# leopard-ai/betty

Measured on AMD Instinct MI355X. Metric: hypergradient-steps/sec (CG K=20, 10M inner params), higher is better.
Workload: dtype f32

## Files before the change

### betty_amd/_native.py

```python
from __future__ import annotations

import ctypes
import os
from ctypes import POINTER, c_char_p, c_double, c_float, c_int, c_int32, c_int64, c_size_t, c_void_p

_HERE = os.path.dirname(os.path.abspath(__file__))
LIB_PATH = os.environ.get("BHG_LIB") or os.path.join(_HERE, "csrc", "libbhg.so")
AB_LIB_PATH = os.environ.get("BHG_AB_LIB") or os.path.join(_HERE, "csrc", "libbhg_ab.so")

BHG_CHUNK_ELEMS = 4096
BHG_FLAT_ALIGN = 64
BHG_CG_AUTO, BHG_CG_STREAM, BHG_CG_RESIDENT = 0, 1, 2
BHG_CG_GLOBAL_CHAIN, BHG_CG_GLOBAL_UPDATE, BHG_CG_GLOBAL_DOTS = 0, 1, 2
BHG_CG_FX_BEGIN, BHG_CG_FX_CHAIN, BHG_CG_FX_GRAM, BHG_CG_FX_END = 0, 1, 2, 3


class NativeLibraryError(RuntimeError):
    """libbhg.so is missing or a call into it failed."""


class Chunk(ctypes.Structure):

    _fields_ = [
        ("flat_off", c_int64),
        ("src_off", c_int64),
        ("tensor", c_int32),
        ("len", c_int32),
    ]


BHG_MLP_MAX_LAYERS = 32


class Mlp(ctypes.Structure):

    _fields_ = [
        ("L", c_int32),
        ("B", c_int32),
        ("Bp", c_int32),
        ("dims", c_int32 * (BHG_MLP_MAX_LAYERS + 1)),
        ("W", c_void_p * BHG_MLP_MAX_LAYERS),
        ("h", c_void_p * BHG_MLP_MAX_LAYERS),
        ("mask", c_void_p * BHG_MLP_MAX_LAYERS),
        ("delta", c_void_p * BHG_MLP_MAX_LAYERS),
        ("prob", c_void_p),
        ("sd", c_void_p),
        ("Rh", c_void_p * BHG_MLP_MAX_LAYERS),
        ("Rd", c_void_p * BHG_MLP_MAX_LAYERS),
        ("partial", c_void_p),
        ("partial_floats", c_size_t),
        ("ridge2", c_float),
        ("prepacked", c_int32),
    ]


_PP = POINTER(c_void_p)
_CH = c_void_p

SYMBOLS = {
    "bhg_version": (c_int, []),
    "bhg_last_error": (c_char_p, []),
    "bhg_layout_flat_size": (c_int64, [POINTER(c_int64), c_int]),
    "bhg_layout_num_chunks": (c_int64, [POINTER(c_int64), c_int]),
    "bhg_layout_build": (c_int, [POINTER(c_int64), c_int, POINTER(c_int64), POINTER(Chunk)]),
    "bhg_workspace_bytes": (c_size_t, [c_int]),
    "bhg_flatten": (c_int, [_PP, c_int, _CH, c_int, c_void_p, c_float, c_void_p, c_void_p]),
    "bhg_scatter": (c_int, [c_void_p, _PP, c_int, _CH, c_int, c_float, c_void_p, c_void_p]),
    "bhg_neumann_init": (c_int, [_PP, c_int, _CH, c_int, c_void_p, c_void_p, c_void_p, c_void_p]),
    "bhg_neumann_step": (
        c_int,
        [_PP, c_int, _CH, c_int, c_void_p, c_void_p, c_float, c_float, c_float, c_void_p, c_void_p],
    ),
    "bhg_cg_init": (c_int, [_PP, c_int, _CH, c_int, c_void_p, c_void_p, c_void_p, c_void_p, c_void_p]),
    "bhg_cg_init_masked": (c_int, [_PP, c_int, _CH, c_int, c_void_p, c_void_p, c_void_p, ctypes.c_uint64, c_void_p, c_void_p]),
    "bhg_cg_step": (
        c_int,
        [_PP, c_int, _CH, c_int, c_void_p, c_void_p, c_void_p, c_float, c_int, c_float, c_float, c_int, c_void_p, c_void_p],
    ),
    "bhg_cg_phase": (
        c_int,
        [c_int, _PP, c_int, _CH, c_int, c_void_p, c_void_p, c_void_p, c_float, c_int, c_float, c_float, c_void_p, c_void_p],
    ),
    "bhg_cg_partials_dev": (c_void_p, [c_void_p, c_int, c_int]),
    "bhg_cg_partials_count": (c_int, []),
    "bhg_cg_resident_capacity_chunks": (c_int, []),
    "bhg_cg_resident_ok": (c_int, []),
    "bhg_cg_resident_usable": (c_int, [c_int]),
    "bhg_cg_scalars_dev": (c_void_p, [c_void_p]),
    "bhg_cg_timeout_flag_dev": (c_void_p, [c_void_p]),
    "bhg_scale_flat": (c_int, [c_void_p, c_int64, c_float, c_void_p]),
    "bhg_darts_eps": (c_int, [_PP, c_int, _CH, c_int, c_double, c_void_p, c_void_p, c_void_p, c_void_p]),
    "bhg_axpy_multi": (c_int, [_PP, _PP, c_int, _CH, c_int, c_void_p, c_float, c_void_p, c_void_p]),
    "bhg_fd_perturb": (c_int, [_PP, c_void_p, _PP, c_int, _CH, c_int, c_void_p, c_float, c_void_p, c_void_p]),
    "bhg_cg_step_fd": (
        c_int,
        [_PP, _PP, c_void_p, c_int, _CH, c_int, c_void_p, c_void_p, c_void_p, c_float, c_int, c_float, c_float, c_int, c_void_p, c_void_p],
    ),
    "bhg_neumann_step_fd": (
        c_int,
        [_PP, _PP, c_void_p, c_int, _CH, c_int, c_void_p, c_void_p, c_float, c_float, c_float, c_void_p, c_void_p],
    ),
    "bhg_sama_adam_precondition": (
        c_int,
        [_PP, _PP, _PP, _PP, c_int, _CH, c_int, c_void_p, c_double, c_double, c_double, c_double, c_void_p, c_void_p],
    ),
    "bhg_debug_set": (c_int, [c_char_p, c_int]),
    "bhg_debug_unset": (c_int, [c_char_p]),
    "bhg_debug_reset": (None, []),
    "bhg_debug_key_count": (c_int, []),
    "bhg_debug_key_name": (c_char_p, [c_int]),
    "bhg_is_ab_build": (c_int, []),
    "bhg_timing_enable": (c_int, [c_int]),
    "bhg_timing_read": (c_int, [c_int, POINTER(c_double), POINTER(c_int)]),
    "bhg_logreg_prepare": (c_int, [c_void_p, c_void_p, c_void_p, c_int, c_int, c_void_p]),
    "bhg_logreg_tmp_floats": (c_size_t, [c_int, c_int]),
    "bhg_logreg_hvp": (
        c_int,
        [c_void_p, c_void_p, c_void_p, c_void_p, c_void_p, c_void_p, c_int, c_int, c_void_p],
    ),
    "bhg_mlp_partial_floats": (c_size_t, [POINTER(Mlp)]),
    "bhg_mlp_hvp": (c_int, [POINTER(Mlp), _PP, _PP, c_void_p]),
    "bhg_mlp_hvp_mode": (c_int, [POINTER(Mlp), _PP, _PP, c_int, c_void_p]),
    "bhg_mlp_supports_native_prepare": (c_int, [POINTER(Mlp)]),
    "bhg_mlp_forward": (c_int, [POINTER(Mlp), _PP, c_void_p, c_void_p, c_void_p]),
    "bhg_mlp_backward": (c_int, [POINTER(Mlp), c_void_p, c_void_p]),
    "bhg_mlp_mixed_coeff": (c_int, [POINTER(Mlp), _PP, c_void_p, c_void_p, c_void_p]),
    "bhg_mlp_supports_fused_solve": (c_int, [POINTER(Mlp)]),
    "bhg_mlp_fused_ws_bytes": (c_size_t, [POINTER(Mlp)]),
    "bhg_mlp_cg_solve": (
        c_int,
        [POINTER(Mlp), c_void_p, c_void_p, c_void_p, POINTER(c_int64), _CH, c_int, c_int, c_float, c_float, c_void_p,
         c_void_p, c_size_t, c_void_p],
    ),
    "bhg_mlp_cg_state_mask": (ctypes.c_uint64, [POINTER(Mlp), c_int]),
    "bhg_mlp_cg_solve_rhs": (
        c_int,
        [POINTER(Mlp), c_void_p, c_void_p, c_void_p, POINTER(c_int64), _CH, c_int, c_int, c_float, c_float, c_void_p,
         c_void_p, c_size_t, _PP, c_void_p],
    ),
    "bhg_mlp_cg_global_phase": (
        c_int,
        [POINTER(Mlp), c_void_p, c_void_p, c_void_p, POINTER(c_int64), _CH, c_int, c_int, c_int, c_int, c_int, c_void_p, c_float,
         c_float, c_void_p, c_void_p, c_size_t, c_void_p],
    ),
    "bhg_mlp_fx_supported": (c_int, [POINTER(Mlp), c_int]),
    "bhg_mlp_fx_ws_bytes": (c_size_t, [POINTER(Mlp), c_int]),
    "bhg_mlp_fx_const_floats": (c_size_t, [POINTER(Mlp)]),
    "bhg_mlp_fx_slab_floats": (c_size_t, [POINTER(Mlp)]),
    "bhg_mlp_fx_scal_doubles": (c_size_t, [POINTER(Mlp)]),
    "bhg_mlp_cg_fx_phase": (
        c_int,
        [POINTER(Mlp), _PP, c_int, c_int, c_int, c_int, c_int, c_void_p, c_void_p, c_void_p, c_float, c_float, c_void_p, c_size_t,
         c_void_p, c_size_t, c_void_p],
    ),
    "bhg_mlp_neumann_fx_phase": (
        c_int,
        [POINTER(Mlp), _PP, c_int, c_int, c_int, c_int, c_int, c_void_p, c_void_p, c_void_p, c_float, c_float, c_void_p, c_size_t,
         c_void_p, c_size_t, c_void_p],
    ),
    "bhg_mlp_cg_mixed_coeff": (c_int, [POINTER(Mlp), c_void_p, c_void_p, c_float, c_void_p, c_size_t, c_void_p]),
    "bhg_mlp_timeout_flag_dev": (c_void_p, [POINTER(Mlp), c_void_p]),
    "bhg_mlp_stage_batch": (c_int, [POINTER(Mlp), c_void_p, c_void_p, c_void_p, c_void_p]),
    "bhg_mlp_supports_packed_prepare": (c_int, [POINTER(Mlp)]),
    "bhg_mlp_forward_packed": (c_int, [POINTER(Mlp), _PP, c_void_p, c_void_p, c_void_p, c_size_t, c_void_p]),
    "bhg_mlp_backward_packed": (c_int, [POINTER(Mlp), c_void_p, c_void_p, c_size_t, c_void_p]),
    "bhg_mwn_max_hidden": (c_int, []),
    "bhg_mlp_fd_ws_bytes": (c_size_t, [POINTER(c_int), c_int, c_int]),
    "bhg_mlp_fd_forward": (
        c_int,
        [c_void_p, c_void_p, c_int, POINTER(c_int), c_int, _PP, _PP, c_void_p, c_int, c_void_p, c_void_p, c_void_p, c_size_t, c_void_p],
    ),
    "bhg_mwn_fd_vjp": (
        c_int,
        [c_void_p, c_void_p, c_int, c_void_p, c_void_p, c_void_p, c_void_p, c_int, c_void_p, c_int, c_void_p, c_void_p, c_void_p, c_void_p,
         c_void_p],
    ),
    "bhg_quad_fd": (c_int, [_PP, _PP, _PP, c_int, _CH, c_int, c_void_p, c_float, c_int, c_int, c_int, c_void_p]),
    "bhg_mwn_forward": (c_int, [c_void_p, c_int, c_void_p, c_void_p, c_void_p, c_void_p, c_int, c_void_p, c_void_p, c_void_p]),
    "bhg_mwn_backward": (
        c_int,
        [c_void_p, c_void_p, c_int, c_void_p, c_void_p, c_void_p, c_void_p, c_int, c_float, c_void_p, c_void_p, c_void_p, c_void_p, c_void_p],
    ),
    "bhg_mlp_neumann_solve": (
        c_int,
        [POINTER(Mlp), c_void_p, c_void_p, c_void_p, POINTER(c_int64), c_int, c_float, c_float, c_void_p, c_size_t, POINTER(c_int), c_void_p],
    ),
    "bhg_mlp_wsk_launches": (c_int64, []),
    "bhg_mlp_hoist_launches": (c_int64, []),
    "bhg_mlp_proj_iterations": (c_int64, []),
    "bhg_mlp_lin_launches": (c_int64, []),
    "bhg_mlp_neumann_mixed_coeff": (c_int, [POINTER(Mlp), _PP, c_void_p, c_void_p, c_float, c_int, c_int, c_void_p, c_size_t, c_void_p]),
    "bhg_mlp_plan_describe": (c_int, [POINTER(Mlp), c_int, c_int, ctypes.c_char_p, c_size_t]),
    "bhg_copy2d": (c_int, [c_void_p, c_int64, c_void_p, c_int64, c_int64, c_int64, c_void_p]),
    "bhg_bn_ws_bytes": (c_size_t, [c_int]),
    "bhg_bn_backward_vjp": (
        c_int,
        [c_void_p, c_void_p, c_void_p, c_void_p, c_void_p, c_void_p, c_void_p, c_void_p, c_int, c_int, c_int, c_void_p, c_void_p, c_void_p,
         c_void_p, c_size_t, c_void_p],
    ),
}

_libs = {}
_current = [None]


_PY_ENV = {"BHG_LIB", "BHG_AB_LIB", "BHG_HVP_GRAPH", "BHG_ALL_RANKS_ON_GPU0"}
_warned_env = [False]


def _warn_legacy_env() -> None:
    if _warned_env[0]:
        return
    _warned_env[0] = True
    stale = sorted(k for k in os.environ if k.startswith("BHG_") and k not in _PY_ENV)
    if stale:
        import warnings

        warnings.warn("betty_amd: environment variable(s) " + ", ".join(stale) + " are IGNORED — libbhg reads no environment variable. "
                      "Measurement arms are selected with betty_amd._native.use_ab() + debug_set(key, int) (bench.py --debug KEY=INT) "
                      "on the measurement build libbhg_ab.so.", RuntimeWarning, stacklevel=3)


def _bind(path: str) -> ctypes.CDLL:
    lib = _libs.get(path)
    if lib is not None:
        return lib
    _warn_legacy_env()
    if not os.path.exists(path):
        raise NativeLibraryError(
            f"{path} not found: the HIP extension has not been built. Run "
            "`python -c 'import __graft_entry__ as g; g.build()'` or `make -C betty_amd/csrc`. "
            "betty_amd has no CPU fallback."
        )
    lib = ctypes.CDLL(path)
    for name, (restype, argtypes) in SYMBOLS.items():
        try:
            fn = getattr(lib, name)
        except AttributeError as exc:
            raise NativeLibraryError(f"{path} does not export {name}") from exc
        fn.restype = restype
        fn.argtypes = argtypes
    _libs[path] = lib
    return lib


def load() -> ctypes.CDLL:
    return _bind(_current[0] or LIB_PATH)


def current_lib_path() -> str:
    return _current[0] or LIB_PATH


def is_ab() -> bool:
    return bool(load().bhg_is_ab_build())


def use_ab(on: bool = True) -> None:
    if on:
        _bind(AB_LIB_PATH)
        _current[0] = AB_LIB_PATH
    else:
        _current[0] = None


def check(rc: int, what: str) -> None:
    if rc != 0:
        msg = load().bhg_last_error()
        raise NativeLibraryError(f"{what} failed with code {rc}: {msg.decode() if msg else ''}")


def _debug_key(key: str) -> bytes:
    k = key.strip()
    if k.upper().startswith("BHG_"):
        k = k[4:]
    return k.lower().encode()


def debug_set(key: str, value) -> None:
    lib = load()
    if value is not None and not lib.bhg_is_ab_build():
        raise NativeLibraryError(f"bhg_debug_set({key}): the product libbhg.so carries no measurement arm — call "
                                 "betty_amd._native.use_ab() first (libbhg_ab.so; the `bhg_debug` fixture and `bench.py --debug` do)")
    if value is None:
        check(lib.bhg_debug_unset(_debug_key(key)), f"bhg_debug_unset({key})")
    else:
        check(lib.bhg_debug_set(_debug_key(key), int(value)), f"bhg_debug_set({key})")


def debug_reset() -> None:
    load().bhg_debug_reset()


def debug_keys():
    lib = load()
    return [lib.bhg_debug_key_name(i).decode() for i in range(lib.bhg_debug_key_count())]


def ptr_array(ptrs):
    arr = (c_void_p * len(ptrs))(*ptrs)
    return ctypes.cast(arr, _PP), arr


def plan_describe(dims, B: int, algo: str = "cg", keep_solution: bool = False) -> dict:
    lib = load()
    d = Mlp()
    d.L, d.B, d.Bp = len(dims) - 1, int(B), (int(B) + 127) // 128 * 128
    for i, v in enumerate(dims):
        d.dims[i] = int(v)
    buf = ctypes.create_string_buffer(2048)
    check(lib.bhg_mlp_plan_describe(ctypes.byref(d), {"cg": 0, "neumann": 1}[algo], 1 if keep_solution else 0, buf, 2048), "bhg_mlp_plan_describe")
    out, text = {}, buf.value.decode()
    import re

    for key, quoted, plain in re.findall(r'(\w+)=(?:"([^"]*)"|(\S+))', text):
        val = quoted if quoted else plain
        out[key] = int(val) if re.fullmatch(r"-?\d+", val) else val
    return out
```

### betty_amd/csrc/bhg_common.hpp

```cpp
#pragma once
#include <hip/hip_runtime.h>
#include <stdint.h>
#include <stddef.h>
#include <stdio.h>
#include <string.h>

#include "bhg.h"

namespace bhg {

constexpr int kThreads = 256;
constexpr int kWaves = kThreads / 64;
constexpr int kChunk = BHG_CHUNK_ELEMS;
constexpr int kVecPerThread = kChunk / (kThreads * 4);
constexpr int kMaxBlocks = 1024;
constexpr int kInlineT = 32;
constexpr int kWriterT = 448;

constexpr size_t kWsScal = 0;
constexpr size_t kWsPartP = 128;
constexpr size_t kWsPartR = kWsPartP + 8 * kMaxBlocks;
constexpr size_t kWsBarrier = kWsPartR + 16 * kMaxBlocks;
constexpr size_t kWsTables = kWsBarrier + 256;
inline size_t ws_bytes(int T) {
  size_t b = kWsTables + 4 * sizeof(void*) * (size_t)(T > 0 ? T : 0);
  return (b + 255) & ~(size_t)255;
}

enum { S_RR_OLD = 0, S_PHP = 1, S_ALPHA = 2, S_RR_NEW = 3, S_BETA = 4, S_PP = 5 , S_ALPHA_RING = 10 ,
       S_NPART0 = 8  };

#define BHG_DBG_KEYS(X)                                                                                                      \
  X(mlp_wsk) X(mlp_wsk_maxk) X(mlp_wsk_depth) X(mlp_wsk_lds) X(wsl_depth) X(no_nt_slabs) X(gemm_no_xpose) X(mlp_no_fast)      \
  X(mlp_tn) X(split_target) X(split_cap) X(mlp_no_head) X(gram_ksplit) X(gram_kchunk) X(proj_graw_split) X(mlp_proj)         \
  X(mlp_hoist) X(hoist_wgs) X(proj_step_alone) X(mlp_no_side) X(mlp_no_fuse) X(mlp_no_outer_all) X(neumann_side)             \
  X(hoist_staged_mink) X(proj_alpha_alone) X(proj_small_alone) X(outer_order_by_work) X(outer_no_pre) X(outer_stagger)       \
  X(mlp_no_fused_solve) X(cg_eager_p) X(cg_x_every_iter) X(neumann_p_every_iter) X(head_no_prefetch) X(cg_spin_limit)        \
  X(packed_chain) X(packed_depth) X(packed_gram) X(proj_max_ratio) X(proj_ws_cap_mb) X(alpha_in_hoist) X(graw_v2) X(wskp_ragged) X(pstep_v2) X(pstep_unroll) X(rnew_in_graw) X(graw_cols) X(lin_first) X(lin_prio) X(lin_nub) X(lin_order) X(lin_update_next) X(lin_withhold_beta) X(neumann_vnew) X(cg_rhs_direct) X(packed_prepare) X(lin_deep) X(graw_kloop) X(lin_update_in_head) X(xcd_pairs) X(headu_head_first) X(fx_ksplit)
enum DbgKey : int {
#define BHG_DBG_ENUM(n) DBG_##n,
  BHG_DBG_KEYS(BHG_DBG_ENUM)
#undef BHG_DBG_ENUM
  DBG_COUNT
};
constexpr int kDbgUnset = INT32_MIN;
#ifdef BHG_AB
extern int g_dbg[DBG_COUNT];
inline bool dbg_is_set(DbgKey k) { return g_dbg[k] != kDbgUnset; }
inline int dbg(DbgKey k, int dflt) { return g_dbg[k] == kDbgUnset ? dflt : g_dbg[k]; }
#else
constexpr bool dbg_is_set(DbgKey) { return false; }
constexpr int dbg(DbgKey, int dflt) { return dflt; }
#endif

constexpr int kStampKernels = 4, kStampBlocks = 4096, kStampSlots = 8;
#ifdef BHG_STAMPS
#ifdef __HIPCC__
#define BHG_STAMP(kid, slot)                                                                                            \
  do {                                                                                                                  \
    if (threadIdx.x == 0 && blockIdx.x < ::bhg::kStampBlocks) {                                                         \
      unsigned long long* sp_ = ::bhg::d_stamps;                                                                        \
      if (sp_) sp_[((kid) * ::bhg::kStampBlocks + blockIdx.x) * ::bhg::kStampSlots + (slot)] = wall_clock64();          \
    }                                                                                                                   \
  } while (0)
#endif
#else
#define BHG_STAMP(kid, slot) do { } while (0)
#endif

void set_error(const char* fmt, ...);
#define BHG_HIP_CHECK(expr)                                                        \
  do {                                                                             \
    hipError_t _e = (expr);                                                        \
    if (_e != hipSuccess) {                                                        \
      ::bhg::set_error("%s failed: %s (%s:%d)", #expr, hipGetErrorString(_e), __FILE__, \
                       __LINE__);                                                  \
      return BHG_ERR_HIP;                                                          \
    }                                                                              \
  } while (0)
#define BHG_REQUIRE(cond, msg)                                                     \
  do {                                                                             \
    if (!(cond)) {                                                                 \
      ::bhg::set_error("%s: %s", __func__, msg);                                   \
      return BHG_ERR_ARG;                                                          \
    }                                                                              \
  } while (0)

struct PtrTab {
  const void* const* dev;
  const void* inl[kInlineT];
};

int make_table(PtrTab* out, const void* const* host_ptrs, int T, void* ws, int slot,
               hipStream_t stream);

bool span_begin(int kind, hipEvent_t* a, hipEvent_t* b);

#ifdef __HIPCC__
__device__ __forceinline__ float* tab_ptr(const PtrTab& t, int i) {
  const void* p = t.dev ? t.dev[i] : t.inl[i];
  return (float*)p;
}

__device__ __forceinline__ float4 ld4(const float* __restrict__ base, int e, int len) {
  if (e + 4 <= len) return *reinterpret_cast<const float4*>(base + e);
  float4 r = make_float4(0.f, 0.f, 0.f, 0.f);
  if (e < len) r.x = base[e];
  if (e + 1 < len) r.y = base[e + 1];
  if (e + 2 < len) r.z = base[e + 2];
  return r;
}
__device__ __forceinline__ void st4(float* __restrict__ base, int e, int len, float4 v) {
  if (e + 4 <= len) {
    *reinterpret_cast<float4*>(base + e) = v;
    return;
  }
  if (e < len) base[e] = v.x;
  if (e + 1 < len) base[e + 1] = v.y;
  if (e + 2 < len) base[e + 2] = v.z;
}

template <int BYTES>
__device__ __forceinline__ void kernarg_warm() {
  typedef const __attribute__((address_space(4))) unsigned* KP;
  KP kp = (KP)__builtin_amdgcn_kernarg_segment_ptr();
  unsigned acc = 0;
#pragma unroll
  for (int o = 0; o < BYTES; o += 64) acc |= kp[o / 4];
  asm volatile("" ::"s"(acc));
}
template <int U>
__device__ __forceinline__ double sum_strided(const double* __restrict__ p, const int n, const int t, const int stride) {
  double acc = 0.0;
  for (int i0 = t; i0 < n; i0 += U * stride) {
    double v[U];
#pragma unroll
    for (int u = 0; u < U; ++u) {
      const int i = i0 + u * stride;
      v[u] = p[i < n ? i : n - 1];
    }
#pragma unroll
    for (int u = 0; u < U; ++u)
      if (i0 + u * stride < n) acc += v[u];
  }
  return acc;
}

template <int U>
struct StridedRegs { double v[U]; };
template <int U>
__device__ __forceinline__ void strided_load(StridedRegs<U>& r, const double* __restrict__ p, const int n, const int t, const int stride,
                                             const double* __restrict__ dummy) {
  const double* q = (p && n > 0) ? p : dummy;
  const int last = (p && n > 0) ? n - 1 : 0;
#pragma unroll
  for (int u = 0; u < U; ++u) {
    const int i = t + u * stride;
    r.v[u] = q[i < n && i <= last ? i : last];
  }
}
template <int U>
__device__ __forceinline__ double strided_sum(const StridedRegs<U>& r, const int n, const int t, const int stride) {
  double acc = 0.0;
#pragma unroll
  for (int u = 0; u < U; ++u)
    if (t + u * stride < n) acc += r.v[u];
  return acc;
}

template <int CTRL>
__device__ __forceinline__ double dpp_mov_f64(const double v) {
  const unsigned long long u = __builtin_bit_cast(unsigned long long, v);
  const unsigned lo = (unsigned)__builtin_amdgcn_mov_dpp((int)(unsigned)u, CTRL, 0xf, 0xf, true);
  const unsigned hi = (unsigned)__builtin_amdgcn_mov_dpp((int)(unsigned)(u >> 32), CTRL, 0xf, 0xf, true);
  return __builtin_bit_cast(double, ((unsigned long long)hi << 32) | (unsigned long long)lo);
}
__device__ __forceinline__ double readlane_f64(const double v, const int lane) {
  const unsigned long long u = __builtin_bit_cast(unsigned long long, v);
  const unsigned lo = (unsigned)__builtin_amdgcn_readlane((int)(unsigned)u, lane);
  const unsigned hi = (unsigned)__builtin_amdgcn_readlane((int)(unsigned)(u >> 32), lane);
  return __builtin_bit_cast(double, ((unsigned long long)hi << 32) | (unsigned long long)lo);
}
__device__ __forceinline__ double wave_sum(double v) {
  v += dpp_mov_f64<0xB1>(v);
  v += dpp_mov_f64<0x4E>(v);
  v += dpp_mov_f64<0x141>(v);
  v += dpp_mov_f64<0x140>(v);
  const double r0 = readlane_f64(v, 0), r1 = readlane_f64(v, 16), r2 = readlane_f64(v, 32), r3 = readlane_f64(v, 48);
  return (r0 + r1) + (r2 + r3);
}
template <int CTRL>
__device__ __forceinline__ float dpp_mov_f32(const float v) {
  return __builtin_bit_cast(float, __builtin_amdgcn_mov_dpp(__builtin_bit_cast(int, v), CTRL, 0xf, 0xf, true));
}
__device__ __forceinline__ float wave_sum_f32(float v) {
  v += dpp_mov_f32<0xB1>(v);
  v += dpp_mov_f32<0x4E>(v);
  v += dpp_mov_f32<0x141>(v);
  v += dpp_mov_f32<0x140>(v);
  const float r0 = __builtin_bit_cast(float, __builtin_amdgcn_readlane(__builtin_bit_cast(int, v), 0));
  const float r1 = __builtin_bit_cast(float, __builtin_amdgcn_readlane(__builtin_bit_cast(int, v), 16));
  const float r2 = __builtin_bit_cast(float, __builtin_amdgcn_readlane(__builtin_bit_cast(int, v), 32));
  const float r3 = __builtin_bit_cast(float, __builtin_amdgcn_readlane(__builtin_bit_cast(int, v), 48));
  return (r0 + r1) + (r2 + r3);
}
__device__ __forceinline__ void block_sum3(double& a, double& b, double& c, double* red) {
  const double wa = wave_sum(a), wb = wave_sum(b), wc = wave_sum(c);
  const int lane = threadIdx.x & 63, w = threadIdx.x >> 6;
  __syncthreads();
  if (lane == 0) { red[w] = wa; red[kWaves + w] = wb; red[2 * kWaves + w] = wc; }
  __syncthreads();
  double sa = 0.0, sb = 0.0, sc = 0.0;
#pragma unroll
  for (int i = 0; i < kWaves; ++i) { sa += red[i]; sb += red[kWaves + i]; sc += red[2 * kWaves + i]; }
  a = sa; b = sb; c = sc;
}
__device__ __forceinline__ double block_sum(double v, double* red) {
  v = wave_sum(v);
  const int lane = threadIdx.x & 63, w = threadIdx.x >> 6;
  __syncthreads();
  if (lane == 0) red[w] = v;
  __syncthreads();
  double s = 0.0;
#pragma unroll
  for (int i = 0; i < kWaves; ++i) s += red[i];
  return s;
}
__device__ __forceinline__ double sum_partials(const double* __restrict__ part, int n,
                                               double* red) {
  double a = 0.0;
  for (int i = threadIdx.x; i < n; i += kThreads) a += part[i];
  return block_sum(a, red);
}
#endif

}
```

### betty_amd/csrc/bhg_mlp.hip

```cpp
#include <stdlib.h>
#include <vector>


#include "bhg_common.hpp"

#ifdef BHG_STAMPS
namespace bhg { __device__ unsigned long long* d_stamps = nullptr; }
#endif

namespace bhg {
namespace {
#include "mlp/gemm.inc"

#include "mlp/outer.inc"

#include "mlp/scalars.inc"

#include "mlp/head.inc"

#include "mlp/wsk.inc"

#include "mlp/wskp.inc"

inline int wsk_mode(int chain_mode, int unfused_hint) {
  if (dbg_is_set(DBG_mlp_wsk)) return dbg(DBG_mlp_wsk, 0);
  if (chain_mode == FUSE_CG) return 2;
  if (chain_mode == FUSE_NEUMANN) return 3;
  return unfused_hint;
}
inline bool wsk_wanted(int mode, int pairs, int K) {
  if (mode == 1) return true;
  if (mode != 2 && mode != 3) return false;
  return pairs * K <= dbg(DBG_mlp_wsk_maxk, 1024);
}
inline int wsk_depth() {
  const int d = dbg(DBG_mlp_wsk_depth, 3);
  return d == 2 ? 2 : 3;
}
inline bool wsk_eligible(const WskArgs& a) {
  if (a.pairs < 1 || a.pairs > 2) return false;
  bool ok = a.M % 32 == 0 && a.N % 32 == 0 && a.K % 32 == 0 && a.K >= 32;
  for (int i = 0; i < a.pairs; ++i) ok = ok && (a.pr[i].lda & 3) == 0 && (a.pr[i].ldb & 3) == 0;
  return ok;
}
int64_t g_wsk_launches = 0;
int64_t g_hoist_launches = 0;
int64_t g_proj_iterations = 0;
int64_t g_lin_launches = 0;
template <int LB>
void launch_gemm_wsk(const WskArgs& a_in, hipStream_t st, bool staged = false) {
  WskArgs a = a_in;
  ++g_wsk_launches;
  a.ntm = a.M / 32;
  a.ntn = a.N / 32;
  bool bf = false;
  for (int i = 0; i < a.pairs; ++i) bf = bf || a.pr[i].mix != 0;
  const dim3 grid(a.ntm * a.ntn), block(64 * kWskWaves);
  const int d = wsk_depth();
  const bool force_staged = dbg(DBG_mlp_wsk_lds, 0) != 0;
  if ((staged || force_staged) && !bf) {
    const int lds = (int)(sizeof(float) * kWslWaveFloats * kWskWaves);
    static bool attr_done = false;
    if (!attr_done) {
      (void)hipFuncSetAttribute(reinterpret_cast<const void*>(k_gemm_wsk<LB, false, 2, true>), hipFuncAttributeMaxDynamicSharedMemorySize, lds);
      attr_done = true;
    }
#ifdef BHG_AB
    const int wsl_depth = dbg(DBG_wsl_depth, 2);
    if (wsl_depth == 3) {
      static bool attr3 = false;
      if (!attr3) {
        (void)hipFuncSetAttribute(reinterpret_cast<const void*>(k_gemm_wsk<LB, false, 3, true>), hipFuncAttributeMaxDynamicSharedMemorySize, lds);
        attr3 = true;
      }
      hipLaunchKernelGGL((k_gemm_wsk<LB, false, 3, true>), grid, block, lds, st, a);
      return;
    }
#endif
    hipLaunchKernelGGL((k_gemm_wsk<LB, false, 2, true>), grid, block, lds, st, a);
    return;
  }
#define BHG_WSK(BFV, DV) hipLaunchKernelGGL((k_gemm_wsk<LB, BFV, DV>), grid, block, 0, st, a)
  if (bf) {
    if (d == 2 || LB == LAYOUT_RC) BHG_WSK(true, 2); else BHG_WSK(true, LB == LAYOUT_RC ? 2 : 3);
  } else {
#ifdef BHG_AB
    if (d == 2) BHG_WSK(false, 2); else
#endif
    BHG_WSK(false, 3);
  }
#undef BHG_WSK
}

#ifdef BHG_AB
void launch_wsk_group(const WskGroupArgs& g, int blocks, hipStream_t st) {
  const int lds = (int)(sizeof(float) * kWslWaveFloats * kWskWaves);
  static bool attr_done = false;
  if (!attr_done) {
    (void)hipFuncSetAttribute(reinterpret_cast<const void*>(k_wsk_group<2>), hipFuncAttributeMaxDynamicSharedMemorySize, lds);
#ifdef BHG_AB
    (void)hipFuncSetAttribute(reinterpret_cast<const void*>(k_wsk_group<3>), hipFuncAttributeMaxDynamicSharedMemorySize, lds);
#endif
    attr_done = true;
  }
#ifdef BHG_AB
  const int wsl_depth = dbg(DBG_wsl_depth, 2);
  if (wsl_depth == 3) { hipLaunchKernelGGL(k_wsk_group<3>, dim3(blocks), dim3(64 * kWskWaves), lds, st, g); return; }
#endif
  hipLaunchKernelGGL(k_wsk_group<2>, dim3(blocks), dim3(64 * kWskWaves), lds, st, g);
}
#endif

int chip_cus() {
  static int cus[64];
  int dev = 0;
  if (hipGetDevice(&dev) != hipSuccess || dev < 0 || dev >= 64) { (void)hipGetLastError(); return 256; }
  if (cus[dev] > 0) return cus[dev];
  int n = 0;
  if (hipDeviceGetAttribute(&n, hipDeviceAttributeMultiprocessorCount, dev) != hipSuccess || n <= 0) { (void)hipGetLastError(); n = 256; }
  return cus[dev] = n;
}
inline void wskp_tiling(WskpProb* q, bool ragged) {
  q->nfull = q->RA / 32;
  q->nstrip = 0;
  q->pairs = dbg(DBG_xcd_pairs, 1);
  if (!ragged || q->raw || q->nsplit != 1 || q->RB % 64 != 0) return;
  int nf = q->B / 32, rem = q->B % 32;
  if (rem > 16) { ++nf; rem = 0; }
  if (nf == 0) return;
  q->nfull = nf;
  q->nstrip = rem > 0 ? q->RB / 64 : 0;
}
struct WskpBuilder {
  WskpArgs g{};
  int blk = 0;
  bool add(const WskpProb& q_in) {
    if (g.n >= kWskpMax) return false;
    g.p[g.n++] = q_in;
    return true;
  }
  void tile(bool ragged) {
    blk = 0;
    for (int i = 0; i < g.n; ++i) {
      WskpProb& q = g.p[i];
      wskp_tiling(&q, ragged);
      g.blk0[i] = blk;
      blk += (((q.nfull * (q.RB / 32) + q.nstrip) * q.nsplit) + 7) & ~7;
    }
  }
  void launch(hipStream_t st) {
    if (!g.n) return;
    const int mode = dbg(DBG_wskp_ragged, 1);
    tile(mode == 2);
    if (mode == 1 && blk > chip_cus()) tile(true);
    g.blk0[g.n] = blk;
    const int d = dbg(DBG_packed_depth, 2);
    bool riders = g.n <= 3;
    for (int i = 1; i < g.n && riders; ++i) {
      const WskpProb& r = g.p[i];
      riders = r.raw && r.nsplit == 1 && r.RA == g.p[0].RA && r.RB == g.p[0].RA && r.B == g.p[0].B && !r.bias && !r.mask && !r.addend &&
               !r.partT2 && r.nstrip == 0 && r.nfull == r.RA / 32;
    }
    if (riders) {
      WskpcArgs c{};
      c.a = g.p[0];
      c.na = g.n >= 2 ? g.blk0[1] : blk;
      if (g.n >= 2) { c.r0 = {g.p[1].Ap, g.p[1].Bq, g.p[1].out, g.p[1].outp, g.p[1].K, 0}; c.nr0 = (g.n == 3 ? g.blk0[2] : blk) - g.blk0[1]; }
      if (g.n == 3) c.r1 = {g.p[2].Ap, g.p[2].Bq, g.p[2].out, g.p[2].outp, g.p[2].K, 0};
#ifdef BHG_AB
      if (d != 2) hipLaunchKernelGGL(k_wskpc<3>, dim3(blk), dim3(64 * kWskpWaves), 0, st, c); else
#endif
      hipLaunchKernelGGL(k_wskpc<2>, dim3(blk), dim3(64 * kWskpWaves), 0, st, c);
    } else {
#ifdef BHG_AB
      if (d != 2) hipLaunchKernelGGL(k_wskp<3>, dim3(blk), dim3(64 * kWskpWaves), 0, st, g); else
#endif
      hipLaunchKernelGGL(k_wskp<2>, dim3(blk), dim3(64 * kWskpWaves), 0, st, g);
    }
    (void)d;
    g = WskpArgs{};
    blk = 0;
  }
};

template <int LA, int LB>
void launch_gemm(const GemmArgs& a_in, int tn, hipStream_t st) {
  GemmArgs a = a_in;
  const bool nt_slabs = dbg(DBG_no_nt_slabs, 0) == 0;
  a.nt_out = (nt_slabs && (a.splits > 1 || a.out_rows > 0)) ? 1 : 0;
  const bool xpose = dbg(DBG_gemm_no_xpose, 0) == 0;
  a.xpose_out = xpose ? 1 : 0;
  dim3 grid((a.N + tn - 1) / tn, (a.M + kTM - 1) / kTM, a.splits);
  bool fast = a.M % kTM == 0 && a.N % tn == 0 && a.K % kTK == 0;
  bool bf = false;
  for (int i = 0; i < a.pairs; ++i) {
    fast = fast && (a.pr[i].lda & 3) == 0 && (a.pr[i].ldb & 3) == 0;
    bf = bf || a.pr[i].mix != 0;
  }
  if (bf)
    for (int i = 0; i < a.pairs; ++i)
      if (!a.pr[i].mix) a.pr[i].B2 = a.pr[i].B;
  const bool no_fast = dbg(DBG_mlp_no_fast, 0) != 0;
  if (no_fast) fast = false;
#define BHG_GEMM(TNV, F, BFV) hipLaunchKernelGGL((k_gemm<LA, LB, TNV, F, BFV>), grid, dim3(256), 0, st, a)
#ifdef BHG_AB
  if (tn == 64) {
    if (bf) { if (fast) BHG_GEMM(64, true, true); else BHG_GEMM(64, false, true); }
    else    { if (fast) BHG_GEMM(64, true, false); else BHG_GEMM(64, false, false); }
  } else
#endif
  {
    if (bf) { if (fast) BHG_GEMM(32, true, true); else BHG_GEMM(32, false, true); }
    else    { if (fast) BHG_GEMM(32, true, false); else BHG_GEMM(32, false, false); }
  }
#undef BHG_GEMM
}
inline int skinny_tile_n() {
  const int tn = dbg(DBG_mlp_tn, 32);
  return tn == 64 ? 64 : 32;
}

void launch_reduce_mask(hipStream_t st, const float* part, int splits, int slab, const float* bias,
                        const float* mask, float* out, int rows, int N, int B, float* relu_mask_out = nullptr,
                        float* outp = nullptr) {
  if ((N & 3) == 0) {
    int blocks = (slab / 4 + 255) / 256;
    if (blocks > 2048) blocks = 2048;
    hipLaunchKernelGGL(k_reduce_mask<4>, dim3(blocks), dim3(256), 0, st, part, splits, slab, bias, mask, out, rows, N, B,
                       relu_mask_out, outp);
  } else {
    int blocks = (slab + 255) / 256;
    if (blocks > 2048) blocks = 2048;
    hipLaunchKernelGGL(k_reduce_mask<1>, dim3(blocks), dim3(256), 0, st, part, splits, slab, bias, mask, out, rows, N, B,
                       relu_mask_out, (float*)nullptr);
  }
}

int pick_splits(int tiles, int K, int pairs) {
  const int ksteps = (K + kTK - 1) / kTK;
  const int target = dbg(DBG_split_target, 768);
  int s = (target + tiles - 1) / tiles;
  if (s > ksteps) s = ksteps;
  const int cap = dbg(DBG_split_cap, 16);
  if (s > cap) s = cap;
  if (s < 1) s = 1;
  if (ksteps % s != 0) {
    for (int d = 1; d <= 2; ++d) {
      if (s - d >= 1 && ksteps % (s - d) == 0) { s -= d; break; }
      if (s + d <= cap && s + d <= ksteps && ksteps % (s + d) == 0) { s += d; break; }
    }
  }
  return s;
}

#include "mlp/recurrence.inc"

#include "mlp/proj.inc"

#include "mlp/graw.inc"

#include "mlp/pstep.inc"
#include "mlp/wskpl.inc"
#include "mlp/headu.inc"

void launch_wskpu(const WskpProb& q_in, const PstepArgs& ps, int nu, hipStream_t st) {
  WskpuArgs u{};
  WskpProb q = q_in;
  const int mode = dbg(DBG_wskp_ragged, 1);
  wskp_tiling(&q, mode == 2);
  int blk = (((q.nfull * (q.RB / 32) + q.nstrip) * q.nsplit) + 7) & ~7;
  if (mode == 1 && blk > chip_cus()) {
    wskp_tiling(&q, true);
    blk = (((q.nfull * (q.RB / 32) + q.nstrip) * q.nsplit) + 7) & ~7;
  }
  u.c.a = q; u.c.na = blk;
  u.nu = nu; u.ps = ps;
  hipLaunchKernelGGL((k_wskpu<2, 4>), dim3(nu + blk), dim3(64 * kWskpWaves), 0, st, u);
}

struct SideState {
  hipStream_t side;
  hipEvent_t ev_rd[BHG_MLP_MAX_LAYERS];
  hipEvent_t ev_join;
};
int side_state(SideState** out) {
  static SideState per_device[64];
  int dev = 0;
  BHG_HIP_CHECK(hipGetDevice(&dev));
  BHG_REQUIRE(dev >= 0 && dev < 64, "device index out of range");
  SideState& ss = per_device[dev];
  if (!ss.side) {
    BHG_HIP_CHECK(hipStreamCreateWithFlags(&ss.side, hipStreamNonBlocking));
    const unsigned fl = hipEventDisableTiming | hipEventDisableSystemFence;
    for (int i = 0; i < BHG_MLP_MAX_LAYERS; ++i) BHG_HIP_CHECK(hipEventCreateWithFlags(&ss.ev_rd[i], fl));
    BHG_HIP_CHECK(hipEventCreateWithFlags(&ss.ev_join, fl));
#define BHG_OUTER_LDS(F, M) \
    BHG_HIP_CHECK(hipFuncSetAttribute(reinterpret_cast<const void*>(k_outer<F, M>), hipFuncAttributeMaxDynamicSharedMemorySize, 96 * 1024))
    BHG_OUTER_LDS(true, FUSE_NONE); BHG_OUTER_LDS(false, FUSE_NONE);
    BHG_OUTER_LDS(true, FUSE_CG); BHG_OUTER_LDS(false, FUSE_CG);
    BHG_OUTER_LDS(true, FUSE_NEUMANN); BHG_OUTER_LDS(false, FUSE_NEUMANN);
#undef BHG_OUTER_LDS
#ifdef BHG_AB
    BHG_HIP_CHECK(hipFuncSetAttribute(reinterpret_cast<const void*>(k_outer_all<FUSE_CG, false>), hipFuncAttributeMaxDynamicSharedMemorySize, 96 * 1024));
    BHG_HIP_CHECK(hipFuncSetAttribute(reinterpret_cast<const void*>(k_outer_all<FUSE_NEUMANN, false>), hipFuncAttributeMaxDynamicSharedMemorySize, 96 * 1024));
#endif
    BHG_HIP_CHECK(hipFuncSetAttribute(reinterpret_cast<const void*>(k_outer_all<FUSE_CG, true>), hipFuncAttributeMaxDynamicSharedMemorySize, 96 * 1024));
    BHG_HIP_CHECK(hipFuncSetAttribute(reinterpret_cast<const void*>(k_outer_all<FUSE_NEUMANN, true>), hipFuncAttributeMaxDynamicSharedMemorySize, 96 * 1024));
// ... 1262 lines not shown
  c->cg_alpha = cg_alpha; c->shift = hvp_shift; c->rhs = nullptr;
  carve_fused_ws(m, fws, &c->w);
  char* wsb = static_cast<char*>(ws);
  c->scal = reinterpret_cast<double*>(wsb + kWsScal);
  c->partR0 = reinterpret_cast<const double*>(wsb + kWsPartR);
  c->n_init = n_chunks < kMaxBlocks ? n_chunks : kMaxBlocks;
  for (int i = 0; i < 2 * m->L; ++i) c->dir[i] = p + starts[i];
  c->pgrid = n_chunks < kMaxBlocks ? n_chunks : kMaxBlocks;
  const bool eager = dbg(DBG_cg_eager_p, 0) != 0;
  c->lazy = global || !eager;
  BetaArgs& ba = c->ba;
  ba = BetaArgs{};
  int small_total = 0;
  {
    const bool head = use_head(m);
    ba.stride = c->w.nRR; ba.n = c->w.nRR; ba.scal = c->scal; ba.r = r; ba.p = p;
    for (int l = 0; l < m->L; ++l) {
      ba.off[ba.nt] = starts[2 * l + 1]; ba.len[ba.nt] = m->dims[l + 1]; small_total += ba.len[ba.nt]; ++ba.nt;
    }
    if (head) {
      ba.off[ba.nt] = starts[2 * (m->L - 1)]; ba.len[ba.nt] = m->dims[m->L] * m->dims[m->L - 1]; small_total += ba.len[ba.nt]; ++ba.nt;
    }
  }
  c->bgrid = small_total > 0 ? (small_total + kThreads - 1) / kThreads : 1;
  c->hplan.ok = false;
  if (c->lazy && hoist_mode() != 0) hoist_plan(m, &c->hplan);
  c->hoist = c->lazy && c->hplan.ok;
  c->proj_level = (!c->hoist || !c->hplan.proj_ok || proj_mode() == 0 || global) ? 0 : ((proj_mode() == 9 || x) ? 1 : 2);
  c->lin = c->proj_level == 2 && c->hplan.lin_ok && packed_chain_on(c->w) && dbg(DBG_packed_gram, 1) != 0 && dbg(DBG_graw_v2, 1) != 0 &&
           graw_batch_ok(m->Bp) && dbg(DBG_proj_small_alone, 0) == 0 && dbg(DBG_alpha_in_hoist, 1) != 0 && dbg(DBG_rnew_in_graw, 1) != 0 &&
           c->ba.nt <= 16 && proj_step_merged() && dbg(DBG_pstep_v2, 1) != 0 && dbg(DBG_lin_first, 1) != 0;
  c->lin_head = c->lin && m->L == 4 && dbg(DBG_lin_update_next, 1) != 0 && dbg(DBG_lin_update_in_head, 1) != 0 && dbg(DBG_lin_nub, 0) == 0 &&
                m->dims[m->L] <= 12 && m->dims[m->L - 1] <= 512 && dbg(DBG_head_no_prefetch, 0) == 0;
}
static int cg_iteration(CgCtx* c, int k, int gphase, double* php, double inv_world, hipStream_t st) {
  const bhg_mlp* m = c->m;
  FusedWs& w = c->w;
  const int K = c->K;
  const bool lazy = c->lazy, hoist = c->hoist;
  hipEvent_t ta, tb, tc, td;
  const bool timed = gphase == 0 && span_begin(BHG_TIMING_MLP_HVP, &ta, &tb);
  const bool timed_it = gphase == 0 && span_begin(BHG_TIMING_MLP_CG_ITER, &tc, &td);
  if (timed_it) BHG_HIP_CHECK(hipEventRecord(tc, st));
  if (lazy && k > 0 && gphase != 2) {
    c->ba.part = w.partRR[k & 1];
    if (!hoist || c->proj_level == 1) hipLaunchKernelGGL(k_cg_beta, dim3(c->bgrid), dim3(kThreads), 0, st, c->ba);
  }
  if (timed) BHG_HIP_CHECK(hipEventRecord(ta, st));
  ChainMode cm{};
  cm.mode = FUSE_CG;
  cm.fa = c->r; cm.fb = c->x; cm.fd = c->p; cm.starts = c->starts;
  cm.shift = c->shift; cm.cg_alpha = c->cg_alpha;
  cm.apply_out = k == K - 1; cm.out_scale = -c->cg_alpha;
  cm.ws = &w; cm.scal = c->scal;
  cm.partRR_old = c->partR0;
  cm.nRR_old = k == 0 ? c->n_init : 0;
  cm.partPP = k == 0 ? c->partR0 : w.partPP;
  cm.nPP = k == 0 ? c->n_init : (lazy ? 0 : c->pgrid);
  cm.partRR_new = w.partRR[(k + 1) & 1];
  cm.lazy = lazy;
  const bool x_every = dbg(DBG_cg_x_every_iter, 0) != 0;
  cm.x_mode = (lazy && !x_every) ? ((k & 1) ? 2 : (k + 1 < K ? 1 : 0)) : 0;
  if (!c->x) cm.x_mode = 1;
  cm.skip_outputs = (!c->x && k == K - 1) ? 1 : 0;
  cm.first = k == 0;
  cm.kpar = k & 1;
  cm.hoist = hoist ? &c->hplan : nullptr;
  cm.beta = &c->ba; cm.beta_blocks = c->bgrid;
  cm.proj = c->proj_level;
  cm.gphase = gphase; cm.php = php; cm.inv_world = inv_world;
  cm.second = k == 1;
  if (c->proj_level == 2 && proj_step_merged())
    c->dir[1] = k == 0 ? static_cast<const void*>(c->p + c->starts[1]) : static_cast<const void*>(w.pb0[k & 1]);
  if (c->lin) c->dir[3] = k == 0 ? static_cast<const void*>(c->p + c->starts[3]) : static_cast<const void*>(w.pb1[k & 1]);
  cm.lin = c->lin ? 1 : 0;
  cm.lin_head = c->lin_head ? 1 : 0;
  cm.rhs = c->rhs;
  if (int rc = run_chain(m, c->dir, cm, st)) return rc;
  if (timed) BHG_HIP_CHECK(hipEventRecord(tb, st));
#ifdef BHG_AB
  if (!lazy && k + 1 < K)
    hipLaunchKernelGGL(k_cg_pdir, dim3(c->pgrid), dim3(kThreads), 0, st, c->chunks_dev, c->n_chunks, (const float*)c->r, c->p,
                       (const double*)w.partRR[(k + 1) & 1], w.nRR, w.partPP, c->scal);
#endif
  if (timed_it) BHG_HIP_CHECK(hipEventRecord(td, st));
  return BHG_OK;
}

int bhg_mlp_cg_solve(const bhg_mlp* m, float* x, float* r, float* p, const int64_t* starts,
                     const bhg_chunk* chunks_dev, int n_chunks, int K, float cg_alpha, float hvp_shift, void* ws,
                     void* fws, size_t fws_bytes, void* stream) {
  return bhg_mlp_cg_solve_rhs(m, x, r, p, starts, chunks_dev, n_chunks, K, cg_alpha, hvp_shift, ws, fws, fws_bytes, nullptr, stream);
}

unsigned long long bhg_mlp_cg_state_mask(const bhg_mlp* m, int has_x) {
  if (!m || m->L < 1 || m->L > BHG_MLP_MAX_LAYERS || 2 * m->L > 64 || has_x || !bhg_mlp_supports_fused_solve(m)) return ~0ull;
  HoistPlan hp;
  hp.ok = false;
  if (dbg(DBG_cg_eager_p, 0) == 0 && hoist_mode() != 0) hoist_plan(m, &hp);
  const bool level2 = hp.ok && hp.proj_ok && proj_mode() != 0 && proj_mode() != 9;
  if (!level2 || dbg(DBG_cg_rhs_direct, 1) == 0) return ~0ull;
  unsigned long long mask = 0ull;
  for (int l = 0; l < m->L; ++l) mask |= 1ull << (2 * l + 1);
  mask |= 1ull << (2 * (m->L - 1));
  return mask;
}

int bhg_mlp_cg_solve_rhs(const bhg_mlp* m, float* x, float* r, float* p, const int64_t* starts,
                         const bhg_chunk* chunks_dev, int n_chunks, int K, float cg_alpha, float hvp_shift, void* ws,
                         void* fws, size_t fws_bytes, const void* const* rhs, void* stream) {
  if (int rc = solve_common_checks(m, starts, fws, fws_bytes)) return rc;
  BHG_REQUIRE(r && p && ws && chunks_dev, "NULL argument");
  BHG_REQUIRE(K >= 0 && n_chunks > 0, "bad size");
  if (K == 0) return BHG_OK;
  hipStream_t st = static_cast<hipStream_t>(stream);
  CgCtx c;
  cg_ctx_init(&c, m, x, r, p, starts, chunks_dev, n_chunks, K, cg_alpha, hvp_shift, ws, fws, false);
  BHG_REQUIRE(!rhs || c.proj_level == 2, "rhs names the right-hand side for the FULLY PROJECTED solver only (see bhg_mlp_cg_state_mask)");
  if (rhs)
    for (int l = 0; l + 1 < m->L; ++l) BHG_REQUIRE(rhs[2 * l] && ((uintptr_t)rhs[2 * l] & 15) == 0, "rhs tensors must be 16-byte aligned device pointers");
  c.rhs = rhs;
  if (c.hoist && packed_chain_on(c.w) && !m->prepacked)
    if (int rc = pack_operands(m, c.w, st)) return rc;
  for (int k = 0; k < K; ++k)
    if (int rc = cg_iteration(&c, k, 0, nullptr, 1.0, st)) return rc;
  BHG_HIP_CHECK(hipGetLastError());
  return BHG_OK;
}

int bhg_mlp_cg_global_phase(const bhg_mlp* m, float* x, float* r, float* p, const int64_t* starts, const bhg_chunk* chunks_dev,
                            int n_chunks, int k, int K, int phase, int world, double* php, float cg_alpha, float hvp_shift,
                            void* ws, void* fws, size_t fws_bytes, void* stream) {
  if (int rc = solve_common_checks(m, starts, fws, fws_bytes)) return rc;
  BHG_REQUIRE(r && p && ws && chunks_dev && php, "NULL argument");
  BHG_REQUIRE(K > 0 && k >= 0 && k < K && n_chunks > 0 && world >= 1, "bad size");
  BHG_REQUIRE(phase == BHG_CG_GLOBAL_CHAIN || phase == BHG_CG_GLOBAL_UPDATE || phase == BHG_CG_GLOBAL_DOTS, "unknown phase");
  hipStream_t st = static_cast<hipStream_t>(stream);
  CgCtx c;
  cg_ctx_init(&c, m, x, r, p, starts, chunks_dev, n_chunks, K, cg_alpha, hvp_shift, ws, fws, true);
  if (phase == BHG_CG_GLOBAL_DOTS) {
    BHG_REQUIRE(k + 1 < K, "the last iteration has no direction update");
    int grid = n_chunks < c.w.nRR ? n_chunks : c.w.nRR;
    if (grid > kMaxBlocks) grid = kMaxBlocks;
    hipLaunchKernelGGL(k_cg_global_dots, dim3(grid), dim3(kThreads), 0, st, chunks_dev, n_chunks, (const float*)r, (const float*)p,
                       c.w.partRR[(k + 1) & 1], c.w.nRR, c.w.nRR);
    BHG_HIP_CHECK(hipGetLastError());
    return BHG_OK;
  }
  if (k == 0 && phase == BHG_CG_GLOBAL_CHAIN && c.hoist && packed_chain_on(c.w) && !m->prepacked)
    if (int rc = pack_operands(m, c.w, st)) return rc;
  if (int rc = cg_iteration(&c, k, phase == BHG_CG_GLOBAL_CHAIN ? 1 : 2, php, 1.0 / (double)world, st)) return rc;
  BHG_HIP_CHECK(hipGetLastError());
  return BHG_OK;
}

int bhg_mlp_fx_supported(const bhg_mlp* m, int world) {
  if (!m || m->L < 1 || m->L > BHG_MLP_MAX_LAYERS || m->Bp <= 0 || m->Bp % kTM != 0 || !bhg_mlp_supports_fused_solve(m)) return 0;
  FxPlan fp;
  fx_plan(m, world, &fp);
  return fp.ok && dbg(DBG_packed_chain, 1) != 0 ? 1 : 0;
}
size_t bhg_mlp_fx_ws_bytes(const bhg_mlp* m, int world) {
  if (!bhg_mlp_fx_supported(m, world)) return 0;
  FxPlan fp; fx_plan(m, world, &fp);
  FxWs x; fx_carve(m, fp, nullptr, &x);
  return x.bytes;
}
size_t bhg_mlp_fx_const_floats(const bhg_mlp* m) {
  if (!bhg_mlp_fx_supported(m, 1)) return 0;
  FxPlan fp; fx_plan(m, 1, &fp);
  return fp.const_floats;
}
size_t bhg_mlp_fx_slab_floats(const bhg_mlp* m) {
  if (!bhg_mlp_fx_supported(m, 1)) return 0;
  FxPlan fp; fx_plan(m, 1, &fp);
  return fp.slab_floats;
}
size_t bhg_mlp_fx_scal_doubles(const bhg_mlp* m) {
  if (!bhg_mlp_fx_supported(m, 1)) return 0;
  FxPlan fp; fx_plan(m, 1, &fp);
  return fp.scal_doubles;
}
static int fx_phase(int algo, const bhg_mlp* m, const void* const* rhs, int k, int K, int phase, int world, int rank, float* const_all,
                    float* slab_all, double* scal_all, float alpha, float hvp_shift, void* fws, size_t fws_bytes, void* xws, size_t xws_bytes,
                    void* stream) {
  if (int rc = check_mlp(m)) return rc;
  const bool neumann = algo == 1;
  BHG_REQUIRE(world >= 1 && rank >= 0 && rank < world, "bad world size / rank");
  BHG_REQUIRE(bhg_mlp_fx_supported(m, world), "this network does not take the factor-exchange form (bhg_mlp_fx_supported)");
  BHG_REQUIRE(phase == BHG_CG_FX_BEGIN || phase == BHG_CG_FX_CHAIN || phase == BHG_CG_FX_GRAM || phase == BHG_CG_FX_END, "unknown phase");
  BHG_REQUIRE(K > 0 && k >= 0 && (k < K || (neumann && k == K && (phase == BHG_CG_FX_CHAIN || phase == BHG_CG_FX_END))), "bad iteration index");
  BHG_REQUIRE(const_all && slab_all && scal_all && fws && xws, "NULL argument");
  BHG_REQUIRE(m->partial && m->partial_floats >= bhg_mlp_partial_floats(m), "split-K scratch too small");
  BHG_REQUIRE(fws_bytes >= bhg_mlp_fused_ws_bytes(m), "fused workspace too small");
  BHG_REQUIRE(xws_bytes >= bhg_mlp_fx_ws_bytes(m, world), "factor-exchange workspace too small");
  hipStream_t st = static_cast<hipStream_t>(stream);
  FxPlan fp;
  fx_plan(m, world, &fp);
  FusedWs w;
  carve_fused_ws(m, fws, &w);
  FxWs x;
  fx_carve(m, fp, xws, &x);
  const bhg_mlp ml = fx_local(m, fp, slab_all, rank);
  double* scal_mine = scal_all + (size_t)rank * fp.scal_doubles;
  if (phase == BHG_CG_FX_BEGIN) {
    BHG_REQUIRE(k == 0, "BEGIN belongs to iteration 0");
    return fx_begin(m, fp, const_all, rank, st);
  }
  if (phase == BHG_CG_FX_CHAIN) {
    if (k == 0) {
      BHG_REQUIRE(rhs, "iteration 0 reads the right-hand side");
      for (int l = 0; l + 1 < m->L; ++l) BHG_REQUIRE(rhs[2 * l] && ((uintptr_t)rhs[2 * l] & 15) == 0, "rhs tensors must be 16-byte aligned device pointers");
      for (int i = 0; i < 2 * m->L; ++i) BHG_REQUIRE(rhs[i], "rhs holds 2 L device pointers");
      if (int rc = fx_first(m, &ml, fp, w, x, rhs, const_all, rank, st, neumann)) return rc;
    } else {
      if (int rc = fx_step(&ml, fp, w, x, scal_all, k - 1, false, alpha, hvp_shift, st, neumann)) return rc;
    }
    return fx_chain(&ml, fp, w, x, k & 1, st, neumann && k == K);
  }
  if (phase == BHG_CG_FX_GRAM) {
    BHG_REQUIRE(k < K, "GRAM belongs to iterations 0 .. K-1");
    return fx_gram(&ml, fp, w, x, slab_all, const_all, scal_mine, k & 1, hvp_shift, st);
  }
  BHG_REQUIRE(k == (neumann ? K : K - 1), "END belongs to the last iteration");
  return fx_step(&ml, fp, w, x, scal_all, k, true, alpha, hvp_shift, st, neumann);
}
int bhg_mlp_cg_fx_phase(const bhg_mlp* m, const void* const* rhs, int k, int K, int phase, int world, int rank, float* const_all,
                        float* slab_all, double* scal_all, float cg_alpha, float hvp_shift, void* fws, size_t fws_bytes, void* xws,
                        size_t xws_bytes, void* stream) {
  return fx_phase(0, m, rhs, k, K, phase, world, rank, const_all, slab_all, scal_all, cg_alpha, hvp_shift, fws, fws_bytes, xws, xws_bytes, stream);
}
int bhg_mlp_neumann_fx_phase(const bhg_mlp* m, const void* const* rhs, int k, int K, int phase, int world, int rank, float* const_all,
                             float* slab_all, double* scal_all, float alpha, float hvp_shift, void* fws, size_t fws_bytes, void* xws,
                             size_t xws_bytes, void* stream) {
  return fx_phase(1, m, rhs, k, K, phase, world, rank, const_all, slab_all, scal_all, alpha, hvp_shift, fws, fws_bytes, xws, xws_bytes, stream);
}

int bhg_mlp_neumann_solve(const bhg_mlp* m, float* v0, float* v1, float* p, const int64_t* starts, int K, float alpha,
                          float hvp_shift, void* fws, size_t fws_bytes, int* projected_out, void* stream) {
  if (int rc = solve_common_checks(m, starts, fws, fws_bytes)) return rc;
  BHG_REQUIRE(v0 && v1, "NULL argument");
  BHG_REQUIRE(K >= 0, "bad size");
  BHG_REQUIRE(p || use_head(m), "the accumulator-free Neumann solver needs the narrow-head kernels");
  hipStream_t st = static_cast<hipStream_t>(stream);
  FusedWs w;
  carve_fused_ws(m, fws, &w);
  HoistPlan hplan;
  hplan.ok = false;
  const bool want_proj = !p && K > 0 && proj_mode() != 0 && hoist_mode() != 0;
  if (hoist_mode() == 2 || want_proj) hoist_plan(m, &hplan);
  const bool proj = want_proj && hplan.ok && hplan.proj_ok && use_head(m);
  if (projected_out) *projected_out = proj ? 1 : 0;
  if (hplan.ok && K > 0 && packed_chain_on(w) && !m->prepacked)
    if (int rc = pack_operands(m, w, st)) return rc;
  for (int k = 0; k < K; ++k) {
    float* vin = (k & 1) ? v1 : v0;
    float* vout = (k & 1) ? v0 : v1;
    const void* dir[2 * BHG_MLP_MAX_LAYERS];
    for (int i = 0; i < 2 * m->L; ++i) dir[i] = vin + starts[i];
    hipEvent_t ta, tb;
    const bool timed = span_begin(BHG_TIMING_MLP_HVP, &ta, &tb);
    if (timed) BHG_HIP_CHECK(hipEventRecord(ta, st));
    ChainMode cm{};
    cm.mode = FUSE_NEUMANN;
    cm.fa = vout; cm.fb = p; cm.fd = vin; cm.starts = starts;
    cm.alpha = alpha; cm.shift = hvp_shift;
    cm.apply_out = k == K - 1; cm.out_scale = -alpha;
    const bool p_every = dbg(DBG_neumann_p_every_iter, 0) != 0;
    cm.x_mode = p_every ? 0 : ((k & 1) ? 2 : (k + 1 < K ? 1 : 0));
    cm.first = k == 0;
    if (!p) { cm.x_mode = 1; cm.rzx_acc = w.rzx; }
    cm.ws = &w;
    cm.hoist = hplan.ok ? &hplan : nullptr;
    cm.proj = proj ? 1 : 0;
    cm.nk = k;
    if (int rc = run_chain(m, dir, cm, st)) return rc;
    if (timed) BHG_HIP_CHECK(hipEventRecord(tb, st));
  }
  if (proj) {
    float* vin = (K & 1) ? v1 : v0;
    const void* dir[2 * BHG_MLP_MAX_LAYERS];
    for (int i = 0; i < 2 * m->L; ++i) dir[i] = vin + starts[i];
    ChainMode cm{};
    cm.mode = FUSE_NEUMANN;
    cm.fa = (K & 1) ? v0 : v1; cm.fb = nullptr; cm.fd = vin; cm.starts = starts;
    cm.alpha = alpha; cm.shift = hvp_shift;
    cm.x_mode = 1; cm.rzx_acc = w.rzx; cm.first = 0;
    cm.ws = &w; cm.hoist = &hplan; cm.proj = 1; cm.stop_after_head = 1; cm.nk = K;
    if (int rc = run_chain(m, dir, cm, st)) return rc;
  }
  return BHG_OK;
}

int bhg_mlp_cg_mixed_coeff(const bhg_mlp* m, const int64_t* labels, float* coeff, float cg_alpha, void* fws,
                           size_t fws_bytes, void* stream) {
  if (int rc = check_mlp(m)) return rc;
  BHG_REQUIRE(labels && coeff && fws, "NULL argument");
  BHG_REQUIRE(fws_bytes >= bhg_mlp_fused_ws_bytes(m), "fused workspace too small");
  FusedWs w;
  carve_fused_ws(m, fws, &w);
  hipLaunchKernelGGL(k_coeff_from_rzx, dim3((m->Bp + kThreads - 1) / kThreads), dim3(kThreads), 0, static_cast<hipStream_t>(stream),
                     (const double*)w.rzx, m->prob, labels, coeff, m->Bp, m->dims[m->L], m->B, -cg_alpha, 0.f);
  BHG_HIP_CHECK(hipGetLastError());
  return BHG_OK;
}

static int check_head_problem(const bhg_mlp* m) {
  BHG_REQUIRE(m, "NULL descriptor");
  BHG_REQUIRE(m->L >= 1 && m->L <= BHG_MLP_MAX_LAYERS, "unsupported layer count");
  BHG_REQUIRE(m->Bp > 0 && m->Bp % kTM == 0 && m->B >= 1 && m->B <= m->Bp, "Bp must be a multiple of 128 rows >= B");
  BHG_REQUIRE(m->partial && m->partial_floats >= bhg_mlp_partial_floats(m), "split-K scratch too small");
  return BHG_OK;
}
static bool narrow_head(const bhg_mlp* m) { return m->dims[m->L] <= kSmallC && (m->dims[m->L - 1] & 3) == 0; }

int bhg_mlp_supports_native_prepare(const bhg_mlp* m) {
  return m && m->L >= 1 && m->L <= BHG_MLP_MAX_LAYERS && m->Bp > 0 && m->Bp % kTM == 0;
}

}
namespace bhg {
namespace {
__global__ __launch_bounds__(kThreads) void k_softmax_ce_rows(float* __restrict__ z, const int64_t* __restrict__ labels,
                                                              float* __restrict__ ce, int C, int B) {
  __shared__ double red[kWaves];
  __shared__ float redf[kWaves];
  const int b = blockIdx.x, t = threadIdx.x;
  float* row = z + (int64_t)b * C;
  if (b >= B) {
    for (int c = t; c < C; c += kThreads) row[c] = 0.f;
    if (t == 0) ce[b] = 0.f;
    return;
  }
  float mx = -INFINITY;
  for (int c = t; c < C; c += kThreads) mx = fmaxf(mx, row[c]);
  for (int o = 32; o > 0; o >>= 1) mx = fmaxf(mx, __shfl_xor(mx, o));
  if ((t & 63) == 0) redf[t >> 6] = mx;
  __syncthreads();
  mx = redf[0];
  for (int w = 1; w < kWaves; ++w) mx = fmaxf(mx, redf[w]);
  double s = 0.0;
  for (int c = t; c < C; c += kThreads) s += (double)expf(row[c] - mx);
  s = block_sum(s, red);
  const float lse = mx + logf((float)s);
  const float zy = row[(int)labels[b]];
  __syncthreads();
  for (int c = t; c < C; c += kThreads) row[c] = expf(row[c] - lse);
  if (t == 0) ce[b] = lse - zy;
}
__global__ __launch_bounds__(kThreads) void k_coeff_rows(const float* __restrict__ prob, const float* __restrict__ rz,
                                                         const int64_t* __restrict__ labels, float* __restrict__ coeff, int C, int B) {
  __shared__ double red[kWaves];
  const int b = blockIdx.x, t = threadIdx.x;
  if (b >= B) { if (t == 0) coeff[b] = 0.f; return; }
  const int y = (int)labels[b];
  double s = 0.0;
  for (int c = t; c < C; c += kThreads) s += (double)((prob[(int64_t)b * C + c] - (c == y ? 1.f : 0.f)) * rz[(int64_t)b * C + c]);
  s = block_sum(s, red);
  if (t == 0) coeff[b] = (float)(s / (double)B);
}
}
}
using namespace bhg;
extern "C" {

int bhg_mlp_forward(const bhg_mlp* m, const void* const* bias, const int64_t* labels, float* ce, void* stream) {
  if (int rc = check_head_problem(m)) return rc;
  BHG_REQUIRE(bias && labels && ce, "NULL argument");
  hipStream_t st = static_cast<hipStream_t>(stream);
  const int L = m->L, Bp = m->Bp, B = m->B;
  for (int l = 0; l < L; ++l) {
    const int K = m->dims[l], N = m->dims[l + 1];
    const float* b = static_cast<const float*>(bias[l]);
    if (l == L - 1 && narrow_head(m)) {
      launch_head_forward(st, Bp, nullptr, m->h[l], m->W[l] , m->W[l], b, nullptr, nullptr,
                          const_cast<float*>(m->prob), K, N, B, HEAD_LOGITS, labels, ce, nullptr, nullptr, nullptr);
      break;
    }
    GemmArgs a{};
    a.pr[0] = {m->h[l], m->W[l], K, K};
    a.pairs = 1;
    a.M = Bp; a.N = N; a.K = K;
    const int tn = skinny_tile_n();
    a.splits = pick_splits((N + tn - 1) / tn, K, 1);
    a.out = m->partial; a.ldo = N; a.out_rows = Bp;
    launch_gemm<LAYOUT_KC, LAYOUT_KC>(a, tn, st);
    if (l == L - 1) {
      launch_reduce_mask(st, m->partial, a.splits, Bp * N, b, nullptr, const_cast<float*>(m->prob), Bp, N, B);
      hipLaunchKernelGGL(k_softmax_ce_rows, dim3(Bp), dim3(kThreads), 0, st, const_cast<float*>(m->prob), labels, ce, N, B);
      break;
    }
    launch_reduce_mask(st, m->partial, a.splits, Bp * N, b, nullptr, const_cast<float*>(m->h[l + 1]), Bp, N, B,
                       const_cast<float*>(m->mask[l]));
  }
  BHG_HIP_CHECK(hipGetLastError());
  return BHG_OK;
}

int bhg_mlp_backward(const bhg_mlp* m, const int64_t* labels, void* stream) {
  if (int rc = check_head_problem(m)) return rc;
  BHG_REQUIRE(labels, "NULL argument");
  hipStream_t st = static_cast<hipStream_t>(stream);
  const int L = m->L, Bp = m->Bp, B = m->B;
  const int C = m->dims[L];
  hipLaunchKernelGGL(k_delta_top, dim3((Bp * C + 255) / 256), dim3(256), 0, st, m->prob, m->sd, labels,
                     const_cast<float*>(m->delta[L - 1]), Bp, C, B);
  for (int l = L - 1; l >= 1; --l) {
    const int K = m->dims[l + 1], N = m->dims[l];
    if (l == L - 1 && narrow_head(m)) {
      const int blocks = (Bp * (N / 4) + 255) / 256;
      hipLaunchKernelGGL(k_head_backward, dim3(blocks), dim3(256), 0, st, (const float*)nullptr, m->delta[l], m->W[l],
                         (const float*)nullptr, m->mask[l - 1], const_cast<float*>(m->delta[l - 1]), N, K, B, Bp);
      continue;
    }
    GemmArgs a{};
    a.pr[0] = {m->delta[l], m->W[l], K, N};
    a.pairs = 1;
    a.M = Bp; a.N = N; a.K = K;
    const int tn = skinny_tile_n();
    a.splits = pick_splits((N + tn - 1) / tn, K, 1);
    a.out = m->partial; a.ldo = N; a.out_rows = Bp;
    launch_gemm<LAYOUT_KC, LAYOUT_RC>(a, tn, st);
    launch_reduce_mask(st, m->partial, a.splits, Bp * N, nullptr, m->mask[l - 1], const_cast<float*>(m->delta[l - 1]), Bp,
                       N, B);
  }
  BHG_HIP_CHECK(hipGetLastError());
  return BHG_OK;
}

int bhg_mlp_supports_packed_prepare(const bhg_mlp* m) {
  if (!bhg_mlp_supports_native_prepare(m) || !bhg_mlp_supports_fused_solve(m) || dbg(DBG_packed_prepare, 1) == 0) return 0;
  HoistPlan hp;
  hoist_plan(m, &hp);
  return hp.ok && dbg(DBG_packed_chain, 1) != 0 ? 1 : 0;
}

int bhg_mlp_forward_packed(const bhg_mlp* m, const void* const* bias, const int64_t* labels, float* ce, void* fws, size_t fws_bytes,
                           void* stream) {
  if (int rc = check_head_problem(m)) return rc;
  BHG_REQUIRE(narrow_head(m), "the packed once-per-step passes need a narrow classifier head (<= 256 classes, feature width % 4 == 0)");
  BHG_REQUIRE(bias && labels && ce && fws, "NULL argument");
  BHG_REQUIRE(bhg_mlp_supports_packed_prepare(m), "this network does not take the packed form (bhg_mlp_supports_packed_prepare)");
  BHG_REQUIRE(fws_bytes >= bhg_mlp_fused_ws_bytes(m), "fused workspace too small");
  hipStream_t st = static_cast<hipStream_t>(stream);
  const int L = m->L, Bp = m->Bp, B = m->B;
  FusedWs w;
  carve_fused_ws(m, fws, &w);
  if (int rc = pack_operands(m, w, st, true)) return rc;
  {
    const int K = m->dims[0], N = m->dims[1];
    GemmArgs a{};
    a.pr[0] = {m->h[0], m->W[0], K, K};
    a.pairs = 1;
    a.M = Bp; a.N = N; a.K = K;
    const int tn = skinny_tile_n();
    a.splits = pick_splits((N + tn - 1) / tn, K, 1);
    a.out = m->partial; a.ldo = N; a.out_rows = Bp;
    launch_gemm<LAYOUT_KC, LAYOUT_KC>(a, tn, st);
    launch_reduce_mask(st, m->partial, a.splits, Bp * N, static_cast<const float*>(bias[0]), nullptr, const_cast<float*>(m->h[1]), Bp, N, B,
                       const_cast<float*>(m->mask[0]), w.hpk[1]);
  }
  for (int l = 1; l + 1 < L; ++l) {
    WskpfArgs f{};
    WskpProb& q = f.a;
    q.Ap = w.hpk[l]; q.Bq = w.Wf[l]; q.RA = Bp; q.RB = m->dims[l + 1]; q.K = m->dims[l]; q.B = B; q.nsplit = 1;
    q.bias = static_cast<const float*>(bias[l]);
    q.out = const_cast<float*>(m->h[l + 1]);
    q.outp = l + 2 < L ? w.hpk[l + 1] : nullptr;
    f.relu_mask = const_cast<float*>(m->mask[l]);
    wskp_tiling(&q, false);
    const int blk = q.nfull * (q.RB / 32) + q.nstrip;
    hipLaunchKernelGGL(k_wskpf<2>, dim3(blk), dim3(64 * kWskpWaves), 0, st, f);
  }
  launch_head_forward(st, Bp, nullptr, m->h[L - 1], m->W[L - 1] , m->W[L - 1], static_cast<const float*>(bias[L - 1]),
                      nullptr, nullptr, const_cast<float*>(m->prob), m->dims[L - 1], m->dims[L], B, HEAD_LOGITS, labels, ce, nullptr,
                      nullptr, nullptr);
  BHG_HIP_CHECK(hipGetLastError());
  return BHG_OK;
}

int bhg_mlp_backward_packed(const bhg_mlp* m, const int64_t* labels, void* fws, size_t fws_bytes, void* stream) {
  if (int rc = check_head_problem(m)) return rc;
  BHG_REQUIRE(narrow_head(m), "the packed once-per-step passes need a narrow classifier head (<= 256 classes, feature width % 4 == 0)");
  BHG_REQUIRE(labels && fws, "NULL argument");
  BHG_REQUIRE(bhg_mlp_supports_packed_prepare(m), "this network does not take the packed form (bhg_mlp_supports_packed_prepare)");
  BHG_REQUIRE(fws_bytes >= bhg_mlp_fused_ws_bytes(m), "fused workspace too small");
  hipStream_t st = static_cast<hipStream_t>(stream);
  const int L = m->L, Bp = m->Bp, B = m->B;
  const int C = m->dims[L];
  FusedWs w;
  carve_fused_ws(m, fws, &w);
  hipLaunchKernelGGL(k_delta_top, dim3((Bp * C + 255) / 256), dim3(256), 0, st, m->prob, m->sd, labels,
                     const_cast<float*>(m->delta[L - 1]), Bp, C, B);
  {
    const int l = L - 1, K = m->dims[l + 1], N = m->dims[l];
    const int blocks = (Bp * (N / 4) + 255) / 256;
    hipLaunchKernelGGL(k_head_backward, dim3(blocks), dim3(256), 0, st, (const float*)nullptr, m->delta[l], m->W[l],
                       (const float*)nullptr, m->mask[l - 1], const_cast<float*>(m->delta[l - 1]), N, K, B, Bp, w.dpk[l - 1]);
  }
  for (int l = L - 2; l >= 1; --l) {
    WskpBuilder wb;
    WskpProb q{};
    q.Ap = w.dpk[l]; q.Bq = w.Wb[l]; q.RA = Bp; q.RB = m->dims[l]; q.K = m->dims[l + 1]; q.B = B; q.nsplit = 1;
    q.mask = m->mask[l - 1]; q.out = const_cast<float*>(m->delta[l - 1]);
    q.outp = l >= 2 ? w.dpk[l - 1] : nullptr;
    wb.add(q);
    wb.launch(st);
  }
  BHG_HIP_CHECK(hipGetLastError());
  return BHG_OK;
}

__global__ __launch_bounds__(256) void k_stage_batch(const float* __restrict__ x, const int64_t* __restrict__ y, float* __restrict__ h0,
                                                     int64_t* __restrict__ labels, int64_t n4, int B) {
  for (int64_t i = (int64_t)blockIdx.x * 256 + threadIdx.x; i < n4; i += (int64_t)gridDim.x * 256)
    reinterpret_cast<float4*>(h0)[i] = reinterpret_cast<const float4*>(x)[i];
  if (blockIdx.x == 0)
    for (int b = threadIdx.x; b < B; b += 256) labels[b] = y[b];
}
int bhg_mlp_stage_batch(const bhg_mlp* m, const float* x, const int64_t* y, int64_t* labels, void* stream) {
  if (int rc = check_mlp(m)) return rc;
  BHG_REQUIRE(x && y && labels && m->h[0], "NULL argument");
  BHG_REQUIRE((m->dims[0] & 3) == 0 && ((uintptr_t)x & 15) == 0, "the input batch must be 16-byte aligned with a width that is a multiple of 4");
  const int64_t n4 = (int64_t)m->B * m->dims[0] / 4;
  int blocks = (int)((n4 + 255) / 256);
  if (blocks > 2048) blocks = 2048;
  if (blocks < 1) blocks = 1;
  hipLaunchKernelGGL(k_stage_batch, dim3(blocks), dim3(256), 0, static_cast<hipStream_t>(stream), x, y, const_cast<float*>(m->h[0]), labels, n4, m->B);
  BHG_HIP_CHECK(hipGetLastError());
  return BHG_OK;
}

int bhg_mlp_mixed_coeff(const bhg_mlp* m, const void* const* dir, const int64_t* labels, float* coeff, void* stream) {
  if (int rc = check_head_problem(m)) return rc;
  BHG_REQUIRE(dir && labels && coeff, "NULL argument");
  hipStream_t st = static_cast<hipStream_t>(stream);
  const int L = m->L, Bp = m->Bp, B = m->B;
  for (int l = 0; l < L; ++l) {
    const int K = m->dims[l], N = m->dims[l + 1];
    const float* V = static_cast<const float*>(dir[2 * l]);
    const float* c = static_cast<const float*>(dir[2 * l + 1]);
    if (l == L - 1 && narrow_head(m)) {
      launch_head_forward(st, Bp, l > 0 ? (const float*)m->Rh[l - 1] : nullptr, m->h[l], m->W[l], V, c, m->prob, nullptr,
                          nullptr, K, N, B, HEAD_COEFF, labels, coeff, nullptr, nullptr, nullptr);
      break;
    }
    GemmArgs a{};
    a.pr[0] = {m->h[l], V, K, K};
    a.pairs = 1;
    if (l > 0) { a.pr[1] = {m->Rh[l - 1], m->W[l], K, K}; a.pairs = 2; }
    a.M = Bp; a.N = N; a.K = K;
    const int tn = skinny_tile_n();
    a.splits = pick_splits((N + tn - 1) / tn, K, a.pairs);
    a.out = m->partial; a.ldo = N; a.out_rows = Bp;
    launch_gemm<LAYOUT_KC, LAYOUT_KC>(a, tn, st);
    if (l == L - 1) {
      launch_reduce_mask(st, m->partial, a.splits, Bp * N, c, nullptr, m->Rd[l], Bp, N, B);
      hipLaunchKernelGGL(k_coeff_rows, dim3(Bp), dim3(kThreads), 0, st, m->prob, (const float*)m->Rd[l], labels, coeff, N, B);
      break;
    }
    launch_reduce_mask(st, m->partial, a.splits, Bp * N, c, m->mask[l], m->Rh[l], Bp, N, B);
  }
  BHG_HIP_CHECK(hipGetLastError());
  return BHG_OK;
}

int bhg_mlp_plan_describe(const bhg_mlp* m, int algo, int keep_solution, char* buf, size_t buf_bytes) {
  if (int rc = check_mlp(m)) return rc;
  BHG_REQUIRE(buf && buf_bytes >= 64, "output buffer too small");
  BHG_REQUIRE(algo == 0 || algo == 1, "algo: 0 = cg, 1 = neumann");
  const int L = m->L;
  const bool fused = bhg_mlp_supports_fused_solve(m) != 0;
  HoistPlan hp;
  hoist_plan(m, &hp);
  const char* form = "unfused";
  int hoist = 0, proj_level = 0, lin = 0, lin_head = 0, upd_first = 0;
  const char* closing = "k_outer_all";
  if (fused) {
    int64_t numel[2 * BHG_MLP_MAX_LAYERS], starts[2 * BHG_MLP_MAX_LAYERS];
    for (int l = 0; l < L; ++l) { numel[2 * l] = (int64_t)m->dims[l] * m->dims[l + 1]; numel[2 * l + 1] = m->dims[l + 1]; }
    const int64_t nch = bhg_layout_num_chunks(numel, 2 * L);
    std::vector<bhg_chunk> chunks((size_t)(nch > 0 ? nch : 1));
    if (int rc = bhg_layout_build(numel, 2 * L, starts, chunks.data())) return rc;
    float* const fake = reinterpret_cast<float*>((uintptr_t)1 << 30);
    if (algo == 0) {
      static CgCtx c;
      cg_ctx_init(&c, m, keep_solution ? fake : nullptr, fake, fake, starts, nullptr, (int)nch, 2, 1.f, 0.f, fake, fake, false);
      hoist = c.hoist ? 1 : 0; proj_level = c.proj_level; lin = c.lin ? 1 : 0; lin_head = c.lin_head ? 1 : 0;
      upd_first = (c.lin && L > 4) ? 1 : 0;
      form = !c.lazy ? "classic-eager" : (!c.hoist ? "classic" : (c.proj_level == 0 ? "hoisted" : (c.proj_level == 1 ? "projected-keep-state" :
             (c.lin ? (c.lin_head ? "six-launch (k_wskpl .. k_headu .. k_graw)" : "six-launch-class (k_wskpl first, recurrences beside the chain)") :
              "fully-projected (k_pstep launch)"))));
      if (c.proj_level >= 1) closing = graw_batch_ok(m->Bp) ? (m->Bp == 128 ? "k_graw" : "k_grawk") : "k_hoist+k_proj_update";
    } else {
      const bool want_proj = !keep_solution && proj_mode() != 0 && hoist_mode() != 0;
      const bool proj = want_proj && hp.ok && hp.proj_ok && use_head(m);
      hoist = (hp.ok && (hoist_mode() == 2 || want_proj)) ? 1 : 0;
      proj_level = proj ? 1 : 0;
      form = proj ? "projected-neumann (update inside k_graw)" : (hoist ? "hoisted" : "classic");
      if (proj) closing = graw_batch_ok(m->Bp) ? (m->Bp == 128 ? "k_graw" : "k_grawk") : "k_hoist+k_proj_update";
    }
  }
  size_t gram = 0;
  if (hp.ok && hp.proj_ok)
    for (int l = 0; l + 1 < L; ++l) gram += (size_t)m->Bp * m->Bp * (l >= 1 ? (2 + 2 * kGramSplitMax + 6) : 2);
  const int n = snprintf(buf, buf_bytes,
                         "algo=%s keep_solution=%d fused=%d form=\"%s\" hoist=%d proj_level=%d lin=%d lin_head=%d upd_first=%d closing=%s "
                         "plan_ok=%d proj_ok=%d lin_ok=%d hoist_products=%d hoist_wgs=%d gram_floats=%zu fused_ws_bytes=%zu narrow_head=%d packed_prepare=%d "
                         "global_form=%s fx_slab_bytes=%zu fx_ws_bytes_world8=%zu",
                         algo == 0 ? "cg" : "neumann", keep_solution ? 1 : 0, fused ? 1 : 0, form, hoist, proj_level, lin, lin_head, upd_first, closing,
                         hp.ok ? 1 : 0, hp.proj_ok ? 1 : 0, hp.lin_ok ? 1 : 0, hp.n, hp.ok ? hp.blk0[hp.n] : 0, gram,
                         fused ? bhg_mlp_fused_ws_bytes(m) : (size_t)0, narrow_head(m) ? 1 : 0, bhg_mlp_supports_packed_prepare(m),
                         (algo == 0 && !keep_solution && bhg_mlp_fx_supported(m, 1)) ? "factor-exchange" : (fused ? "one-pass" : "sharded"),
                         sizeof(float) * bhg_mlp_fx_slab_floats(m), bhg_mlp_fx_ws_bytes(m, 8));
  BHG_REQUIRE(n > 0 && (size_t)n < buf_bytes, "output buffer too small");
  return BHG_OK;
}

#ifdef BHG_STAMPS
static unsigned long long* g_stamps_dev = nullptr;
int bhg_debug_stamps_enable(int on) {
  const size_t bytes = sizeof(unsigned long long) * bhg::kStampKernels * bhg::kStampBlocks * bhg::kStampSlots;
  if (on && !g_stamps_dev) {
    BHG_HIP_CHECK(hipMalloc(&g_stamps_dev, bytes));
  }
  if (g_stamps_dev) BHG_HIP_CHECK(hipMemset(g_stamps_dev, 0, bytes));
  unsigned long long* p = on ? g_stamps_dev : nullptr;
  BHG_HIP_CHECK(hipMemcpyToSymbol(HIP_SYMBOL(bhg::d_stamps), &p, sizeof(p)));
  return BHG_OK;
}
int bhg_debug_stamps_read(unsigned long long* host, size_t count) {
  BHG_REQUIRE(g_stamps_dev && host, "stamps are not enabled");
  const size_t total = (size_t)bhg::kStampKernels * bhg::kStampBlocks * bhg::kStampSlots;
  BHG_HIP_CHECK(hipDeviceSynchronize());
  BHG_HIP_CHECK(hipMemcpy(host, g_stamps_dev, sizeof(unsigned long long) * (count < total ? count : total), hipMemcpyDeviceToHost));
  return BHG_OK;
}
#endif

}

#ifndef BHG_LAYOUT_PAD
#define BHG_LAYOUT_PAD 8
#endif
namespace bhg {
namespace {
#define BHG_STR2(x) #x
#define BHG_STR(x) BHG_STR2(x)
__global__ __attribute__((aligned(16384))) void k_layout_anchor() {
#if BHG_LAYOUT_PAD > 0
  asm volatile(".rept " BHG_STR(BHG_LAYOUT_PAD) " * 64 - 8\n s_nop 0\n .endr");
#endif
}
}
}
```

### betty_amd/csrc/bhg_mwn.hip

```cpp
#include "bhg_common.hpp"

namespace bhg {
namespace {

constexpr int kMwnMaxH = 2048;
constexpr int kMwnChunk = 1024;

__device__ __forceinline__ float mwn_sigmoid(float z) { return 1.f / (1.f + expf(-z)); }

__global__ __launch_bounds__(kThreads) void k_mwn_forward(const float* __restrict__ ce, int B, const float* __restrict__ w1,
                                                          const float* __restrict__ b1, const float* __restrict__ w2,
                                                          const float* __restrict__ b2, int H, float* __restrict__ s,
                                                          float* __restrict__ sd) {
  extern __shared__ float sp[];
  for (int j = threadIdx.x; j < H; j += kThreads) { sp[j] = w1[j]; sp[H + j] = b1[j]; sp[2 * H + j] = w2[j]; }
  __syncthreads();
  const int i = blockIdx.x * kThreads + threadIdx.x;
  if (i >= B) return;
  const float c = ce[i];
  float z = b2[0];
  for (int j = 0; j < H; ++j) {
    const float a = fmaf(sp[j], c, sp[H + j]);
    z = fmaf(sp[2 * H + j], a > 0.f ? a : 0.f, z);
  }
  const float v = mwn_sigmoid(z);
  if (s) s[i] = v;
  if (sd) sd[i] = v / (float)B;
}

__global__ __launch_bounds__(kThreads) void k_mwn_backward(const float* __restrict__ ce, const float* __restrict__ coeff, int B,
                                                           const float* __restrict__ w1, const float* __restrict__ b1,
                                                           const float* __restrict__ w2, const float* __restrict__ b2, int H,
                                                           float scale, float* __restrict__ gw1, float* __restrict__ gb1,
                                                           float* __restrict__ gw2, float* __restrict__ gb2) {
  extern __shared__ float sp[];
  __shared__ float red[kWaves];
  float* sdz = sp + 3 * H;
  float* sce = sdz + kMwnChunk;
  for (int j = threadIdx.x; j < H; j += kThreads) { sp[j] = w1[j]; sp[H + j] = b1[j]; sp[2 * H + j] = w2[j]; }
  const float bias2 = b2[0];
  constexpr int kPer = kMwnMaxH / kThreads;
  float a_w1[kPer], a_b1[kPer], a_w2[kPer];
#pragma unroll
  for (int u = 0; u < kPer; ++u) a_w1[u] = a_b1[u] = a_w2[u] = 0.f;
  float a_b2 = 0.f;
  constexpr int kSPer = kMwnChunk / kThreads;
  float c_pre[kSPer], k_pre[kSPer];
#pragma unroll
  for (int u = 0; u < kSPer; ++u) {
    const int t = threadIdx.x + kThreads * u;
    c_pre[u] = ce[t < B ? t : 0];
    k_pre[u] = coeff[t < B ? t : 0];
  }
  __syncthreads();
  for (int i0 = 0; i0 < B; i0 += kMwnChunk) {
    const int n = B - i0 < kMwnChunk ? B - i0 : kMwnChunk;
#pragma unroll
    for (int u = 0; u < kSPer; ++u) {
      const int t = threadIdx.x + kThreads * u;
      if (t >= n) continue;
      const float c = i0 == 0 ? c_pre[u] : ce[i0 + t];
      const float kc = i0 == 0 ? k_pre[u] : coeff[i0 + t];
      float z = bias2;
      for (int j = 0; j < H; ++j) {
        const float a = fmaf(sp[j], c, sp[H + j]);
        z = fmaf(sp[2 * H + j], a > 0.f ? a : 0.f, z);
      }
      const float v = mwn_sigmoid(z);
      const float dz = kc * (v * (1.f - v));
      sdz[t] = dz;
      sce[t] = c;
      a_b2 += dz;
    }
    __syncthreads();
#pragma unroll
    for (int u = 0; u < kPer; ++u) {
      const int j = threadIdx.x + kThreads * u;
      if (j < H) {
        const float wj = sp[j], bj = sp[H + j], vj = sp[2 * H + j];
        for (int t = 0; t < n; ++t) {
          const float c = sce[t], dz = sdz[t];
          const float a = fmaf(wj, c, bj);
          const bool on = a > 0.f;
          a_w2[u] = fmaf(dz, on ? a : 0.f, a_w2[u]);
          const float g1 = on ? dz * vj : 0.f;
          a_b1[u] += g1;
          a_w1[u] = fmaf(g1, c, a_w1[u]);
        }
      }
    }
    __syncthreads();
  }
#pragma unroll
  for (int u = 0; u < kPer; ++u) {
    const int j = threadIdx.x + kThreads * u;
    if (j < H) { gw1[j] = scale * a_w1[u]; gb1[j] = scale * a_b1[u]; gw2[j] = scale * a_w2[u]; }
  }
#pragma unroll
  for (int off = 32; off > 0; off >>= 1) a_b2 += __shfl_down(a_b2, off, 64);
  if ((threadIdx.x & 63) == 0) red[threadIdx.x >> 6] = a_b2;
  __syncthreads();
  if (threadIdx.x == 0) gb2[0] = scale * ((red[0] + red[1]) + (red[2] + red[3]));
}

int check_mwn(const float* ce, int B, const float* w1, const float* b1, const float* w2, const float* b2, int H) {
  BHG_REQUIRE(ce && w1 && b1 && w2 && b2, "NULL argument");
  BHG_REQUIRE(B >= 1 && H >= 1 && H <= kMwnMaxH, "the closed-form meta-weight-net takes 1 <= hidden width <= 2048");
  return BHG_OK;
}

}
}

using namespace bhg;

extern "C" {

int bhg_mwn_max_hidden(void) { return kMwnMaxH; }

int bhg_mwn_forward(const float* ce, int B, const float* w1, const float* b1, const float* w2, const float* b2, int H, float* s,
                    float* sd, void* stream) {
  if (int rc = check_mwn(ce, B, w1, b1, w2, b2, H)) return rc;
  BHG_REQUIRE(s || sd, "no output requested");
  hipLaunchKernelGGL(k_mwn_forward, dim3((B + kThreads - 1) / kThreads), dim3(kThreads), sizeof(float) * 3 * (size_t)H,
                     static_cast<hipStream_t>(stream), ce, B, w1, b1, w2, b2, H, s, sd);
  BHG_HIP_CHECK(hipGetLastError());
  return BHG_OK;
}

int bhg_mwn_backward(const float* ce, const float* coeff, int B, const float* w1, const float* b1, const float* w2, const float* b2,
                     int H, float scale, float* gw1, float* gb1, float* gw2, float* gb2, void* stream) {
  if (int rc = check_mwn(ce, B, w1, b1, w2, b2, H)) return rc;
  BHG_REQUIRE(coeff && gw1 && gb1 && gw2 && gb2, "NULL argument");
  hipLaunchKernelGGL(k_mwn_backward, dim3(1), dim3(kThreads), sizeof(float) * (3 * (size_t)H + 2 * kMwnChunk),
                     static_cast<hipStream_t>(stream), ce, coeff, B, w1, b1, w2, b2, H, scale, gw1, gb1, gw2, gb2);
  BHG_HIP_CHECK(hipGetLastError());
  return BHG_OK;
}

}
```

### betty_amd/hypergradient/_mlp_hip.py

```python
from __future__ import annotations

import ctypes
import weakref

import torch

from .. import _native

TILE_M = 128

_BUFFERS = weakref.WeakKeyDictionary()



class _Buffers:

    def __init__(self, dims, BP, device, lib):
        L = len(dims) - 1
        self.BP = BP
        self.dims, self.L = dims, L
        z = lambda *shape: torch.zeros(*shape, dtype=torch.float32, device=device)
        self.h = [z(BP, dims[l]) for l in range(L)]
        self.mask = [z(BP, dims[l + 1]) for l in range(L - 1)]
        self.delta = [z(BP, dims[l + 1]) for l in range(L)]
        self.prob = z(BP, dims[L])
        self.sd = z(BP)
        self.ce = z(BP)
        self.coeff = z(BP)
        self.labels = torch.zeros(BP, dtype=torch.int64, device=device)
        self.Rh = [z(BP, dims[l + 1]) for l in range(L - 1)]
        self.Rd = [z(BP, dims[l + 1]) for l in range(L)]
        d = _native.Mlp()
        d.L, d.Bp = L, BP
        for i, v in enumerate(dims):
            d.dims[i] = v
        for l in range(L):
            d.h[l] = self.h[l].data_ptr()
            d.delta[l] = self.delta[l].data_ptr()
            d.Rd[l] = self.Rd[l].data_ptr()
            if l + 1 < L:
                d.mask[l] = self.mask[l].data_ptr()
                d.Rh[l] = self.Rh[l].data_ptr()
        d.prob, d.sd = self.prob.data_ptr(), self.sd.data_ptr()
        d.ridge2 = 0.0
        d.B = 1
        n_part = int(lib.bhg_mlp_partial_floats(ctypes.byref(d)))
        self.partial = torch.empty(max(n_part, 1), dtype=torch.float32, device=device)
        d.partial, d.partial_floats = self.partial.data_ptr(), n_part
        self.desc = d
        self.out = None
        self.native_prepare = bool(lib.bhg_mlp_supports_native_prepare(ctypes.byref(d)))


def _stream() -> int:
    return int(torch.cuda.current_stream().cuda_stream)


def _native_weight_net(lib, wn, upper, device):
    if wn is None:
        return None
    slots = wn.slots(list(upper))
    ts = [t.detach() for t in wn.tensors()]
    if (slots is None or ts[0].shape[0] > int(lib.bhg_mwn_max_hidden())
            or not all(t.is_cuda and t.device == device and t.dtype == torch.float32 and t.is_contiguous() for t in ts)):
        return None
    return ts, slots


def _flat_upper(upper, slots, device):
    sizes = [p.numel() for p in upper]
    flat = torch.empty(sum(sizes), dtype=torch.float32, device=device)
    views, off = [], 0
    for p, n in zip(upper, sizes):
        views.append(flat[off: off + n].view(p.shape))
        off += n
    return flat, views, [views[i] for i in slots]


class FusedSolve:

    __slots__ = ("kind", "alpha", "K", "layout", "v_last", "materialised", "projected")

    def __init__(self, kind, alpha, K, layout, v_last=None, materialised=True, projected=0):
        self.kind, self.alpha, self.K, self.layout, self.v_last, self.materialised = kind, alpha, K, layout, v_last, materialised
        self.projected = projected

    def __bool__(self):
        return True


class HipMLPState:
    def __init__(self, spec, x, y):
        if not x.is_cuda:
            raise _native.NativeLibraryError("WeightedCEMLP(impl='hip') needs CUDA/HIP tensors; there is no CPU fallback")
        self.lib = lib = _native.load()
        self.spec = spec
        Ws = [lin.weight.detach() for lin in spec.layers]
        bs = [lin.bias.detach() for lin in spec.layers]
        L, B = len(Ws), x.shape[0]
        BP = (B + TILE_M - 1) // TILE_M * TILE_M
        if L > _native.BHG_MLP_MAX_LAYERS:
            raise ValueError("too many layers")
        for t in Ws + bs:
            if t.dtype != torch.float32 or not t.is_contiguous() or t.data_ptr() % 16 != 0:
                raise ValueError("weights and biases must be contiguous, 16-byte aligned fp32 tensors")
        dims = tuple([Ws[0].shape[1]] + [W.shape[0] for W in Ws])
        key = (dims, BP, str(x.device))
        owner = _BUFFERS.setdefault(spec.layers[0], {})
        buf = owner.get(key)
        if buf is None:
            buf = owner[key] = _Buffers(dims, BP, x.device, lib)
        self.buf, self.B, self.L, self.Ws = buf, B, L, Ws
        d = buf.desc
        d.B = B
        for l in range(L):
            d.W[l] = Ws[l].data_ptr()
        self.desc = d
        if getattr(buf, "last_B", B) > B:
            buf.h[0][B:].zero_()
        buf.last_B = B
        xs, ys = x.detach().reshape(B, -1), y.detach().reshape(-1)
        same_dev = (xs.device == buf.h[0].device and ys.device == xs.device and xs.is_cuda
                    and torch.cuda.current_device() == (xs.device.index if xs.device.index is not None else torch.cuda.current_device()))
        if (same_dev and xs.dtype == torch.float32 and xs.is_contiguous() and xs.data_ptr() % 16 == 0 and dims[0] % 4 == 0
                and ys.dtype == torch.int64 and ys.is_contiguous()):
            _native.check(lib.bhg_mlp_stage_batch(ctypes.byref(d), xs.data_ptr(), ys.data_ptr(), buf.labels.data_ptr(), _stream()),
                          "bhg_mlp_stage_batch")
        else:
            buf.h[0][:B].copy_(xs.to(torch.float32))
            buf.labels[:B].copy_(ys)

        d.prepacked = 0
        self.packed_prepare = bool(buf.native_prepare and lib.bhg_mlp_supports_packed_prepare(ctypes.byref(d)))
        if self.packed_prepare:
            fws = self._fused_ws(x.device)
            bias_tab, self._bias_keep = _native.ptr_array([b.data_ptr() for b in bs])
            _native.check(lib.bhg_mlp_forward_packed(ctypes.byref(d), bias_tab, buf.labels.data_ptr(), buf.ce.data_ptr(), fws.data_ptr(),
                                                     fws.numel(), _stream()), "bhg_mlp_forward_packed")
            ce = buf.ce[:B]
        elif buf.native_prepare:
            bias_tab, self._bias_keep = _native.ptr_array([b.data_ptr() for b in bs])
            _native.check(lib.bhg_mlp_forward(ctypes.byref(d), bias_tab, buf.labels.data_ptr(), buf.ce.data_ptr(), _stream()),
                          "bhg_mlp_forward")
            ce = buf.ce[:B]
        else:
            raise _native.NativeLibraryError("bhg_mlp_supports_native_prepare refused this network (layer count / batch padding): there is no ATen path")
        native = _native_weight_net(lib, spec.weight_net, spec.prev.trainable_parameters(), x.device)
        self.native_upper, self.sample_weight = native is not None, None
        if self.native_upper:
            self._wn, self._upper_slots = native
            ts = self._wn
            _native.check(lib.bhg_mwn_forward(buf.ce.data_ptr(), B, ts[0].data_ptr(), ts[1].data_ptr(), ts[2].data_ptr(), ts[3].data_ptr(),
                                              ts[0].shape[0], None, buf.sd.data_ptr(), _stream()), "bhg_mwn_forward")
        else:
            self.sample_weight = spec.weight_fn(ce.detach().clone())
            buf.sd[:B].copy_(self.sample_weight.detach().reshape(-1).to(torch.float32) / B)
        if self.packed_prepare:
            _native.check(lib.bhg_mlp_backward_packed(ctypes.byref(d), buf.labels.data_ptr(), buf.fws.data_ptr(), buf.fws.numel(), _stream()),
                          "bhg_mlp_backward_packed")
            d.prepacked = 1
        else:
            _native.check(lib.bhg_mlp_backward(ctypes.byref(d), buf.labels.data_ptr(), _stream()), "bhg_mlp_backward")
        if buf.out is None:
            buf.out = []
            for lin in spec.layers:
                buf.out += [torch.empty_like(lin.weight), torch.empty_like(lin.bias)]
            buf.out_tab, buf.out_keep = _native.ptr_array([t.data_ptr() for t in buf.out])
        self.out = buf.out
        self._out_tab = buf.out_tab

    def upper_vjp(self, coeff, upper, scale: float = 1.0, retain_graph: bool = False, with_flat: bool = False):
        if not self.native_upper:
            sw = self.sample_weight
            out = list(torch.autograd.grad(sw, upper, grad_outputs=coeff.reshape(sw.shape), retain_graph=retain_graph, allow_unused=retain_graph))
            return (out, None) if with_flat else out
        ts, B = self._wn, self.B
        H = ts[0].shape[0]
        flat, views, g = _flat_upper(upper, self._upper_slots, ts[0].device)
        coeff = coeff if (coeff.dtype == torch.float32 and coeff.is_contiguous()) else coeff.to(torch.float32).contiguous()
        _native.check(
            self.lib.bhg_mwn_backward(self.buf.ce.data_ptr(), coeff.data_ptr(), B, ts[0].data_ptr(), ts[1].data_ptr(), ts[2].data_ptr(),
                                      ts[3].data_ptr(), H, float(scale), g[0].data_ptr(), g[1].data_ptr(), g[2].data_ptr(),
                                      g[3].data_ptr(), _stream()), "bhg_mwn_backward")
        return (views, flat) if with_flat else views

    @staticmethod
    def _dir_table(direction_views):
        dirs = []
        for t in direction_views:
            if not (t.is_cuda and t.dtype == torch.float32 and t.is_contiguous() and t.data_ptr() % 16 == 0):
                t = t.detach().to(torch.float32).contiguous().clone()
            dirs.append(t)
        tab, keep = _native.ptr_array([t.data_ptr() for t in dirs])
        return tab, (dirs, keep)

    def hvp(self, direction_views):
        self._solve = None
        key = tuple(map(id, direction_views))
        cached = getattr(self, "_dir_cache", None)
        if cached is None or cached[0] != key:
            tab, keep = self._dir_table(direction_views)
            cached = (key, tab, keep, list(direction_views))
            self._dir_cache = cached if all(a is b for a, b in zip(keep[0], direction_views)) else None
        mode = 3 if getattr(getattr(self.spec.curr, "config", None), "type", None) == "neumann" else 0
        _native.check(self.lib.bhg_mlp_hvp_mode(ctypes.byref(self.desc), cached[1], self._out_tab, mode, _stream()), "bhg_mlp_hvp_mode")
        return self.out

    def fused_supported(self, layout) -> bool:
        if not self.lib.bhg_mlp_supports_fused_solve(ctypes.byref(self.desc)):
            return False
        want = []
        for W in self.Ws:
            want += [W.numel(), W.shape[0]]
        return tuple(want) == tuple(layout.numels) and str(layout.device) == str(self.Ws[0].device)

    def _fused_ws(self, device):
        buf = self.buf
        if getattr(buf, "fws", None) is None:
            n = int(self.lib.bhg_mlp_fused_ws_bytes(ctypes.byref(self.desc)))
            buf.fws = torch.zeros(max(n, 256), dtype=torch.uint8, device=device)
            addr = self.lib.bhg_mlp_timeout_flag_dev(ctypes.byref(self.desc), buf.fws.data_ptr())
            if addr:
                off = int(addr) - buf.fws.data_ptr()
                buf.fws_flag = buf.fws[off: off + 4].view(torch.int32)
                from ..backend import get_backend

                get_backend().watch_fused_workspace(buf.fws_flag)
        return buf.fws

    def _fused_args(self, layout):
        fws = self._fused_ws(layout.device)
        starts = (ctypes.c_int64 * len(layout.starts))(*layout.starts)
        return fws, starts

    def cg_state_mask(self):
        mask = int(self.lib.bhg_mlp_cg_state_mask(ctypes.byref(self.desc), 0))
        return None if mask == (1 << 64) - 1 else mask

    def cg_solve(self, layout, x, r, p, K: int, cg_alpha: float, shift: float, keep_x: bool = True, rhs=None) -> FusedSolve:
        fws, starts = self._fused_args(layout)
        rhs_tab, _rhs_keep = (None, None) if rhs is None else _native.ptr_array([t.data_ptr() for t in rhs])
        _native.check(
            self.lib.bhg_mlp_cg_solve_rhs(ctypes.byref(self.desc), x.data_ptr() if keep_x else None, r.data_ptr(), p.data_ptr(), starts,
                                          layout.chunks_dev.data_ptr(), layout.n_chunks, int(K), float(cg_alpha), float(shift),
                                          layout.workspace.data_ptr(), fws.data_ptr(), fws.numel(), rhs_tab, _stream()),
            "bhg_mlp_cg_solve_rhs",
        )
        self._rhs_keep = (rhs, _rhs_keep)
        self._solve = FusedSolve("cg", float(cg_alpha), int(K), layout, materialised=keep_x)
        return self._solve

    solution_free = True

    def cg_global_phase(self, layout, x, r, p, k: int, K: int, phase: int, world: int, php, cg_alpha: float, shift: float,
                        keep_x: bool = True) -> None:
        fws, starts = self._fused_args(layout)
        if k == 0 and phase == _native.BHG_CG_GLOBAL_CHAIN:
            self._solve = None
        _native.check(
            self.lib.bhg_mlp_cg_global_phase(ctypes.byref(self.desc), x.data_ptr() if keep_x else None, r.data_ptr(), p.data_ptr(),
                                             starts, layout.chunks_dev.data_ptr(), layout.n_chunks, int(k), int(K), int(phase),
                                             int(world), php.data_ptr(), float(cg_alpha), float(shift),
                                             layout.workspace.data_ptr(), fws.data_ptr(), fws.numel(), _stream()),
            "bhg_mlp_cg_global_phase",
        )

    def cg_global_finish(self, layout, K: int, cg_alpha: float, keep_x: bool = True) -> FusedSolve:
        self._solve = FusedSolve("cg", float(cg_alpha), int(K), layout, materialised=keep_x)
        return self._solve

    def fx_supported(self, layout, world: int) -> bool:
        return bool(self.fused_supported(layout) and self.lib.bhg_mlp_fx_supported(ctypes.byref(self.desc), int(world)))

    def fx_buffers(self, world: int):
        buf = self.buf
        held = getattr(buf, "fx", None)
        if held is None:
            held = buf.fx = {}
        got = held.get(world)
        if got is None:
            d, lib, dev = ctypes.byref(self.desc), self.lib, buf.h[0].device
            z = lambda n, dt: torch.zeros(int(n), dtype=dt, device=dev)
            got = held[world] = {
                "const": z(world * lib.bhg_mlp_fx_const_floats(d), torch.float32).view(world, -1),
                "slab": z(world * lib.bhg_mlp_fx_slab_floats(d), torch.float32).view(world, -1),
                "scal": z(world * lib.bhg_mlp_fx_scal_doubles(d), torch.float64).view(world, -1),
                "xws": z(max(int(lib.bhg_mlp_fx_ws_bytes(d, world)), 256), torch.uint8),
            }
        return got

    def _fx_phase(self, symbol: str, rhs, k: int, K: int, phase: int, world: int, rank: int, alpha: float, shift: float) -> None:
        b = self.fx_buffers(world)
        fws = self._fused_ws(self.buf.h[0].device)
        if phase == _native.BHG_CG_FX_BEGIN:
            self._solve = None
            self._fx_rhs = _native.ptr_array([t.data_ptr() for t in rhs]) + (list(rhs),)
        _native.check(
            getattr(self.lib, symbol)(ctypes.byref(self.desc), self._fx_rhs[0], int(k), int(K), int(phase), int(world), int(rank),
                                      b["const"].data_ptr(), b["slab"].data_ptr(), b["scal"].data_ptr(), float(alpha), float(shift),
                                      fws.data_ptr(), fws.numel(), b["xws"].data_ptr(), b["xws"].numel(), _stream()),
            symbol,
        )

    def cg_fx_phase(self, rhs, k: int, K: int, phase: int, world: int, rank: int, cg_alpha: float, shift: float) -> None:
        self._fx_phase("bhg_mlp_cg_fx_phase", rhs, k, K, phase, world, rank, cg_alpha, shift)

    def neumann_fx_phase(self, rhs, k: int, K: int, phase: int, world: int, rank: int, alpha: float, shift: float) -> None:
        self._fx_phase("bhg_mlp_neumann_fx_phase", rhs, k, K, phase, world, rank, alpha, shift)

    def neumann_fx_finish(self, layout, K: int, alpha: float) -> FusedSolve:
        self._solve = FusedSolve("neumann", float(alpha), int(K), layout, v_last=None, materialised=False, projected=1)
        return self._solve

    def cg_fx_finish(self, layout, K: int, cg_alpha: float) -> FusedSolve:
        self._solve = FusedSolve("cg", float(cg_alpha), int(K), layout, materialised=False)
        return self._solve

    def neumann_solve(self, layout, v0, v1, p, K: int, alpha: float, shift: float, keep_p: bool = True) -> FusedSolve:
        fws, starts = self._fused_args(layout)
        projected = ctypes.c_int(0)
        _native.check(
            self.lib.bhg_mlp_neumann_solve(ctypes.byref(self.desc), v0.data_ptr(), v1.data_ptr(), p.data_ptr() if keep_p else None,
                                           starts, int(K), float(alpha), float(shift), fws.data_ptr(), fws.numel(), ctypes.byref(projected),
                                           _stream()),
            "bhg_mlp_neumann_solve",
        )
        self._solve = FusedSolve("neumann", float(alpha), int(K), layout, v_last=v0 if K % 2 == 0 else v1, materialised=keep_p)
        self._solve.projected = int(projected.value)
        return self._solve

    def mixed_coeff(self, dir_views, solve: FusedSolve = None):
        buf = self.buf
        if solve is not None and solve is not getattr(self, "_solve", None):
            raise RuntimeError("stale fused-solve token: another solve or a hand-driven HVP has reused this state's workspace")
        if solve is not None and solve.kind == "neumann" and not solve.materialised:
            lay, v_last = solve.layout, solve.v_last
            if v_last is None:
                tab, _keep = None, None
            else:
                views = [v_last[s: s + n] for s, n in zip(lay.starts, lay.numels)]
                tab, _keep = self._dir_table(views)
            _native.check(
                self.lib.bhg_mlp_neumann_mixed_coeff(ctypes.byref(self.desc), tab, buf.labels.data_ptr(), buf.coeff.data_ptr(),
                                                     solve.alpha, solve.K, int(getattr(solve, "projected", 0)), buf.fws.data_ptr(),
                                                     buf.fws.numel(), _stream()),
                "bhg_mlp_neumann_mixed_coeff",
            )
        elif solve is not None and solve.kind == "cg":
            _native.check(
                self.lib.bhg_mlp_cg_mixed_coeff(ctypes.byref(self.desc), buf.labels.data_ptr(), buf.coeff.data_ptr(), solve.alpha,
                                                buf.fws.data_ptr(), buf.fws.numel(), _stream()),
                "bhg_mlp_cg_mixed_coeff",
            )
        else:
            tab, _keep = self._dir_table(dir_views)
            _native.check(
                self.lib.bhg_mlp_mixed_coeff(ctypes.byref(self.desc), tab, buf.labels.data_ptr(), buf.coeff.data_ptr(), _stream()),
                "bhg_mlp_mixed_coeff",
            )
        coeff = buf.coeff[:self.B]
        return coeff if self.native_upper else coeff.clone()


PAD_WIDTHS_TO_32 = True
_TWINS = weakref.WeakKeyDictionary()


def _pad32(n: int) -> int:
    return (int(n) + 31) // 32 * 32


def padded_dims(dims):
    return tuple(_pad32(d) for d in dims[:-1]) + (int(dims[-1]),)


class _TwinLayer:

    __slots__ = ("weight", "bias", "__weakref__")

    def __init__(self, out_f, in_f, device):
        self.weight = torch.zeros(out_f, in_f, dtype=torch.float32, device=device)
        self.bias = torch.zeros(out_f, dtype=torch.float32, device=device)


class _Twin:
    def __init__(self, dims, pdims, device):
        self.layers = [_TwinLayer(pdims[l + 1], pdims[l], device) for l in range(len(dims) - 1)]
        self.x = None
        self.dirs = [t for lay in self.layers for t in (torch.zeros_like(lay.weight), torch.zeros_like(lay.bias))]
        self.rhs = [torch.zeros_like(t) for t in self.dirs]


def _copy2d(lib, dst, ldd, src, lds, rows, cols):
    _native.check(lib.bhg_copy2d(dst.data_ptr(), int(ldd), src.data_ptr(), int(lds), int(rows), int(cols), _stream()), "bhg_copy2d")


class _TwinSpec:

    def __init__(self, spec, twin):
        self._spec, self.layers = spec, twin.layers

    def __getattr__(self, name):
        return getattr(self._spec, name)


class PaddedHipMLPState:

    solution_free = True

    def __init__(self, spec, x, y):
        if not x.is_cuda:
            raise _native.NativeLibraryError("WeightedCEMLP(impl='hip') needs CUDA/HIP tensors; there is no CPU fallback")
        self.lib = lib = _native.load()
        self.spec = spec
        real = [lin for lin in spec.layers]
        self.real_Ws = [lin.weight.detach() for lin in real]
        self.real_bs = [lin.bias.detach() for lin in real]
        for t in self.real_Ws + self.real_bs:
            if t.dtype != torch.float32 or not t.is_contiguous():
                raise ValueError("weights and biases must be contiguous fp32 tensors")
        dims = tuple([self.real_Ws[0].shape[1]] + [W.shape[0] for W in self.real_Ws])
        self.dims, self.pdims = dims, padded_dims(dims)
        self.shapes = [s for W in self.real_Ws for s in ((W.shape[0], W.shape[1]), (1, W.shape[0]))]
        self.pcols = [c for l in range(len(dims) - 1) for c in (self.pdims[l], self.pdims[l + 1])]
        owner = _TWINS.setdefault(spec.layers[0], {})
        key = (self.pdims, str(x.device))
        twin = owner.get(key)
        if twin is None:
            twin = owner[key] = _Twin(dims, self.pdims, x.device)
        self.twin = twin
        for l, (W, b) in enumerate(zip(self.real_Ws, self.real_bs)):
            _copy2d(lib, twin.layers[l].weight, self.pdims[l], W, dims[l], W.shape[0], W.shape[1])
            _copy2d(lib, twin.layers[l].bias, self.pdims[l + 1], b, dims[l + 1], 1, b.shape[0])
        B = x.shape[0]
        xs = x.detach().reshape(B, -1)
        xs = xs if (xs.dtype == torch.float32 and xs.is_contiguous()) else xs.to(torch.float32).contiguous()
        if twin.x is None or twin.x.shape[0] != B:
            twin.x = torch.zeros(B, self.pdims[0], dtype=torch.float32, device=x.device)
        _copy2d(lib, twin.x, self.pdims[0], xs, dims[0], B, dims[0])
        self.inner = HipMLPState(_TwinSpec(spec, twin), twin.x, y)
        self.B = B
        self.out = None

    @property
    def native_upper(self):
        return self.inner.native_upper

    @property
    def sample_weight(self):
        return self.inner.sample_weight

    def upper_vjp(self, *a, **k):
        return self.inner.upper_vjp(*a, **k)

    def _pad(self, tensors, into):
        for t, dst, (rows, cols), ldd in zip(tensors, into, self.shapes, self.pcols):
            if not (t.is_cuda and t.dtype == torch.float32 and t.is_contiguous()):
                t = t.detach().to(torch.float32).contiguous()
            _copy2d(self.lib, dst, ldd, t, cols, rows, cols)
        return into

    def _unpad(self, padded, into):
        for src, t, (rows, cols), lds in zip(padded, into, self.shapes, self.pcols):
            _copy2d(self.lib, t, cols, src, lds, rows, cols)
        return into

    def _real_views(self, layout, flat):
        like = [t for W, b in zip(self.real_Ws, self.real_bs) for t in (W, b)]
        return layout.views(flat, like)

    def _twin_layout(self):
        from ..backend import get_backend

        return get_backend().layout(self.twin.dirs)

    def hvp(self, direction_views):
        out_p = self.inner.hvp(self._pad(direction_views, self.twin.dirs))
        if self.out is None:
            self.out = [torch.empty_like(t) for W, b in zip(self.real_Ws, self.real_bs) for t in (W, b)]
        return self._unpad(out_p, self.out)

    def fused_supported(self, layout) -> bool:
        want = [n for W in self.real_Ws for n in (W.numel(), W.shape[0])]
        return (tuple(want) == tuple(layout.numels) and str(layout.device) == str(self.real_Ws[0].device)
                and self.inner.fused_supported(self._twin_layout()))

    def cg_solve(self, layout, x, r, p, K: int, cg_alpha: float, shift: float, keep_x: bool = True, rhs=None) -> FusedSolve:
        from ..backend import get_backend

        be, play = get_backend(), self._twin_layout()
        self._pad(self._real_views(layout, r), self.twin.rhs)
        px, pr, pp = play.state(3)
        skip_x = not keep_x
        mask = self.inner.cg_state_mask() if skip_x else None
        ts = be.cg_init(play, self.twin.rhs, None if skip_x else px, pr, pp, keep_mask=mask) if mask is not None else \
            be.cg_init(play, self.twin.rhs, None if skip_x else px, pr, pp)
        token = self.inner.cg_solve(play, px, pr, pp, K, cg_alpha, shift, keep_x=keep_x, rhs=ts if mask is not None else None)
        if keep_x:
            self._unpad(play.views(px, self.twin.dirs), self._real_views(layout, x))
        return token

    def neumann_solve(self, layout, v0, v1, p, K: int, alpha: float, shift: float, keep_p: bool = True) -> FusedSolve:
        from ..backend import get_backend

        be, play = get_backend(), self._twin_layout()
        self._pad(self._real_views(layout, v0), self.twin.rhs)
        pv0, pv1, pp = play.state(3)
        be.neumann_init(play, self.twin.rhs, pv0, pp if keep_p else None)
        token = self.inner.neumann_solve(play, pv0, pv1, pp, K, alpha, shift, keep_p=keep_p)
        self._twin_p = (token, play, pp) if keep_p else None
        if keep_p:
            self._unpad(play.views(pp, self.twin.dirs), self._real_views(layout, p))
        return token

    def mixed_coeff(self, dir_views, solve: FusedSolve = None):
        if solve is not None:
            held = getattr(self, "_twin_p", None)
            if solve.kind == "neumann" and solve.materialised and held is not None and held[0] is solve:
                return self.inner.mixed_coeff(held[1].views(held[2], self.twin.dirs), solve)
            return self.inner.mixed_coeff(None, solve)
        return self.inner.mixed_coeff(self._pad(dir_views, self.twin.dirs))


def make_state(spec, x, y):
    Ws = [lin.weight for lin in spec.layers]
    dims = tuple([Ws[0].shape[1]] + [W.shape[0] for W in Ws])
    if (PAD_WIDTHS_TO_32 and spec.pad_widths and len(Ws) >= 3 and dims[-1] <= 256 and padded_dims(dims) != dims and x.is_cuda):
        return PaddedHipMLPState(spec, x, y)
    return HipMLPState(spec, x, y)


_FD_WS = weakref.WeakKeyDictionary()


def fd_hop(spec, vector, eps32, two_eps, x, y, upper, sync: bool, restore: bool):
    lib = _native.load()
    params = [t for lin in spec.layers for t in (lin.weight, lin.bias)]
    L, B = len(spec.layers), int(x.shape[0])
    dims = [spec.layers[0].weight.shape[1]] + [lin.weight.shape[0] for lin in spec.layers]
    dims_c = (ctypes.c_int * len(dims))(*dims)
    dev = params[0].device
    xs = x.detach().reshape(B, -1)
    xs = xs if (xs.dtype == torch.float32 and xs.is_contiguous()) else xs.to(torch.float32).contiguous()
    ys = y.detach().reshape(-1).to(device=dev, dtype=torch.int64).contiguous()
    dirs = [v if (v.dtype == torch.float32 and v.is_contiguous()) else v.detach().to(torch.float32).contiguous() for v in vector]
    owner = _FD_WS.setdefault(spec.layers[0], {})
    key = (tuple(dims), B, str(dev))
    ws = owner.get(key)
    if ws is None:
        n = int(lib.bhg_mlp_fd_ws_bytes(dims_c, L, B))
        if n <= 0:
            raise _native.NativeLibraryError(f"bhg_mlp_fd_ws_bytes refused widths {dims} at batch {B}")
        ws = owner[key] = torch.empty(n, dtype=torch.uint8, device=dev)
    ce = torch.empty(2, B, dtype=torch.float32, device=dev)
    eps = eps32 if (eps32.dtype == torch.float32 and eps32.device == dev) else eps32.to(device=dev, dtype=torch.float32)
    ptab, _pk = _native.ptr_array([p.data.data_ptr() for p in params])
    dtab, _dk = _native.ptr_array([d.data_ptr() for d in dirs])
    _native.check(lib.bhg_mlp_fd_forward(xs.data_ptr(), ys.data_ptr(), B, dims_c, L, ptab, dtab, eps.data_ptr(), int(restore),
                                         ce[0].data_ptr(), ce[1].data_ptr(), ws.data_ptr(), ws.numel(), _stream()), "bhg_mlp_fd_forward")
    native = _native_weight_net(lib, spec.weight_net, upper, dev)
    if native is None:
        return spec.fd_upper_autograd(ce[0], ce[1], two_eps, upper, sync)
    ts, slots = native
    if sync:
        for p in upper:
            if p.grad is None:
                p.grad = torch.zeros_like(p, memory_format=torch.contiguous_format)
            elif not (p.grad.dtype == torch.float32 and p.grad.is_contiguous()):
                p.grad = p.grad.to(torch.float32).contiguous()
        outs = [p.grad for p in upper]
        g = [outs[i] for i in slots]
    else:
        _flat, outs, g = _flat_upper(upper, slots, dev)
    _native.check(lib.bhg_mwn_fd_vjp(ce[0].data_ptr(), ce[1].data_ptr(), B, ts[0].data_ptr(), ts[1].data_ptr(), ts[2].data_ptr(),
                                     ts[3].data_ptr(), ts[0].shape[0], two_eps.data_ptr(), int(sync), g[0].data_ptr(), g[1].data_ptr(),
                                     g[2].data_ptr(), g[3].data_ptr(), _stream()), "bhg_mwn_fd_vjp")
    return None if sync else outs
```

### betty_amd/hypergradient/structured.py

```python
from __future__ import annotations

from typing import Callable, List, Optional, Sequence

import math
import warnings

import torch
import torch.nn.functional as F

from ._common import _uses_ddp, is_fsdp, precision_of


class StructureMismatchError(RuntimeError):
    """The declared closed form does not describe the problem's actual ``training_step``."""


VERIFY_STRUCTURE = True
VERIFY_RTOL = 1e-3
VERIFY_KINK_MARGIN = 1e-6
VERIFY_RTOL_ON_A_KINK = 3e-2
VERIFY_KINK_RETRIES = 3


AUTO_STRUCTURE = False
# ... 116 lines not shown
        self.curr, self.prev = curr, prev
        self.weight_net = weight_net
        self.verify = bool(verify)
        self.layers = list(layers)
        self.weight_fn = weight_fn
        self.ridge = float(ridge)
        self.hvp_shift = 2.0 * self.ridge
        self.batch = batch
        self.impl = impl
        self.fused = bool(fused)
        self.keep_solution = bool(keep_solution)
        self.pad_widths, self.expects_data_parallel_mean = True, False
        params = list(curr.parameters())
        expect = []
        for lin in self.layers:
            expect += [lin.weight, lin.bias]
        if len(params) != len(expect) or any(a is not b for a, b in zip(params, expect)):
            raise ValueError("WeightedCEMLP: curr.parameters() must be [W1, b1, W2, b2, ...] of `layers`")

    def prepare(self):
        x, y = self.batch if self.batch is not None else self.curr.cur_batch
        impl = self.impl or "hip"
        if impl == "hip":
            from ._mlp_hip import make_state

            self._state = make_state(self, x, y)
        elif impl == "torch":
            from ._mlp_torch import _TorchMLPState

            self._state = _TorchMLPState(self, x, y)
        else:
            raise ValueError(f"unknown impl {impl!r}")
        if self.verify and VERIFY_STRUCTURE:
            self._verify_against_autograd(x, y)
        return self._state.hvp

    def _autograd_second_order(self, params, upper):
        gen = torch.Generator(device="cpu").manual_seed(20240926)
        direction = [torch.randn(p.shape, generator=gen).to(device=p.device, dtype=p.dtype) for p in params]
        devs = [params[0].device] if params and params[0].is_cuda else []
        with torch.random.fork_rng(devices=devs), torch.enable_grad():
            loss = self.curr.training_step_exec(self.batch if self.batch is not None else self.curr.cur_batch)
            grads = torch.autograd.grad(loss, params, create_graph=True)
            dot = sum((g * d).sum() for g, d in zip(grads, direction))
            second = torch.autograd.grad(dot, params + upper, allow_unused=True)
        return direction, second[:len(params)], second[len(params):]

    def _estimate_ridge(self) -> float:
        params = list(self.curr.parameters())
        direction, hv_auto, _ = self._autograd_second_order(params, list(self.prev.trainable_parameters()))
        hv0 = [h.detach().clone() for h in self._state.hvp(direction)]
        num = sum(float(((a.double() - b.double()) * d.double()).sum()) for a, b, d in zip(hv_auto, hv0, direction))
        den = sum(float((d.double() ** 2).sum()) for d in direction)
        c = num / den
        res = sum(float(((a.double() - b.double() - c * d.double()) ** 2).sum()) for a, b, d in zip(hv_auto, hv0, direction)) ** 0.5
        ref = sum(float((a.double() ** 2).sum()) for a in hv_auto) ** 0.5
        if c <= 0.0 or res > VERIFY_RTOL * max(ref, 1e-300) or c * den ** 0.5 <= 1e-5 * ref:
            return 0.0
        rho = 0.5 * c
        for digits in range(1, 7):
            r = round(rho, digits)
            if r > 0 and abs(r - rho) <= 2e-4 * rho:
                return float(r)
        return float(rho)

    def _verify_against_autograd(self, x, y):
        params = list(self.curr.parameters())
        key = (tuple(tuple(p.shape) for p in params), int(x.shape[0]), self.ridge, type(self._state).__name__)
        done = self.curr.__dict__.setdefault("_bhg_structure_verified", set()) if hasattr(self.curr, "__dict__") else set()
        if key in done:
            return
        upper = list(self.prev.trainable_parameters())
        direction, hv_auto, mixed_auto = self._autograd_second_order(params, upper)
        hv = [h.detach().clone() + self.hvp_shift * d for h, d in zip(self._state.hvp(direction), direction)]
        coeff = self._state.mixed_coeff(direction)
        mixed = self._state.upper_vjp(coeff, upper, retain_graph=True)
        mixed = [torch.zeros_like(p) if g is None else g for g, p in zip(mixed, upper)]

        def rel(got, want):
            num = sum(float(((a.double() - (b.double() if b is not None else 0.0)) ** 2).sum()) for a, b in zip(got, want)) ** 0.5
            den = sum(float((b.double() ** 2).sum()) for b in want if b is not None) ** 0.5
            return num / den if den > 0 else num

        e_hvp, e_mix = rel(hv, hv_auto), rel(mixed, mixed_auto)
        tol, relaxed = VERIFY_RTOL, False
        if precision_of(self.curr) in ("fp16", "bf16"):
            tol = max(tol, 5e-2)
        if not (e_hvp <= tol and e_mix <= tol):
            with torch.no_grad():
                h, margin = x.detach().reshape(x.shape[0], -1).to(self.layers[0].weight.dtype), float("inf")
                for lin in self.layers[:-1]:
                    a = torch.addmm(lin.bias, h, lin.weight.t())
                    margin = min(margin, float(a.abs().min() / a.abs().mean().clamp_min(1e-30)))
                    h = torch.relu(a)
            if margin < VERIFY_KINK_MARGIN:
                tol = VERIFY_RTOL_ON_A_KINK
                relaxed = True
        bad = not (e_hvp <= tol and e_mix <= tol)
        import torch.distributed as dist

        if dist.is_available() and dist.is_initialized() and dist.get_world_size() > 1:
            flag = torch.tensor([1.0 if bad else 0.0, 1.0 if relaxed else 0.0], device=params[0].device if dist.get_backend() == "nccl" else "cpu")
            dist.all_reduce(flag, op=dist.ReduceOp.MAX)
            bad, relaxed = bool(flag[0].item() > 0), bool(flag[1].item() > 0)
        if bad:
            raise StructureMismatchError(
                f"hypergradient_structure of problem {getattr(self.curr, 'name', '?')!r} declares {type(self).__name__}, but its "
                f"training_step disagrees with that closed form on a random direction: Hessian-vector product off by {e_hvp:.2e}, "
                f"mixed second derivative by {e_mix:.2e} (tolerance {tol:g}).  Typical causes: label smoothing, dropout, a "
                f"reduction other than the batch mean, a ridge that is not `ridge * sum(w^2)`, layers missing from `layers`.")
        if relaxed:
            tries = self.curr.__dict__.setdefault("_bhg_structure_relaxed", {}) if hasattr(self.curr, "__dict__") else {}
            tries[key] = tries.get(key, 0) + 1
            final = tries[key] >= VERIFY_KINK_RETRIES
            if tries[key] == 1 or final:
                warnings.warn(
                    f"betty_amd: structure check of problem {getattr(self.curr, 'name', '?')!r} passed only under the ReLU-kink tolerance "
                    f"({tol:g}; Hessian-vector product off by {e_hvp:.2e}, mixed second derivative by {e_mix:.2e}: some hidden "
                    "pre-activation of this batch sits within 1e-6 of zero) — " +
                    (f"accepted after {tries[key]} such batches" if final else "not cached, the next batch is checked again"),
                    RuntimeWarning, stacklevel=3)
            if not final:
                return
        done.add(key)

    def _fused_ready(self, K: int, layout, *methods: str, world: Optional[int] = None, skips_solution: bool = False) -> bool:
        st = self._state
        if not (K > 0 and self.fused) or (skips_solution and self.keep_solution):
            return False
        for m in methods:
            if not hasattr(st, m):
                return False
        return bool(st.fused_supported(layout) if world is None else st.fx_supported(layout, world))

    def fused_cg_ready(self, layout, K: int) -> bool:
        return self._fused_ready(K, layout, "cg_solve")

    def fused_cg_skips_solution(self, layout, K: int) -> bool:
        return self._fused_ready(K, layout, "cg_solve", skips_solution=True)

    def fused_cg_state_mask(self, layout, K: int):
        if not self._fused_ready(K, layout, "cg_solve", "cg_state_mask", skips_solution=True):
            return None
        return self._state.cg_state_mask()

    def fused_cg(self, layout, x, r, p, K: int, cg_alpha: float, rhs=None):
        if not self.fused_cg_ready(layout, K):
            return False
        return self._state.cg_solve(layout, x, r, p, K, cg_alpha, self.hvp_shift, keep_x=self.keep_solution, rhs=rhs)

    def fused_cg_global_ready(self, layout, K: int) -> bool:
        return self._fused_ready(K, layout, "cg_global_phase")

    def fused_cg_global_skips_solution(self, layout, K: int) -> bool:
        return self._fused_ready(K, layout, "cg_global_phase", skips_solution=True) and self._state.solution_free

    def cg_global_phase(self, layout, x, r, p, k: int, K: int, phase: int, world: int, php, cg_alpha: float) -> None:
        keep = not self.fused_cg_global_skips_solution(layout, K)
        self._state.cg_global_phase(layout, x, r, p, k, K, phase, world, php, cg_alpha, self.hvp_shift, keep_x=keep)

    def cg_global_finish(self, layout, K: int, cg_alpha: float):
        keep = not self.fused_cg_global_skips_solution(layout, K)
        return self._state.cg_global_finish(layout, K, cg_alpha, keep_x=keep)

    def fused_cg_fx_ready(self, layout, K: int, world: int) -> bool:
        return self._fused_ready(K, layout, "cg_fx_phase", world=world, skips_solution=True)

    def fused_neumann_fx_ready(self, layout, K: int, world: int) -> bool:
        return self._fused_ready(K, layout, "neumann_fx_phase", world=world, skips_solution=True)

    def fx_buffers(self, world: int):
        return self._state.fx_buffers(world)

    def local_batch_size(self) -> int:
        return self._state.B

    def _fx(self, method: str, *args):
        return getattr(self._state, method)(*args)

    def cg_fx_phase(self, rhs, k: int, K: int, phase: int, world: int, rank: int, cg_alpha: float) -> None:
        self._fx("cg_fx_phase", rhs, k, K, phase, world, rank, cg_alpha, self.hvp_shift)

    def cg_fx_finish(self, layout, K: int, cg_alpha: float):
        return self._fx("cg_fx_finish", layout, K, cg_alpha)

    def neumann_fx_phase(self, rhs, k: int, K: int, phase: int, world: int, rank: int, alpha: float) -> None:
        self._fx("neumann_fx_phase", rhs, k, K, phase, world, rank, alpha, self.hvp_shift)

    def neumann_fx_finish(self, layout, K: int, alpha: float):
        return self._fx("neumann_fx_finish", layout, K, alpha)

    def fused_neumann_ready(self, layout, K: int) -> bool:
        return self._fused_ready(K, layout, "neumann_solve")

    def fused_neumann_skips_solution(self, layout, K: int) -> bool:
        return self._fused_ready(K, layout, "neumann_solve", skips_solution=True)

    def fused_neumann(self, layout, v, p, K: int, alpha: float):
        if not self.fused_neumann_ready(layout, K):
            return False
        v_alt = next(t for t in layout.state(3) if t is not v and t is not p)
        return self._state.neumann_solve(layout, v, v_alt, p, K, alpha, self.hvp_shift, keep_p=self.keep_solution)

    def _fd_applies(self, layout, vector):
        curr, prev = self.curr, self.prev
        if is_fsdp(curr):
            return "fsdp"
        if precision_of(curr) != "fp32":
            return "autocast"
        params = list(curr.parameters())
        if (why := _fd_parameters_blocker(curr, params, layout, vector)) is not None:
            return why
        if _uses_ddp(prev):
            return "ddp"
        import torch.distributed as dist

        if dist.is_available() and dist.is_initialized() and dist.get_world_size() > 1:
            return "multi-rank"
        wn = self.weight_net
        if wn is not None and (wn.average_over is not None or wn.slots(list(prev.trainable_parameters())) is None):
            return "upper parameters"
        x, y = self.batch if self.batch is not None else curr.cur_batch
        if not (torch.is_tensor(x) and torch.is_tensor(y)):
            return "batch"
        tensors = params + list(vector) + [x]
        if (self.impl or "hip") == "hip":
            if not all(t.is_cuda and t.dtype == torch.float32 and t.device == params[0].device for t in tensors):
                return "not fp32 cuda"
            if not all(p.is_contiguous() for p in params) or not (1 <= x.shape[0] <= 512):
                return "shape"
        elif not all(t.dtype == torch.float32 for t in tensors):
            return "not fp32"
        return None

    def _fd_guard(self, x):
        if not (self.verify and VERIFY_STRUCTURE):
            return
        params = list(self.curr.parameters())
        head = (tuple(tuple(p.shape) for p in params), int(x.shape[0]), self.ridge)
        done = self.curr.__dict__.get("_bhg_structure_verified", set()) if hasattr(self.curr, "__dict__") else set()
        if any(k[:3] == head for k in done):
            return
        self.prepare()

    def finite_difference(self, layout, vector, eps32, eps64, sync: bool, restore: bool = True):
        vector = list(vector)
        if self._fd_applies(layout, vector) is not None:
            return NotImplemented
        x, y = self.batch if self.batch is not None else self.curr.cur_batch
        self._fd_guard(x)
        two_eps = (2.0 * eps64).to(torch.float32)
        upper = list(self.prev.trainable_parameters())
        if (self.impl or "hip") == "hip":
            from ._mlp_hip import fd_hop

            return fd_hop(self, vector, eps32, two_eps, x, y, upper, bool(sync), bool(restore))
        from ..backend import get_backend

        be = get_backend()
        weights = [p.data for p in self.curr.parameters()]
        with torch.no_grad():
            be.axpy_multi(layout, weights, vector, eps32, 1.0)
            ce_p = self._torch_ce(x, y)
            be.axpy_multi(layout, weights, vector, eps32, -2.0)
            ce_m = self._torch_ce(x, y)
            if restore:
                be.axpy_multi(layout, weights, vector, eps32, 1.0)
        return self.fd_upper_autograd(ce_p, ce_m, two_eps, upper, bool(sync))

    def _torch_ce(self, x, y):
        h = x.detach().reshape(x.shape[0], -1)
        for l, lin in enumerate(self.layers):
            h = F.linear(h, lin.weight.detach(), lin.bias.detach())
            if l + 1 < len(self.layers):
                h = torch.relu(h)
        return F.cross_entropy(h, y.reshape(-1), reduction="none")

    def fd_upper_autograd(self, ce_p, ce_m, two_eps, upper, sync: bool):
        B = ce_p.shape[0]

        def point(ce, scale=None):
            ce = ce.detach().clone()
            with torch.enable_grad():
                s = self.weight_fn(ce)
            seed = torch.full((), 1.0, dtype=ce.dtype, device=ce.device) if scale is None else 1.0 / scale
            return s, ((seed / B) * ce).reshape(s.shape)

        def zero_fill(gs):
            return [torch.zeros_like(p) if g is None else g for g, p in zip(gs, upper)]

        s_p, c_p = point(ce_p)
        g_p = zero_fill(torch.autograd.grad(s_p, upper, grad_outputs=c_p, allow_unused=True))
        if sync:
            self.prev.set_grads(upper, [-(g / two_eps) for g in g_p])
            s_m, c_m = point(ce_m, two_eps)
            torch.autograd.backward(s_m, grad_tensors=c_m, inputs=upper)
            return None
        s_m, c_m = point(ce_m)
        g_m = zero_fill(torch.autograd.grad(s_m, upper, grad_outputs=c_m, allow_unused=True))
        return [(gn - gp) / two_eps for gn, gp in zip(g_m, g_p)]

    def mixed_vjp(self, neg_x_views, sync: bool, solve=None):
        st = self._state
        coeff = st.mixed_coeff(neg_x_views, solve) if solve is not None else st.mixed_coeff(neg_x_views)
        upper = self.prev.trainable_parameters()
        if st.native_upper:
            wn = self.weight_net
            world, group = 1, None
            if sync:
                import torch.distributed as dist

                if dist.is_available() and dist.is_initialized():
                    from ..distributed import ddp_process_group_of

                    if wn.average_over is not None:
                        group = None if wn.average_over is True else wn.average_over
                        world = dist.get_world_size(group)
                    else:
                        wrapped, group = ddp_process_group_of(getattr(self.prev, "fwd", None), getattr(self.prev, "module", None))
                        if wrapped:
                            world = dist.get_world_size(group)
                        elif dist.get_world_size() > 1 and self.expects_data_parallel_mean:
                            raise RuntimeError(
                                "cg_global(sync=True) with a closed-form weight net: declare SigmoidMLPWeightNet(average_over=True) (or a "
                                "process group) or wrap the upper module in DistributedDataParallel — otherwise every rank would "
                                "accumulate the hypergradient of its own batch share only")
            grads, flat = st.upper_vjp(coeff, upper, scale=1.0 / world, with_flat=True)
            if sync:
                from ..distributed import defer_grad_sync, fence_grads, install_optimizer_fence

                fence_grads()
            if world > 1:
                if wn.overlap and sync:
                    if all(p_.grad is None for p_ in upper):
                        work = dist.all_reduce(flat, op=dist.ReduceOp.SUM, group=group, async_op=True)
                        from ..backend import get_backend

                        defer_grad_sync(work, flat, get_backend())
                        install_optimizer_fence(getattr(self.prev, "optimizer", None))
                    else:
                        dist.all_reduce(flat, op=dist.ReduceOp.SUM, group=group)
                else:
                    dist.all_reduce(flat, op=dist.ReduceOp.SUM, group=group)
            if sync:
                for p_, g_ in zip(upper, grads):
                    p_.grad = g_ if p_.grad is None else p_.grad + g_
                return None
            return grads
        if sync:
            torch.autograd.backward(st.sample_weight, grad_tensors=coeff.reshape(st.sample_weight.shape), inputs=upper)
            return None
        return list(torch.autograd.grad(st.sample_weight, upper, grad_outputs=coeff.reshape(st.sample_weight.shape)))


def _fd_parameters_blocker(curr, params, layout, vector):
    meta = list(curr.meta_trainable_parameters()) if hasattr(curr, "meta_trainable_parameters") else params
    if len(meta) != len(params) or any(a is not b for a, b in zip(meta, params)) or len(vector) != len(params):
        return "parameters"
    if tuple(layout.numels) != tuple(p.numel() for p in params) or any(v.shape != p.shape for v, p in zip(vector, params)):
        return "layout"
    return None


def _forward_has_side_effects(module) -> bool:
    for m in module.modules():
        if not m.training:
            continue
        if isinstance(m, torch.nn.modules.dropout._DropoutNd) or next(m.buffers(recurse=False), None) is not None:
            return True
    return False


def _graph_leaves(t) -> set:
    if t.grad_fn is None:
        return {id(t)} if t.requires_grad else set()
    seen, stack, leaves = set(), [t.grad_fn], set()
    while stack:
        fn = stack.pop()
        if fn is None or fn in seen:
            continue
        seen.add(fn)
        var = getattr(fn, "variable", None)
        if var is not None:
            leaves.add(id(var))
        stack.extend(nxt for nxt, _ in fn.next_functions)
    return leaves


class _QuadraticFD:

    impl: Optional[str] = None
    closed_form_fd: Optional[bool] = None
    _fd_side_effects: Optional[bool] = None

    def _quad_fd_blocker(self, layout, vector):
        curr, prev = self.curr, self.prev
        if self.closed_form_fd is False:
            return "declined"
        if is_fsdp(curr) or is_fsdp(prev):
            return "fsdp"
        if precision_of(curr) != "fp32" or torch.is_autocast_enabled("cuda") or torch.is_autocast_enabled("cpu"):
            return "autocast"
        params = list(curr.parameters())
        if not params:
            return "parameters"
        if (why := _fd_parameters_blocker(curr, params, layout, vector)) is not None:
            return why
        hip = (self.impl or "hip") == "hip"
        for t in [p.data for p in params] + list(vector):
            if t.dtype != torch.float32 or t.device != params[0].device or not t.is_contiguous():
                return "not contiguous fp32"
            if hip and not (t.is_cuda and t.data_ptr() % 16 == 0):
                return "not an aligned cuda tensor"
        if self.closed_form_fd is None:
            if self._fd_side_effects is None:
                module = getattr(curr, "module", None)
                self._fd_side_effects = not isinstance(module, torch.nn.Module) or _forward_has_side_effects(module)
            if self._fd_side_effects:
                return "the forward passes have side effects"
        return None

    def _quad_fd_launch(self, layout, vector, out, eps32, scale: float, mode: int, restore: bool, accumulate: bool):
        from ..backend import get_backend

        be = get_backend()
        weights = [p.data for p in self.curr.parameters()]
        if (self.impl or "hip") == "hip":
            be.quad_fd(layout, weights, vector, out, eps32, scale, mode, restore, accumulate)
            return
        if self.impl != "torch":
            raise ValueError(f"unknown impl {self.impl!r}")
        with torch.no_grad():
            res = [float(scale) * v for v in vector] if mode == 0 else [-(w * v) for w, v in zip(weights, vector)]
            be.axpy_multi(layout, weights, vector, eps32, 1.0)
            be.axpy_multi(layout, weights, vector, eps32, -2.0)
            if restore:
                be.axpy_multi(layout, weights, vector, eps32, 1.0)
            for o, r in zip(out, res):
                o.add_(r) if accumulate else o.copy_(r)


class LogisticRegressionL2(_QuadraticFD):

    def __init__(self, curr, prev, weight: torch.nn.Parameter, lam_fn: Callable, batch=None, impl: Optional[str] = None,
                 closed_form_fd: Optional[bool] = None):
        self.curr, self.prev, self.weight, self.lam_fn, self.batch = curr, prev, weight, lam_fn, batch
        self.impl, self.closed_form_fd = impl, closed_form_fd
        params = list(curr.parameters())
        if len(params) != 1 or params[0] is not weight:
            raise ValueError("LogisticRegressionL2: curr.parameters() must be [weight]")

    def prepare(self):
        from .. import _native

        x, _y = self.batch if self.batch is not None else self.curr.cur_batch
        if not x.is_cuda:
            raise _native.NativeLibraryError("LogisticRegressionL2 needs CUDA/HIP tensors; there is no CPU fallback")
        self.lib = _native.load()
        self.X = x.detach().to(torch.float32).contiguous()
        n, d = self.X.shape
        self.n, self.d = n, d
        self.lam = self.lam_fn()
        self.lam_d = self.lam.detach().to(torch.float32).contiguous()
        self.w = self.weight.detach().to(torch.float32).contiguous()
        self.s = torch.empty(n, device=x.device)
        self.tmp = torch.empty(int(self.lib.bhg_logreg_tmp_floats(n, d)), device=x.device)
        self.out = torch.empty(d, device=x.device)
        self._stream = lambda: int(torch.cuda.current_stream().cuda_stream)
        _native.check(self.lib.bhg_logreg_prepare(self.X.data_ptr(), self.w.data_ptr(), self.s.data_ptr(), n, d, self._stream()),
                      "bhg_logreg_prepare")
        self._native = _native
        return self.hvp

    def hvp(self, direction_views):
        (p,) = direction_views
        p = p.detach().to(torch.float32).contiguous()
        self._native.check(
            self.lib.bhg_logreg_hvp(self.X.data_ptr(), self.s.data_ptr(), self.lam_d.data_ptr(), p.data_ptr(),
                                    self.out.data_ptr(), self.tmp.data_ptr(), self.n, self.d, self._stream()),
            "bhg_logreg_hvp",
        )
        return [self.out.view(self.weight.shape)]

    def mixed_vjp(self, neg_x_views, sync: bool):
        coeff = (self.w * neg_x_views[0].reshape(-1)).reshape(self.lam.shape)
        upper = self.prev.trainable_parameters()
        if sync:
            torch.autograd.backward(self.lam, grad_tensors=coeff, inputs=upper)
            return None
        return list(torch.autograd.grad(self.lam, upper, grad_outputs=coeff))

    def finite_difference(self, layout, vector, eps32, eps64, sync: bool, restore: bool = True):
        vector = list(vector)
        if self._quad_fd_blocker(layout, vector) is not None:
            return NotImplemented
        upper = list(self.prev.trainable_parameters())
        lam = self.lam_fn()
        if not torch.is_tensor(lam) or lam.dtype != torch.float32 or lam.numel() != self.weight.numel() or lam.device != self.weight.device:
            return NotImplemented
        leaves = _graph_leaves(lam)
        if not upper or any(id(p) not in leaves for p in upper):
            return NotImplemented
        coeff = torch.empty_like(self.weight.data)
        self._quad_fd_launch(layout, vector, [coeff], eps32, 0.0, 1, bool(restore), False)
        coeff = coeff.reshape(lam.shape)
        if sync:
            torch.autograd.backward(lam, grad_tensors=coeff, inputs=upper)
            return None
        return list(torch.autograd.grad(lam, upper, grad_outputs=coeff))


class ProximalRegularized(_QuadraticFD):

    hvp_is_autograd = True

    def __init__(self, curr, prev, data_loss: Callable, reg: float, batch=None, impl: Optional[str] = None,
                 closed_form_fd: Optional[bool] = None):
        self.curr, self.prev, self.data_loss, self.reg, self.batch = curr, prev, data_loss, float(reg), batch
        self.impl, self.closed_form_fd = impl, closed_form_fd
        self.hvp_shift = 2.0 * self.reg
        inner, upper = list(curr.parameters()), list(prev.trainable_parameters())
        if len(inner) != len(upper) or any(a.shape != b.shape for a, b in zip(inner, upper)):
            raise ValueError("ProximalRegularized: upper and inner parameters must match one-to-one")

    def prepare(self):
        import warnings

        batch = self.batch if self.batch is not None else self.curr.cur_batch
        loss = self.data_loss(batch)
        with warnings.catch_warnings():
            warnings.simplefilter("ignore")
            self._in_grad = torch.autograd.grad(loss, self.curr.trainable_parameters(), create_graph=True)
        params = list(self.curr.parameters())

        def hvp(direction_views):
            return torch.autograd.grad(self._in_grad, params, grad_outputs=direction_views, retain_graph=True)

        return hvp

    def first_order_loss(self):
        return lambda: self.data_loss(self.batch if self.batch is not None else self.curr.cur_batch)

    def mixed_vjp(self, neg_x_views, sync: bool):
        self._in_grad = None
        grads = [(-2.0 * self.reg) * t for t in neg_x_views]
        if sync:
            torch.autograd.backward(list(self.prev.trainable_parameters()), grad_tensors=grads)
            return None
        return grads

    def finite_difference(self, layout, vector, eps32, eps64, sync: bool, restore: bool = True):
        vector = list(vector)
        if self._quad_fd_blocker(layout, vector) is not None:
            return NotImplemented
        upper = list(self.prev.trainable_parameters())
        if len(upper) != len(vector) or any(
                p.shape != v.shape or p.dtype != torch.float32 or p.device != v.device for p, v in zip(upper, vector)):
            return NotImplemented
        if not math.isfinite(self.reg):
            return NotImplemented
        scale = 2.0 * self.reg
        if sync:
            grads = [p.grad for p in upper]
            hip = (self.impl or "hip") == "hip"
            if not _uses_ddp(self.prev) and all(g is not None and g.dtype == torch.float32 and g.shape == p.shape and g.device == p.device
                               and g.is_contiguous() and (not hip or g.data_ptr() % 16 == 0) for g, p in zip(grads, upper)):
                self._quad_fd_launch(layout, vector, grads, eps32, scale, 0, bool(restore), True)
                return None
        out = layout.views(torch.empty(layout.flat_size, dtype=torch.float32, device=vector[0].device), vector)
        self._quad_fd_launch(layout, vector, out, eps32, scale, 0, bool(restore), False)
        if sync:
            torch.autograd.backward(upper, grad_tensors=out)
            return None
        return out
```

### include/bhg.h

```cpp
#ifndef BHG_H_
#define BHG_H_

#include <stddef.h>
#include <stdint.h>

#ifdef __cplusplus
extern "C" {
#endif

#define BHG_VERSION 1
#define BHG_CHUNK_ELEMS 4096
#define BHG_FLAT_ALIGN 64

#define BHG_OK 0
#define BHG_ERR_ARG (-1)
#define BHG_ERR_HIP (-2)
#define BHG_ERR_WS (-3)
#define BHG_ERR_CAPACITY (-4)

typedef struct bhg_chunk {
  int64_t flat_off;
  int64_t src_off;
  int32_t tensor;
  int32_t len;
} bhg_chunk;

int bhg_version(void);
const char* bhg_last_error(void);

int64_t bhg_layout_flat_size(const int64_t* numel, int T);
int64_t bhg_layout_num_chunks(const int64_t* numel, int T);
int bhg_layout_build(const int64_t* numel, int T, int64_t* starts, bhg_chunk* chunks);
size_t bhg_workspace_bytes(int T);

int bhg_flatten(const void* const* src, int T, const bhg_chunk* chunks_dev, int n_chunks,
                float* flat, float scale, void* ws, void* stream);
int bhg_scatter(const float* flat, void* const* dst, int T, const bhg_chunk* chunks_dev,
                int n_chunks, float scale, void* ws, void* stream);

int bhg_neumann_init(const void* const* vec, int T, const bhg_chunk* chunks_dev, int n_chunks,
                     float* v, float* p, void* ws, void* stream);
int bhg_neumann_step(const void* const* hvp, int T, const bhg_chunk* chunks_dev, int n_chunks,
                     float* v, float* p, float alpha, float out_scale, float hvp_shift, void* ws,
                     void* stream);

#define BHG_CG_AUTO 0
#define BHG_CG_STREAM 1
#define BHG_CG_RESIDENT 2
int bhg_cg_init(const void* const* vec, int T, const bhg_chunk* chunks_dev, int n_chunks,
                float* x, float* r, float* p, void* ws, void* stream);
int bhg_cg_init_masked(const void* const* vec, int T, const bhg_chunk* chunks_dev, int n_chunks,
                       float* x, float* r, float* p, unsigned long long keep_mask, void* ws, void* stream);
int bhg_cg_step(const void* const* hvp, int T, const bhg_chunk* chunks_dev, int n_chunks,
                float* x, float* r, float* p, float cg_alpha, int iter, float out_scale,
                float hvp_shift , int variant,
                void* ws, void* stream);
int bhg_cg_resident_capacity_chunks(void);
int bhg_cg_resident_ok(void);
int bhg_cg_resident_usable(int n_chunks);
const double* bhg_cg_scalars_dev(const void* ws);
const unsigned* bhg_cg_timeout_flag_dev(const void* ws);

int bhg_cg_phase(int phase, const void* const* hvp, int T, const bhg_chunk* chunks_dev, int n_chunks, float* x,
                 float* r, float* p, float cg_alpha, int iter, float out_scale, float hvp_shift, void* ws, void* stream);
double* bhg_cg_partials_dev(void* ws, int which, int iter);
int bhg_cg_partials_count(void);

int bhg_scale_flat(float* flat, int64_t n, float scale, void* stream);

int bhg_darts_eps(const void* const* vec, int T, const bhg_chunk* chunks_dev, int n_chunks,
                  double R, double* out_dev, float* eps_f32_dev, void* ws, void* stream);
int bhg_axpy_multi(void* const* dst, const void* const* src, int T, const bhg_chunk* chunks_dev,
                   int n_chunks, const float* coef_dev, float mul, void* ws, void* stream);

int bhg_fd_perturb(void* const* w, const float* w0_flat, const void* const* dir, int T, const bhg_chunk* chunks_dev,
                   int n_chunks, const float* eps_dev, float sign, void* ws, void* stream);
int bhg_cg_step_fd(const void* const* grad_plus, const void* const* grad_minus, const float* two_eps_dev, int T,
                   const bhg_chunk* chunks_dev, int n_chunks, float* x, float* r, float* p, float cg_alpha, int iter,
                   float out_scale, float hvp_shift, int variant, void* ws, void* stream);
int bhg_neumann_step_fd(const void* const* grad_plus, const void* const* grad_minus, const float* two_eps_dev, int T,
                        const bhg_chunk* chunks_dev, int n_chunks, float* v, float* p, float alpha, float out_scale,
                        float hvp_shift, void* ws, void* stream);

int bhg_sama_adam_precondition(const void* const* vec, const void* const* last_grad,
                               const void* const* exp_avg, const void* const* exp_avg_sq, int T,
                               const bhg_chunk* chunks_dev, int n_chunks, float* out_flat,
                               double beta1, double beta2, double eps, double lr, void* ws, void* stream);

int bhg_debug_set(const char* key, int value);
int bhg_debug_unset(const char* key);
void bhg_debug_reset(void);
int bhg_debug_key_count(void);
const char* bhg_debug_key_name(int i);
int bhg_is_ab_build(void);

#define BHG_TIMING_CG_STEP 0
#define BHG_TIMING_NEUMANN_STEP 1
#define BHG_TIMING_MLP_HVP 2
#define BHG_TIMING_MLP_CG_ITER 3
int bhg_timing_enable(int on);
int bhg_timing_read(int kind, double* total_ms, int* launches);

int bhg_logreg_prepare(const float* X, const float* w, float* s, int n, int d, void* stream);
size_t bhg_logreg_tmp_floats(int n, int d);
int bhg_logreg_hvp(const float* X, const float* s, const float* lam, const float* p, float* out,
                   float* tmp, int n, int d, void* stream);

#define BHG_MLP_MAX_LAYERS 32
typedef struct bhg_mlp {
  int32_t L, B, Bp;
  int32_t dims[BHG_MLP_MAX_LAYERS + 1];
  const float* W[BHG_MLP_MAX_LAYERS];
  const float* h[BHG_MLP_MAX_LAYERS];
  const float* mask[BHG_MLP_MAX_LAYERS];
  const float* delta[BHG_MLP_MAX_LAYERS];
  const float* prob;
  const float* sd;
  float* Rh[BHG_MLP_MAX_LAYERS];
  float* Rd[BHG_MLP_MAX_LAYERS];
  float* partial;
  size_t partial_floats;
  float ridge2;
  int32_t prepacked;
} bhg_mlp;
size_t bhg_mlp_partial_floats(const bhg_mlp* m);
int bhg_mlp_hvp(const bhg_mlp* m, const void* const* dir, void* const* out, void* stream);
int bhg_mlp_hvp_mode(const bhg_mlp* m, const void* const* dir, void* const* out, int gemm_mode, void* stream);

int bhg_mlp_supports_native_prepare(const bhg_mlp* m);
int bhg_mlp_forward(const bhg_mlp* m, const void* const* bias, const int64_t* labels, float* ce, void* stream);
int bhg_mlp_backward(const bhg_mlp* m, const int64_t* labels, void* stream);
int bhg_mlp_mixed_coeff(const bhg_mlp* m, const void* const* dir, const int64_t* labels, float* coeff, void* stream);

int bhg_mlp_supports_fused_solve(const bhg_mlp* m);
size_t bhg_mlp_fused_ws_bytes(const bhg_mlp* m);
int bhg_mlp_cg_solve(const bhg_mlp* m, float* x, float* r, float* p, const int64_t* starts,
                     const bhg_chunk* chunks_dev, int n_chunks, int K, float cg_alpha, float hvp_shift, void* ws,
                     void* fws, size_t fws_bytes, void* stream);
int bhg_mlp_neumann_solve(const bhg_mlp* m, float* v0, float* v1, float* p, const int64_t* starts, int K,
                          float alpha, float hvp_shift, void* fws, size_t fws_bytes, int* projected_out, void* stream);
#define BHG_CG_GLOBAL_CHAIN 0
#define BHG_CG_GLOBAL_UPDATE 1
#define BHG_CG_GLOBAL_DOTS 2
int bhg_mlp_cg_global_phase(const bhg_mlp* m, float* x, float* r, float* p, const int64_t* starts, const bhg_chunk* chunks_dev,
                            int n_chunks, int k, int K, int phase, int world, double* php, float cg_alpha, float hvp_shift,
                            void* ws, void* fws, size_t fws_bytes, void* stream);
#define BHG_CG_FX_BEGIN 0
#define BHG_CG_FX_CHAIN 1
#define BHG_CG_FX_GRAM 2
#define BHG_CG_FX_END 3
int bhg_mlp_fx_supported(const bhg_mlp* m, int world);
size_t bhg_mlp_fx_ws_bytes(const bhg_mlp* m, int world);
size_t bhg_mlp_fx_const_floats(const bhg_mlp* m);
size_t bhg_mlp_fx_slab_floats(const bhg_mlp* m);
size_t bhg_mlp_fx_scal_doubles(const bhg_mlp* m);
int bhg_mlp_cg_fx_phase(const bhg_mlp* m, const void* const* rhs, int k, int K, int phase, int world, int rank, float* const_all,
                        float* slab_all, double* scal_all, float cg_alpha, float hvp_shift, void* fws, size_t fws_bytes, void* xws,
                        size_t xws_bytes, void* stream);
int bhg_mlp_neumann_fx_phase(const bhg_mlp* m, const void* const* rhs, int k, int K, int phase, int world, int rank, float* const_all,
                             float* slab_all, double* scal_all, float alpha, float hvp_shift, void* fws, size_t fws_bytes, void* xws,
                             size_t xws_bytes, void* stream);
unsigned long long bhg_mlp_cg_state_mask(const bhg_mlp* m, int has_x);
int bhg_mlp_cg_solve_rhs(const bhg_mlp* m, float* x, float* r, float* p, const int64_t* starts, const bhg_chunk* chunks_dev,
                         int n_chunks, int K, float cg_alpha, float hvp_shift, void* ws, void* fws, size_t fws_bytes,
                         const void* const* rhs, void* stream);
int bhg_mlp_cg_mixed_coeff(const bhg_mlp* m, const int64_t* labels, float* coeff, float cg_alpha, void* fws,
                           size_t fws_bytes, void* stream);
int64_t bhg_mlp_wsk_launches(void);
int64_t bhg_mlp_hoist_launches(void);
int64_t bhg_mlp_proj_iterations(void);
int64_t bhg_mlp_lin_launches(void);
int bhg_mlp_neumann_mixed_coeff(const bhg_mlp* m, const void* const* v_last, const int64_t* labels, float* coeff,
                                float alpha, int K, int projected, void* fws, size_t fws_bytes, void* stream);

int bhg_mlp_stage_batch(const bhg_mlp* m, const float* x, const int64_t* y, int64_t* labels, void* stream);
int bhg_mlp_supports_packed_prepare(const bhg_mlp* m);
int bhg_mlp_forward_packed(const bhg_mlp* m, const void* const* bias, const int64_t* labels, float* ce, void* fws, size_t fws_bytes,
                           void* stream);
int bhg_mlp_backward_packed(const bhg_mlp* m, const int64_t* labels, void* fws, size_t fws_bytes, void* stream);

void* bhg_mlp_timeout_flag_dev(const bhg_mlp* m, void* fws);

int bhg_mwn_max_hidden(void);
int bhg_mwn_forward(const float* ce, int B, const float* w1, const float* b1, const float* w2, const float* b2, int H, float* s,
                    float* sd, void* stream);
int bhg_mwn_backward(const float* ce, const float* coeff, int B, const float* w1, const float* b1, const float* w2, const float* b2,
                     int H, float scale, float* gw1, float* gb1, float* gw2, float* gb2, void* stream);

int bhg_mlp_plan_describe(const bhg_mlp* m, int algo, int keep_solution, char* buf, size_t buf_bytes);

int bhg_copy2d(float* dst, int64_t ldd, const float* src, int64_t lds, int64_t rows, int64_t cols, void* stream);

size_t bhg_bn_ws_bytes(int C);
int bhg_bn_backward_vjp(const float* x, const float* gy, const float* a, const float* gamma, const float* mean, const float* invstd,
                        const float* b, const float* c, int N, int C, int HW, float* dx, float* dgy, float* dgamma, void* ws,
                        size_t ws_bytes, void* stream);

size_t bhg_mlp_fd_ws_bytes(const int* dims, int L, int B);
int bhg_mlp_fd_forward(const float* x, const int64_t* labels, int B, const int* dims, int L, void* const* params, const void* const* dir,
                       const float* eps_dev, int restore, float* ce_plus, float* ce_minus, void* ws, size_t ws_bytes, void* stream);
int bhg_mwn_fd_vjp(const float* ce_plus, const float* ce_minus, int B, const float* w1, const float* b1, const float* w2, const float* b2,
                   int H, const float* two_eps_dev, int accumulate, float* gw1, float* gb1, float* gw2, float* gb2, void* stream);

int bhg_quad_fd(void* const* w, const void* const* dir, void* const* out, int T, const bhg_chunk* chunks_dev, int n_chunks,
                const float* eps_dev, float scale, int mode, int restore, int accumulate, void* stream);

#ifdef __cplusplus
}
#endif
#endif
```

Baseline: 768.9.

## Fuse head forward, weight-net and top backward into step tail; fuse CG coeff with MWN backward

Adds a fused step-tail kernel that combines the classifier head forward, the meta weight-net forward, delta_top and the head backward, replacing several separate launches in the packed prepare path. It also adds a CG hop kernel that computes the mixed coefficients from rzx and runs the weight-net backward in one launch. The goal is to cut kernel-launch count and intermediate global traffic per hypergradient step. The cost is more specialised code paths, gated by class-count and hidden-size limits, that fall back to the old path when unsupported.

```diff
diff --git a/betty_amd/_native.py b/betty_amd/_native.py
--- a/betty_amd/_native.py
+++ b/betty_amd/_native.py
@@ -181,6 +181,18 @@
         c_int,
         [c_void_p, c_void_p, c_int, c_void_p, c_void_p, c_void_p, c_void_p, c_int, c_float, c_void_p, c_void_p, c_void_p, c_void_p, c_void_p],
     ),
+    "bhg_step_supports_prepare": (c_int, [POINTER(Mlp), c_int]),
+    "bhg_step_prepare": (
+        c_int,
+        [POINTER(Mlp), _PP, c_void_p, c_void_p, c_void_p, c_void_p, c_void_p, c_void_p, c_int, c_void_p, c_void_p, c_size_t, c_void_p],
+    ),
+    "bhg_step_supports_cg_hop": (c_int, [POINTER(Mlp), c_int]),
+    "bhg_step_cg_hop": (
+        c_int,
+        [POINTER(Mlp), c_void_p, c_void_p, c_float, c_void_p, c_size_t, c_void_p, c_void_p, c_void_p, c_void_p, c_void_p, c_int, c_float,
+         c_void_p, c_void_p, c_void_p, c_void_p, c_void_p],
+    ),
+    "bhg_step_launches": (c_int64, []),
     "bhg_mlp_neumann_solve": (
         c_int,
         [POINTER(Mlp), c_void_p, c_void_p, c_void_p, POINTER(c_int64), c_int, c_float, c_float, c_void_p, c_size_t, POINTER(c_int), c_void_p],
diff --git a/betty_amd/csrc/bhg_common.hpp b/betty_amd/csrc/bhg_common.hpp
--- a/betty_amd/csrc/bhg_common.hpp
+++ b/betty_amd/csrc/bhg_common.hpp
@@ -36,7 +36,7 @@
   X(mlp_hoist) X(hoist_wgs) X(proj_step_alone) X(mlp_no_side) X(mlp_no_fuse) X(mlp_no_outer_all) X(neumann_side)             \
   X(hoist_staged_mink) X(proj_alpha_alone) X(proj_small_alone) X(outer_order_by_work) X(outer_no_pre) X(outer_stagger)       \
   X(mlp_no_fused_solve) X(cg_eager_p) X(cg_x_every_iter) X(neumann_p_every_iter) X(head_no_prefetch) X(cg_spin_limit)        \
-  X(packed_chain) X(packed_depth) X(packed_gram) X(proj_max_ratio) X(proj_ws_cap_mb) X(alpha_in_hoist) X(graw_v2) X(wskp_ragged) X(pstep_v2) X(pstep_unroll) X(rnew_in_graw) X(graw_cols) X(lin_first) X(lin_prio) X(lin_nub) X(lin_order) X(lin_update_next) X(lin_withhold_beta) X(neumann_vnew) X(cg_rhs_direct) X(packed_prepare) X(lin_deep) X(graw_kloop) X(lin_update_in_head) X(xcd_pairs) X(headu_head_first) X(fx_ksplit)
+  X(packed_chain) X(packed_depth) X(packed_gram) X(proj_max_ratio) X(proj_ws_cap_mb) X(alpha_in_hoist) X(graw_v2) X(wskp_ragged) X(pstep_v2) X(pstep_unroll) X(rnew_in_graw) X(graw_cols) X(lin_first) X(lin_prio) X(lin_nub) X(lin_order) X(lin_update_next) X(lin_withhold_beta) X(neumann_vnew) X(cg_rhs_direct) X(packed_prepare) X(lin_deep) X(graw_kloop) X(lin_update_in_head) X(xcd_pairs) X(headu_head_first) X(fx_ksplit) X(step_tail) X(step_hop)
 enum DbgKey : int {
 #define BHG_DBG_ENUM(n) DBG_##n,
   BHG_DBG_KEYS(BHG_DBG_ENUM)
diff --git a/betty_amd/csrc/bhg_mlp.hip b/betty_amd/csrc/bhg_mlp.hip
--- a/betty_amd/csrc/bhg_mlp.hip
+++ b/betty_amd/csrc/bhg_mlp.hip
@@ -3,6 +3,7 @@
 
 
 #include "bhg_common.hpp"
+#include "bhg_step.hpp"
 
 #ifdef BHG_STAMPS
 namespace bhg { __device__ unsigned long long* d_stamps = nullptr; }
@@ -1871,6 +1872,7 @@
   hipLaunchKernelGGL(k_coeff_from_rzx, dim3((m->Bp + kThreads - 1) / kThreads), dim3(kThreads), 0, static_cast<hipStream_t>(stream),
                      (const double*)w.rzx, m->prob, labels, coeff, m->Bp, m->dims[m->L], m->B, -cg_alpha, 0.f);
   BHG_HIP_CHECK(hipGetLastError());
+  ++g_step_launches;
   return BHG_OK;
 }
 
@@ -2004,6 +2006,9 @@
   return hp.ok && dbg(DBG_packed_chain, 1) != 0 ? 1 : 0;
 }
 
+static int forward_packed_run(const bhg_mlp* m, const void* const* bias, const int64_t* labels, float* ce, const FusedWs& w, hipStream_t st,
+                              bool with_head);
+static int backward_packed_run(const bhg_mlp* m, const int64_t* labels, const FusedWs& w, hipStream_t st, bool with_top);
 int bhg_mlp_forward_packed(const bhg_mlp* m, const void* const* bias, const int64_t* labels, float* ce, void* fws, size_t fws_bytes,
                            void* stream) {
   if (int rc = check_head_problem(m)) return rc;
@@ -2011,11 +2016,16 @@
   BHG_REQUIRE(bias && labels && ce && fws, "NULL argument");
   BHG_REQUIRE(bhg_mlp_supports_packed_prepare(m), "this network does not take the packed form (bhg_mlp_supports_packed_prepare)");
   BHG_REQUIRE(fws_bytes >= bhg_mlp_fused_ws_bytes(m), "fused workspace too small");
-  hipStream_t st = static_cast<hipStream_t>(stream);
-  const int L = m->L, Bp = m->Bp, B = m->B;
   FusedWs w;
   carve_fused_ws(m, fws, &w);
+  return forward_packed_run(m, bias, labels, ce, w, static_cast<hipStream_t>(stream), true);
+}
+
+static int forward_packed_run(const bhg_mlp* m, const void* const* bias, const int64_t* labels, float* ce, const FusedWs& w, hipStream_t st,
+                              bool with_head) {
+  const int L = m->L, Bp = m->Bp, B = m->B;
   if (int rc = pack_operands(m, w, st, true)) return rc;
+  g_step_launches += 3 + (L - 2) + (with_head ? 1 : 0);
   {
     const int K = m->dims[0], N = m->dims[1];
     GemmArgs a{};
@@ -2041,9 +2051,10 @@
     const int blk = q.nfull * (q.RB / 32) + q.nstrip;
     hipLaunchKernelGGL(k_wskpf<2>, dim3(blk), dim3(64 * kWskpWaves), 0, st, f);
   }
-  launch_head_forward(st, Bp, nullptr, m->h[L - 1], m->W[L - 1] , m->W[L - 1], static_cast<const float*>(bias[L - 1]),
-                      nullptr, nullptr, const_cast<float*>(m->prob), m->dims[L - 1], m->dims[L], B, HEAD_LOGITS, labels, ce, nullptr,
-                      nullptr, nullptr);
+  if (with_head)
+    launch_head_forward(st, Bp, nullptr, m->h[L - 1], m->W[L - 1] , m->W[L - 1], static_cast<const float*>(bias[L - 1]),
+                        nullptr, nullptr, const_cast<float*>(m->prob), m->dims[L - 1], m->dims[L], B, HEAD_LOGITS, labels, ce, nullptr,
+                        nullptr, nullptr);
   BHG_HIP_CHECK(hipGetLastError());
   return BHG_OK;
 }
@@ -2054,11 +2065,16 @@
   BHG_REQUIRE(labels && fws, "NULL argument");
   BHG_REQUIRE(bhg_mlp_supports_packed_prepare(m), "this network does not take the packed form (bhg_mlp_supports_packed_prepare)");
   BHG_REQUIRE(fws_bytes >= bhg_mlp_fused_ws_bytes(m), "fused workspace too small");
-  hipStream_t st = static_cast<hipStream_t>(stream);
+  FusedWs w;
+  carve_fused_ws(m, fws, &w);
+  return backward_packed_run(m, labels, w, static_cast<hipStream_t>(stream), true);
+}
+
+static int backward_packed_run(const bhg_mlp* m, const int64_t* labels, const FusedWs& w, hipStream_t st, bool with_top) {
   const int L = m->L, Bp = m->Bp, B = m->B;
   const int C = m->dims[L];
-  FusedWs w;
-  carve_fused_ws(m, fws, &w);
+  g_step_launches += (with_top ? 2 : 0) + (L - 2);
+  if (with_top) {
   hipLaunchKernelGGL(k_delta_top, dim3((Bp * C + 255) / 256), dim3(256), 0, st, m->prob, m->sd, labels,
                      const_cast<float*>(m->delta[L - 1]), Bp, C, B);
   {
@@ -2066,6 +2082,7 @@
     const int blocks = (Bp * (N / 4) + 255) / 256;
     hipLaunchKernelGGL(k_head_backward, dim3(blocks), dim3(256), 0, st, (const float*)nullptr, m->delta[l], m->W[l],
                        (const float*)nullptr, m->mask[l - 1], const_cast<float*>(m->delta[l - 1]), N, K, B, Bp, w.dpk[l - 1]);
+  }
   }
   for (int l = L - 2; l >= 1; --l) {
     WskpBuilder wb;
@@ -2078,6 +2095,55 @@
   }
   BHG_HIP_CHECK(hipGetLastError());
   return BHG_OK;
+}
+
+int bhg_step_supports_prepare(const bhg_mlp* m, int H) {
+  static_assert(kStepMaxClasses == kSmallC, "bhg_step.hip restates the head kernels' class limit");
+  if (!m || H < 1 || H > bhg_mwn_max_hidden() || dbg(DBG_step_tail, 1) == 0) return 0;
+  return bhg_mlp_supports_packed_prepare(m) && narrow_head(m) ? 1 : 0;
+}
+
+int bhg_step_prepare(const bhg_mlp* m, const void* const* bias, const int64_t* labels, float* ce, const float* w1, const float* b1,
+                     const float* w2, const float* b2, int H, float* s, void* fws, size_t fws_bytes, void* stream) {
+  if (int rc = check_head_problem(m)) return rc;
+  BHG_REQUIRE(bias && labels && ce && fws && w1 && b1 && w2 && b2 && m->sd, "NULL argument");
+  BHG_REQUIRE(bhg_step_supports_prepare(m, H), "this network / weight net does not take the fused prepare (bhg_step_supports_prepare)");
+  BHG_REQUIRE(fws_bytes >= bhg_mlp_fused_ws_bytes(m), "fused workspace too small");
+  hipStream_t st = static_cast<hipStream_t>(stream);
+  const int L = m->L;
+  FusedWs w;
+  carve_fused_ws(m, fws, &w);
+  if (int rc = forward_packed_run(m, bias, labels, ce, w, st, false)) return rc;
+  StepTailArgs t{};
+  t.h = m->h[L - 1]; t.W = m->W[L - 1]; t.bias = static_cast<const float*>(bias[L - 1]); t.labels = labels;
+  t.prob = const_cast<float*>(m->prob); t.ce = ce;
+  t.w1 = w1; t.b1 = b1; t.w2 = w2; t.b2 = b2; t.H = H; t.s = s; t.sd = const_cast<float*>(m->sd);
+  t.dtop = const_cast<float*>(m->delta[L - 1]); t.mask = m->mask[L - 2]; t.dprev = const_cast<float*>(m->delta[L - 2]);
+  t.dprev_p = w.dpk[L - 2];
+  t.K = m->dims[L - 1]; t.C = m->dims[L]; t.B = m->B; t.rows = m->Bp;
+  if (int rc = launch_step_tail(t, st)) return rc;
+  return backward_packed_run(m, labels, w, st, false);
+}
+
+int bhg_step_supports_cg_hop(const bhg_mlp* m, int H) {
+  if (!m || H < 1 || H > bhg_mwn_max_hidden() || dbg(DBG_step_hop, 1) == 0) return 0;
+  return bhg_mlp_supports_fused_solve(m) ? 1 : 0;
+}
+
+int bhg_step_cg_hop(const bhg_mlp* m, const int64_t* labels, float* coeff, float cg_alpha, void* fws, size_t fws_bytes, const float* ce,
+                    const float* w1, const float* b1, const float* w2, const float* b2, int H, float scale, float* gw1, float* gb1,
+                    float* gw2, float* gb2, void* stream) {
+  if (int rc = check_mlp(m)) return rc;
+  BHG_REQUIRE(labels && coeff && fws && ce && w1 && b1 && w2 && b2 && gw1 && gb1 && gw2 && gb2, "NULL argument");
+  BHG_REQUIRE(bhg_step_supports_cg_hop(m, H), "this network / weight net does not take the fused hop (bhg_step_supports_cg_hop)");
+  BHG_REQUIRE(fws_bytes >= bhg_mlp_fused_ws_bytes(m), "fused workspace too small");
+  FusedWs w;
+  carve_fused_ws(m, fws, &w);
+  StepHopArgs a{};
+  a.rzx = w.rzx; a.prob = m->prob; a.labels = labels; a.coeff = coeff; a.rows = m->Bp; a.C = m->dims[m->L]; a.B = m->B; a.scale_rz = -cg_alpha;
+  a.ce = ce; a.w1 = w1; a.b1 = b1; a.w2 = w2; a.b2 = b2; a.H = H; a.scale = scale;
+  a.gw1 = gw1; a.gb1 = gb1; a.gw2 = gw2; a.gb2 = gb2;
+  return launch_step_hop(a, static_cast<hipStream_t>(stream));
 }
 
 __global__ __launch_bounds__(256) void k_stage_batch(const float* __restrict__ x, const int64_t* __restrict__ y, float* __restrict__ h0,
@@ -2097,6 +2163,7 @@
   if (blocks < 1) blocks = 1;
   hipLaunchKernelGGL(k_stage_batch, dim3(blocks), dim3(256), 0, static_cast<hipStream_t>(stream), x, y, const_cast<float*>(m->h[0]), labels, n4, m->B);
   BHG_HIP_CHECK(hipGetLastError());
+  ++g_step_launches;
   return BHG_OK;
 }
 
diff --git a/betty_amd/csrc/bhg_mwn.hip b/betty_amd/csrc/bhg_mwn.hip
--- a/betty_amd/csrc/bhg_mwn.hip
+++ b/betty_amd/csrc/bhg_mwn.hip
@@ -1,33 +1,28 @@
 #include "bhg_common.hpp"
+#include "bhg_mwn_dev.hpp"
+#include "bhg_step.hpp"
 
 namespace bhg {
 namespace {
-
-constexpr int kMwnMaxH = 2048;
-constexpr int kMwnChunk = 1024;
-
-__device__ __forceinline__ float mwn_sigmoid(float z) { return 1.f / (1.f + expf(-z)); }
 
 __global__ __launch_bounds__(kThreads) void k_mwn_forward(const float* __restrict__ ce, int B, const float* __restrict__ w1,
                                                           const float* __restrict__ b1, const float* __restrict__ w2,
                                                           const float* __restrict__ b2, int H, float* __restrict__ s,
                                                           float* __restrict__ sd) {
   extern __shared__ float sp[];
-  for (int j = threadIdx.x; j < H; j += kThreads) { sp[j] = w1[j]; sp[H + j] = b1[j]; sp[2 * H + j] = w2[j]; }
+  mwn_stage_params(sp, w1, b1, w2, H);
   __syncthreads();
   const int i = blockIdx.x * kThreads + threadIdx.x;
   if (i >= B) return;
-  const float c = ce[i];
-  float z = b2[0];
-  for (int j = 0; j < H; ++j) {
-    const float a = fmaf(sp[j], c, sp[H + j]);
-    z = fmaf(sp[2 * H + j], a > 0.f ? a : 0.f, z);
-  }
-  const float v = mwn_sigmoid(z);
+  const float v = mwn_weight(sp, H, ce[i], b2[0]);
   if (s) s[i] = v;
   if (sd) sd[i] = v / (float)B;
 }
 
+struct MwnCoeffLoad {
+  const float* __restrict__ coeff;
+  __device__ __forceinline__ float operator()(int i, bool) const { return coeff[i]; }
+};
 __global__ __launch_bounds__(kThreads) void k_mwn_backward(const float* __restrict__ ce, const float* __restrict__ coeff, int B,
                                                            const float* __restrict__ w1, const float* __restrict__ b1,
                                                            const float* __restrict__ w2, const float* __restrict__ b2, int H,
@@ -35,72 +30,7 @@
                                                            float* __restrict__ gw2, float* __restrict__ gb2) {
   extern __shared__ float sp[];
   __shared__ float red[kWaves];
-  float* sdz = sp + 3 * H;
-  float* sce = sdz + kMwnChunk;
-  for (int j = threadIdx.x; j < H; j += kThreads) { sp[j] = w1[j]; sp[H + j] = b1[j]; sp[2 * H + j] = w2[j]; }
-  const float bias2 = b2[0];
-  constexpr int kPer = kMwnMaxH / kThreads;
-  float a_w1[kPer], a_b1[kPer], a_w2[kPer];
-#pragma unroll
-  for (int u = 0; u < kPer; ++u) a_w1[u] = a_b1[u] = a_w2[u] = 0.f;
-  float a_b2 = 0.f;
-  constexpr int kSPer = kMwnChunk / kThreads;
-  float c_pre[kSPer], k_pre[kSPer];
-#pragma unroll
-  for (int u = 0; u < kSPer; ++u) {
-    const int t = threadIdx.x + kThreads * u;
-    c_pre[u] = ce[t < B ? t : 0];
-    k_pre[u] = coeff[t < B ? t : 0];
-  }
-  __syncthreads();
-  for (int i0 = 0; i0 < B; i0 += kMwnChunk) {
-    const int n = B - i0 < kMwnChunk ? B - i0 : kMwnChunk;
-#pragma unroll
-    for (int u = 0; u < kSPer; ++u) {
-      const int t = threadIdx.x + kThreads * u;
-      if (t >= n) continue;
-      const float c = i0 == 0 ? c_pre[u] : ce[i0 + t];
-      const float kc = i0 == 0 ? k_pre[u] : coeff[i0 + t];
-      float z = bias2;
-      for (int j = 0; j < H; ++j) {
-        const float a = fmaf(sp[j], c, sp[H + j]);
-        z = fmaf(sp[2 * H + j], a > 0.f ? a : 0.f, z);
-      }
-      const float v = mwn_sigmoid(z);
-      const float dz = kc * (v * (1.f - v));
-      sdz[t] = dz;
-      sce[t] = c;
-      a_b2 += dz;
-    }
-    __syncthreads();
-#pragma unroll
-    for (int u = 0; u < kPer; ++u) {
-      const int j = threadIdx.x + kThreads * u;
-      if (j < H) {
-        const float wj = sp[j], bj = sp[H + j], vj = sp[2 * H + j];
-        for (int t = 0; t < n; ++t) {
-          const float c = sce[t], dz = sdz[t];
-          const float a = fmaf(wj, c, bj);
-          const bool on = a > 0.f;
-          a_w2[u] = fmaf(dz, on ? a : 0.f, a_w2[u]);
-          const float g1 = on ? dz * vj : 0.f;
-          a_b1[u] += g1;
-          a_w1[u] = fmaf(g1, c, a_w1[u]);
-        }
-      }
-    }
-    __syncthreads();
-  }
-#pragma unroll
-  for (int u = 0; u < kPer; ++u) {
-    const int j = threadIdx.x + kThreads * u;
-    if (j < H) { gw1[j] = scale * a_w1[u]; gb1[j] = scale * a_b1[u]; gw2[j] = scale * a_w2[u]; }
-  }
-#pragma unroll
-  for (int off = 32; off > 0; off >>= 1) a_b2 += __shfl_down(a_b2, off, 64);
-  if ((threadIdx.x & 63) == 0) red[threadIdx.x >> 6] = a_b2;
-  __syncthreads();
-  if (threadIdx.x == 0) gb2[0] = scale * ((red[0] + red[1]) + (red[2] + red[3]));
+  mwn_backward_body(ce, MwnCoeffLoad{coeff}, B, w1, b1, w2, b2, H, scale, gw1, gb1, gw2, gb2, sp, red);
 }
 
 int check_mwn(const float* ce, int B, const float* w1, const float* b1, const float* w2, const float* b2, int H) {
@@ -124,6 +54,7 @@
   BHG_REQUIRE(s || sd, "no output requested");
   hipLaunchKernelGGL(k_mwn_forward, dim3((B + kThreads - 1) / kThreads), dim3(kThreads), sizeof(float) * 3 * (size_t)H,
                      static_cast<hipStream_t>(stream), ce, B, w1, b1, w2, b2, H, s, sd);
+  ++g_step_launches;
   BHG_HIP_CHECK(hipGetLastError());
   return BHG_OK;
 }
@@ -134,6 +65,7 @@
   BHG_REQUIRE(coeff && gw1 && gb1 && gw2 && gb2, "NULL argument");
   hipLaunchKernelGGL(k_mwn_backward, dim3(1), dim3(kThreads), sizeof(float) * (3 * (size_t)H + 2 * kMwnChunk),
                      static_cast<hipStream_t>(stream), ce, coeff, B, w1, b1, w2, b2, H, scale, gw1, gb1, gw2, gb2);
+  ++g_step_launches;
   BHG_HIP_CHECK(hipGetLastError());
   return BHG_OK;
 }
diff --git a/betty_amd/csrc/bhg_mwn_dev.hpp b/betty_amd/csrc/bhg_mwn_dev.hpp
--- /dev/null
+++ b/betty_amd/csrc/bhg_mwn_dev.hpp
@@ -0,0 +1,96 @@
+#pragma once
+#include "bhg_common.hpp"
+
+namespace bhg {
+
+constexpr int kMwnMaxH = 2048;
+constexpr int kMwnChunk = 1024;
+
+#ifdef __HIPCC__
+__device__ __forceinline__ float mwn_sigmoid(float z) { return 1.f / (1.f + expf(-z)); }
+
+__device__ __forceinline__ void mwn_stage_params(float* sp, const float* __restrict__ w1, const float* __restrict__ b1,
+                                                 const float* __restrict__ w2, int H) {
+  for (int j = threadIdx.x; j < H; j += kThreads) { sp[j] = w1[j]; sp[H + j] = b1[j]; sp[2 * H + j] = w2[j]; }
+}
+
+__device__ __forceinline__ float mwn_weight(const float* sp, int H, float c, float bias2) {
+  float z = bias2;
+  for (int j = 0; j < H; ++j) {
+    const float a = fmaf(sp[j], c, sp[H + j]);
+    z = fmaf(sp[2 * H + j], a > 0.f ? a : 0.f, z);
+  }
+  return mwn_sigmoid(z);
+}
+
+template <class CoeffFn>
+__device__ __forceinline__ void mwn_backward_body(const float* __restrict__ ce, const CoeffFn& coeff_of, int B,
+                                                  const float* __restrict__ w1, const float* __restrict__ b1,
+                                                  const float* __restrict__ w2, const float* __restrict__ b2, int H, float scale,
+                                                  float* __restrict__ gw1, float* __restrict__ gb1, float* __restrict__ gw2,
+                                                  float* __restrict__ gb2, float* sp, float* red) {
+  float* sdz = sp + 3 * H;
+  float* sce = sdz + kMwnChunk;
+  mwn_stage_params(sp, w1, b1, w2, H);
+  const float bias2 = b2[0];
+  constexpr int kPer = kMwnMaxH / kThreads;
+  float a_w1[kPer], a_b1[kPer], a_w2[kPer];
+#pragma unroll
+  for (int u = 0; u < kPer; ++u) a_w1[u] = a_b1[u] = a_w2[u] = 0.f;
+  float a_b2 = 0.f;
+  constexpr int kSPer = kMwnChunk / kThreads;
+  float c_pre[kSPer], k_pre[kSPer];
+#pragma unroll
+  for (int u = 0; u < kSPer; ++u) {
+    const int t = threadIdx.x + kThreads * u;
+    c_pre[u] = ce[t < B ? t : 0];
+    k_pre[u] = coeff_of(t < B ? t : 0, t < B);
+  }
+  __syncthreads();
+  for (int i0 = 0; i0 < B; i0 += kMwnChunk) {
+    const int n = B - i0 < kMwnChunk ? B - i0 : kMwnChunk;
+#pragma unroll
+    for (int u = 0; u < kSPer; ++u) {
+      const int t = threadIdx.x + kThreads * u;
+      if (t >= n) continue;
+      const float c = i0 == 0 ? c_pre[u] : ce[i0 + t];
+      const float kc = i0 == 0 ? k_pre[u] : coeff_of(i0 + t, true);
+      const float v = mwn_weight(sp, H, c, bias2);
+      const float dz = kc * (v * (1.f - v));
+      sdz[t] = dz;
+      sce[t] = c;
+      a_b2 += dz;
+    }
+    __syncthreads();
+#pragma unroll
+    for (int u = 0; u < kPer; ++u) {
+      const int j = threadIdx.x + kThreads * u;
+      if (j < H) {
+        const float wj = sp[j], bj = sp[H + j], vj = sp[2 * H + j];
+        for (int t = 0; t < n; ++t) {
+          const float c = sce[t], dz = sdz[t];
+          const float a = fmaf(wj, c, bj);
+          const bool on = a > 0.f;
+          a_w2[u] = fmaf(dz, on ? a : 0.f, a_w2[u]);
+          const float g1 = on ? dz * vj : 0.f;
+          a_b1[u] += g1;
+          a_w1[u] = fmaf(g1, c, a_w1[u]);
+        }
+      }
+    }
+    __syncthreads();
+  }
+#pragma unroll
+  for (int u = 0; u < kPer; ++u) {
+    const int j = threadIdx.x + kThreads * u;
+    if (j < H) { gw1[j] = scale * a_w1[u]; gb1[j] = scale * a_b1[u]; gw2[j] = scale * a_w2[u]; }
+  }
+#pragma unroll
+  for (int off = 32; off > 0; off >>= 1) a_b2 += __shfl_down(a_b2, off, 64);
+  if ((threadIdx.x & 63) == 0) red[threadIdx.x >> 6] = a_b2;
+  __syncthreads();
+  if (threadIdx.x == 0) gb2[0] = scale * ((red[0] + red[1]) + (red[2] + red[3]));
+}
+#endif
+
+}
diff --git a/betty_amd/csrc/bhg_step.hip b/betty_amd/csrc/bhg_step.hip
--- /dev/null
+++ b/betty_amd/csrc/bhg_step.hip
@@ -0,0 +1,160 @@
+#include "bhg_common.hpp"
+#include "bhg_mwn_dev.hpp"
+#include "bhg_step.hpp"
+
+namespace bhg {
+
+int64_t g_step_launches = 0;
+
+namespace {
+
+using f32x4 = __attribute__((ext_vector_type(4))) float;
+__device__ __forceinline__ float4 ld16(const float* __restrict__ p) {
+  const f32x4 v = *reinterpret_cast<const f32x4*>(p);
+  return make_float4(v.x, v.y, v.z, v.w);
+}
+__device__ __forceinline__ float fz_mul(float a, float b) { return __fmul_rn(a, b); }
+__device__ __forceinline__ float fz_add(float a, float b) { return __fadd_rn(a, b); }
+constexpr int kSmallC = kStepMaxClasses;
+enum : int { HEAD_JVP = 0, HEAD_COEFF = 1, HEAD_LOGITS = 2 };
+struct HeadFuse {
+  const float* part;
+  int splits, slab;
+  const float* bias;
+  const float* mask;
+  float* rh_out;
+  const float* addend;
+};
+
+template <int JMAX>
+__device__ __forceinline__ void head_logits_row(const int b_row, const int rows, const float* h, const float* W, const float* cb,
+                                                float* rd, const int K, const int C, const int B, const int64_t* labels, float* aux) {
+  constexpr bool HAS_RH = false, FUSED = false, PF = false;
+  constexpr int mode = HEAD_LOGITS;
+  const float* const Rh = nullptr;
+  const float* const V = W;
+  const float* const prob = nullptr;
+  const float* const sd = nullptr;
+  const float* const delta_top = nullptr;
+  const float* const mask_prev = nullptr;
+  float* const rd_prev = nullptr;
+  float* const rd_prev_p = nullptr;
+  double* const partT1 = nullptr;
+  double* const partT2h = nullptr;
+  float* const rz_out = nullptr;
+  double* const rzx_acc = nullptr;
+  const int rzx_first = 0;
+  const HeadFuse fz{};
+  const float* const lazy_addend2 = nullptr;
+  const float lazy_beta = 0.f;
+  (void)Rh; (void)prob; (void)sd; (void)delta_top; (void)mask_prev; (void)rd_prev; (void)rd_prev_p; (void)partT1; (void)partT2h;
+  (void)rz_out; (void)rzx_acc; (void)rzx_first; (void)lazy_addend2; (void)lazy_beta; (void)rows;
+#define BHG_HEAD_B b_row
+#define BHG_HEAD_ROWS rows
+#define BHG_HEAD_LAZY 1
+#include "mlp/head_body.inc"
+#undef BHG_HEAD_B
+#undef BHG_HEAD_ROWS
+#undef BHG_HEAD_LAZY
+}
+
+template <int JMAX>
+__global__ __launch_bounds__(256) void k_step_tail(const StepTailArgs a) {
+  extern __shared__ __attribute__((aligned(16))) float step_dyn[];
+  __shared__ float sdt[kSmallC];
+  const int b = blockIdx.x, t = threadIdx.x;
+  const int K = a.K, C = a.C;
+  const bool live = b < a.B;
+  if (live) mwn_stage_params(step_dyn, a.w1, a.b1, a.w2, a.H);
+  head_logits_row<JMAX>(b, a.rows, a.h, a.W, a.bias, a.prob, K, C, a.B, a.labels, a.ce);
+  if (!live) {
+    if (t < C) a.dtop[(int64_t)b * C + t] = 0.f;
+    for (int n = 4 * t; n < K; n += 1024) {
+      const float4 z = make_float4(0.f, 0.f, 0.f, 0.f);
+      *reinterpret_cast<float4*>(a.dprev + (int64_t)b * K + n) = z;
+      if (a.dprev_p) *reinterpret_cast<float4*>(a.dprev_p + ((int64_t)(n >> 4) * a.rows + b) * 16 + (n & 15)) = z;
+    }
+    return;
+  }
+  __syncthreads();
+  const float v = mwn_weight(step_dyn, a.H, a.ce[b], a.b2[0]);
+  const float sdv = v / (float)a.B;
+  if (t == 0) {
+    if (a.s) a.s[b] = v;
+    a.sd[b] = sdv;
+  }
+  if (t < C) {
+    const float d = sdv * (a.prob[(int64_t)b * C + t] - ((int)a.labels[b] == t ? 1.f : 0.f));
+    a.dtop[(int64_t)b * C + t] = d;
+    sdt[t] = d;
+  }
+  __syncthreads();
+  for (int n = 4 * t; n < K; n += 1024) {
+    const float4 m = *reinterpret_cast<const float4*>(a.mask + (int64_t)b * K + n);
+    float4 acc = make_float4(0.f, 0.f, 0.f, 0.f);
+#pragma unroll 4
+    for (int c = 0; c < C; ++c) {
+      const float r = sdt[c];
+      const float4 w = *reinterpret_cast<const float4*>(a.W + (int64_t)c * K + n);
+      acc.x += r * w.x; acc.y += r * w.y; acc.z += r * w.z; acc.w += r * w.w;
+    }
+    acc.x *= m.x; acc.y *= m.y; acc.z *= m.z; acc.w *= m.w;
+    *reinterpret_cast<float4*>(a.dprev + (int64_t)b * K + n) = acc;
+    if (a.dprev_p) *reinterpret_cast<float4*>(a.dprev_p + ((int64_t)(n >> 4) * a.rows + b) * 16 + (n & 15)) = acc;
+  }
+}
+
+struct HopCoeff {
+  const double* __restrict__ rzx;
+  const float* __restrict__ prob;
+  const int64_t* __restrict__ labels;
+  float* __restrict__ coeff;
+  int C, B;
+  float scale;
+  __device__ __forceinline__ float operator()(const int i, const bool live) const {
+    if (!live) return 0.f;
+    const int y = (int)labels[i];
+    double acc = 0.0;
+    for (int c = 0; c < C; ++c) acc += ((double)prob[(int64_t)i * C + c] - (c == y ? 1.0 : 0.0)) * rzx[(int64_t)i * C + c];
+    const double o = (double)scale * acc / (double)B;
+    const float out = (float)o;
+    coeff[i] = out;
+    return out;
+  }
+};
+__global__ __launch_bounds__(kThreads) void k_step_hop(const StepHopArgs a) {
+  extern __shared__ float sp[];
+  __shared__ float red[kWaves];
+  for (int b = a.B + (int)threadIdx.x; b < a.rows; b += kThreads) a.coeff[b] = 0.f;
+  mwn_backward_body(a.ce, HopCoeff{a.rzx, a.prob, a.labels, a.coeff, a.C, a.B, a.scale_rz}, a.B, a.w1, a.b1, a.w2, a.b2, a.H, a.scale,
+                    a.gw1, a.gb1, a.gw2, a.gb2, sp, red);
+}
+
+}
+
+int launch_step_tail(const StepTailArgs& a, hipStream_t st) {
+  BHG_REQUIRE(a.h && a.W && a.bias && a.labels && a.prob && a.ce && a.sd && a.dtop && a.mask && a.dprev, "NULL argument");
+  BHG_REQUIRE(a.w1 && a.b1 && a.w2 && a.b2 && a.H >= 1 && a.H <= kMwnMaxH, "the closed-form meta-weight-net takes 1 <= hidden width <= 2048");
+  BHG_REQUIRE(a.C >= 1 && a.C <= kStepMaxClasses && a.K >= 4 && (a.K & 3) == 0, "narrow head only (<= 256 classes, feature width % 4 == 0)");
+  BHG_REQUIRE(a.rows >= 1 && a.B >= 1 && a.B <= a.rows, "1 <= B <= rows");
+  const size_t lds = sizeof(float) * 3 * (size_t)a.H;
+  if (a.C <= 12) hipLaunchKernelGGL(k_step_tail<3>, dim3(a.rows), dim3(256), lds, st, a);
+  else hipLaunchKernelGGL(k_step_tail<8>, dim3(a.rows), dim3(256), lds, st, a);
+  BHG_HIP_CHECK(hipGetLastError());
+  ++g_step_launches;
+  return BHG_OK;
+}
+
+int launch_step_hop(const StepHopArgs& a, hipStream_t st) {
+  BHG_REQUIRE(a.rzx && a.prob && a.labels && a.coeff && a.ce && a.gw1 && a.gb1 && a.gw2 && a.gb2, "NULL argument");
+  BHG_REQUIRE(a.w1 && a.b1 && a.w2 && a.b2 && a.H >= 1 && a.H <= kMwnMaxH, "the closed-form meta-weight-net takes 1 <= hidden width <= 2048");
+  BHG_REQUIRE(a.C >= 1 && a.rows >= 1 && a.B >= 1 && a.B <= a.rows, "1 <= B <= rows");
+  hipLaunchKernelGGL(k_step_hop, dim3(1), dim3(kThreads), sizeof(float) * (3 * (size_t)a.H + 2 * kMwnChunk), st, a);
+  BHG_HIP_CHECK(hipGetLastError());
+  ++g_step_launches;
+  return BHG_OK;
+}
+
+}
+
+extern "C" int64_t bhg_step_launches(void) { return bhg::g_step_launches; }
diff --git a/betty_amd/csrc/bhg_step.hpp b/betty_amd/csrc/bhg_step.hpp
--- /dev/null
+++ b/betty_amd/csrc/bhg_step.hpp
@@ -0,0 +1,35 @@
+#pragma once
+#include "bhg_common.hpp"
+
+namespace bhg {
+
+extern int64_t g_step_launches;
+
+constexpr int kStepMaxClasses = 256;
+
+struct StepTailArgs {
+  const float* h;
+  const float* W;
+  const float* bias;
+  const int64_t* labels;
+  float* prob;
+  float* ce;
+  const float* w1; const float* b1; const float* w2; const float* b2; int H;
+  float* s;
+  float* sd;
+  float* dtop;
+  const float* mask;
+  float* dprev;
+  float* dprev_p;
+  int K, C, B, rows;
+};
+int launch_step_tail(const StepTailArgs& a, hipStream_t st);
+
+struct StepHopArgs {
+  const double* rzx; const float* prob; const int64_t* labels; float* coeff; int rows, C, B; float scale_rz;
+  const float* ce; const float* w1; const float* b1; const float* w2; const float* b2; int H; float scale;
+  float* gw1; float* gb1; float* gw2; float* gb2;
+};
+int launch_step_hop(const StepHopArgs& a, hipStream_t st);
+
+}
diff --git a/betty_amd/hypergradient/_mlp_hip.py b/betty_amd/hypergradient/_mlp_hip.py
--- a/betty_amd/hypergradient/_mlp_hip.py
+++ b/betty_amd/hypergradient/_mlp_hip.py
@@ -132,6 +132,19 @@
 
         d.prepacked = 0
         self.packed_prepare = bool(buf.native_prepare and lib.bhg_mlp_supports_packed_prepare(ctypes.byref(d)))
+        native = _native_weight_net(lib, spec.weight_net, spec.prev.trainable_parameters(), x.device)
+        self.native_upper, self.sample_weight = native is not None, None
+        if self.native_upper:
+            self._wn, self._upper_slots = native
+        if self.packed_prepare and self.native_upper and lib.bhg_step_supports_prepare(ctypes.byref(d), self._wn[0].shape[0]):
+            fws, ts = self._fused_ws(x.device), self._wn
+            bias_tab, self._bias_keep = _native.ptr_array([b.data_ptr() for b in bs])
+            _native.check(lib.bhg_step_prepare(ctypes.byref(d), bias_tab, buf.labels.data_ptr(), buf.ce.data_ptr(), ts[0].data_ptr(),
+                                               ts[1].data_ptr(), ts[2].data_ptr(), ts[3].data_ptr(), ts[0].shape[0], None, fws.data_ptr(),
+                                               fws.numel(), _stream()), "bhg_step_prepare")
+            d.prepacked = 1
+            self._alloc_out(spec)
+            return
         if self.packed_prepare:
             fws = self._fused_ws(x.device)
             bias_tab, self._bias_keep = _native.ptr_array([b.data_ptr() for b in bs])
@@ -145,10 +158,7 @@
             ce = buf.ce[:B]
         else:
             raise _native.NativeLibraryError("bhg_mlp_supports_native_prepare refused this network (layer count / batch padding): there is no ATen path")
-        native = _native_weight_net(lib, spec.weight_net, spec.prev.trainable_parameters(), x.device)
-        self.native_upper, self.sample_weight = native is not None, None
         if self.native_upper:
-            self._wn, self._upper_slots = native
             ts = self._wn
             _native.check(lib.bhg_mwn_forward(buf.ce.data_ptr(), B, ts[0].data_ptr(), ts[1].data_ptr(), ts[2].data_ptr(), ts[3].data_ptr(),
                                               ts[0].shape[0], None, buf.sd.data_ptr(), _stream()), "bhg_mwn_forward")
@@ -161,6 +171,10 @@
             d.prepacked = 1
         else:
             _native.check(lib.bhg_mlp_backward(ctypes.byref(d), buf.labels.data_ptr(), _stream()), "bhg_mlp_backward")
+        self._alloc_out(spec)
+
+    def _alloc_out(self, spec):
+        buf = self.buf
         if buf.out is None:
             buf.out = []
             for lin in spec.layers:
@@ -183,6 +197,24 @@
                                       ts[3].data_ptr(), H, float(scale), g[0].data_ptr(), g[1].data_ptr(), g[2].data_ptr(),
                                       g[3].data_ptr(), _stream()), "bhg_mwn_backward")
         return (views, flat) if with_flat else views
+
+    def cg_hop(self, solve, upper, scale: float = 1.0):
+        if not (self.native_upper and solve is not None and solve.kind == "cg"):
+            return None
+        ts = self._wn
+        H = ts[0].shape[0]
+        if not self.lib.bhg_step_supports_cg_hop(ctypes.byref(self.desc), H):
+            return None
+        if solve is not getattr(self, "_solve", None):
+            raise RuntimeError("stale fused-solve token: another solve or a hand-driven HVP has reused this state's workspace")
+        buf = self.buf
+        flat, views, g = _flat_upper(upper, self._upper_slots, ts[0].device)
+        _native.check(
+            self.lib.bhg_step_cg_hop(ctypes.byref(self.desc), buf.labels.data_ptr(), buf.coeff.data_ptr(), solve.alpha, buf.fws.data_ptr(),
+                                     buf.fws.numel(), buf.ce.data_ptr(), ts[0].data_ptr(), ts[1].data_ptr(), ts[2].data_ptr(),
+                                     ts[3].data_ptr(), H, float(scale), g[0].data_ptr(), g[1].data_ptr(), g[2].data_ptr(), g[3].data_ptr(),
+                                     _stream()), "bhg_step_cg_hop")
+        return views, flat
 
     @staticmethod
     def _dir_table(direction_views):
@@ -452,6 +484,9 @@
 
     def upper_vjp(self, *a, **k):
         return self.inner.upper_vjp(*a, **k)
+
+    def cg_hop(self, *a, **k):
+        return self.inner.cg_hop(*a, **k)
 
     def _pad(self, tensors, into):
         for t, dst, (rows, cols), ldd in zip(tensors, into, self.shapes, self.pcols):
diff --git a/betty_amd/hypergradient/structured.py b/betty_amd/hypergradient/structured.py
--- a/betty_amd/hypergradient/structured.py
+++ b/betty_amd/hypergradient/structured.py
@@ -442,8 +442,10 @@
 
     def mixed_vjp(self, neg_x_views, sync: bool, solve=None):
         st = self._state
-        coeff = st.mixed_coeff(neg_x_views, solve) if solve is not None else st.mixed_coeff(neg_x_views)
         upper = self.prev.trainable_parameters()
+        one_hop = solve is not None and getattr(solve, "kind", None) == "cg" and st.native_upper and hasattr(st, "cg_hop")
+        if not one_hop:
+            coeff = st.mixed_coeff(neg_x_views, solve) if solve is not None else st.mixed_coeff(neg_x_views)
         if st.native_upper:
             wn = self.weight_net
             world, group = 1, None
@@ -465,7 +467,13 @@
                                 "cg_global(sync=True) with a closed-form weight net: declare SigmoidMLPWeightNet(average_over=True) (or a "
                                 "process group) or wrap the upper module in DistributedDataParallel — otherwise every rank would "
                                 "accumulate the hypergradient of its own batch share only")
-            grads, flat = st.upper_vjp(coeff, upper, scale=1.0 / world, with_flat=True)
+            hop = st.cg_hop(solve, upper, scale=1.0 / world) if one_hop else None
+            if hop is not None:
+                grads, flat = hop
+            else:
+                if one_hop:
+                    coeff = st.mixed_coeff(neg_x_views, solve)
+                grads, flat = st.upper_vjp(coeff, upper, scale=1.0 / world, with_flat=True)
             if sync:
                 from ..distributed import defer_grad_sync, fence_grads, install_optimizer_fence
 
diff --git a/include/bhg.h b/include/bhg.h
--- a/include/bhg.h
+++ b/include/bhg.h
@@ -187,6 +187,15 @@
 int bhg_mwn_backward(const float* ce, const float* coeff, int B, const float* w1, const float* b1, const float* w2, const float* b2,
                      int H, float scale, float* gw1, float* gb1, float* gw2, float* gb2, void* stream);
 
+int bhg_step_supports_prepare(const bhg_mlp* m, int H);
+int bhg_step_prepare(const bhg_mlp* m, const void* const* bias, const int64_t* labels, float* ce, const float* w1, const float* b1,
+                     const float* w2, const float* b2, int H, float* s, void* fws, size_t fws_bytes, void* stream);
+int bhg_step_supports_cg_hop(const bhg_mlp* m, int H);
+int bhg_step_cg_hop(const bhg_mlp* m, const int64_t* labels, float* coeff, float cg_alpha, void* fws, size_t fws_bytes, const float* ce,
+                    const float* w1, const float* b1, const float* w2, const float* b2, int H, float scale, float* gw1, float* gb1,
+                    float* gw2, float* gb2, void* stream);
+int64_t bhg_step_launches(void);
+
 int bhg_mlp_plan_describe(const bhg_mlp* m, int algo, int keep_solution, char* buf, size_t buf_bytes);
 
 int bhg_copy2d(float* dst, int64_t ldd, const float* src, int64_t lds, int64_t rows, int64_t cols, void* stream);
```

Result: no change. 773.3, median of 6 (+0.6%).
